# taki0112/vit-tensorflow

Measured on AMD Instinct MI355X. Metric: images/sec (fwd+bwd) ViT-B/16 224px bf16, higher is better.
Workload: dtype bf16; 1 GPU; vit_b16_224 fwd+bwd, batch 256/GPU, N(0,1) NHWC images resident in HBM, random-init weights, softmax-CE cotangent, dropout 0; global_batch=256, parallelism=dp1, compute=bf16

## Files before the change

### vit-tensorflow_amd/csrc/attn_bf16.hip

```cpp
#include "kernels.h"
#include "attn_lds.h"

#ifdef VITX_ATTN_PROBE
__device__ unsigned long long* vitx_attn_probe_buf;
#define ATTN_STAMP(i) do { if (threadIdx.x == 0 && vitx_attn_probe_buf) { vitx_attn_probe_buf[(size_t)blockIdx.x * 8 + (i)] = wall_clock64(); \
    if ((i) == 0) vitx_attn_probe_buf[(size_t)blockIdx.x * 8 + 6] = (unsigned long long)__builtin_amdgcn_s_getreg(63492) | ((unsigned long long)__builtin_amdgcn_s_getreg(63508) << 32); } } while (0)
#else
#define ATTN_STAMP(i) do { } while (0)
#endif

namespace {

using namespace attn_lds;

constexpr int ATT_THREADS = 512;

struct AttnLayout {
  int64_t tok_stride;
  int64_t kv_off;
  int64_t o_stride;
  int64_t q0, o0;
};
__device__ __forceinline__ AttnLayout attn_layout(int planar, int bi, int hi, int nb, int n, int h) {
  AttnLayout a;
// ... 77 lines not shown
}

template <bool MASKED, int QB>
__device__ __forceinline__ void fwd_max_pair(const char* k_rm, int u, int qi, int g, int n, const bf16x8 (&qf)[QB][2], float (&m)[QB]) {
  bf16x8 kf[2][2];
#pragma unroll
  for (int tt = 0; tt < 2; ++tt)
#pragma unroll
    for (int kh = 0; kh < 2; ++kh) kf[tt][kh] = frag_rm(k_rm, (2 * u + tt) * 16 + qi, g + 4 * kh);
  f32x4 a[2][QB];
#pragma unroll
  for (int tt = 0; tt < 2; ++tt)
#pragma unroll
    for (int s = 0; s < QB; ++s) a[tt][s] = mfma16(kf[tt][0], qf[s][0], f32x4{0.f, 0.f, 0.f, 0.f});
#pragma unroll
  for (int tt = 0; tt < 2; ++tt)
#pragma unroll
    for (int s = 0; s < QB; ++s) a[tt][s] = mfma16(kf[tt][1], qf[s][1], a[tt][s]);
#pragma unroll
  for (int tt = 0; tt < 2; ++tt)
#pragma unroll
    for (int s = 0; s < QB; ++s) {
      f32x4 v = a[tt][s];
      if (MASKED) {
#pragma unroll
        for (int r = 0; r < 4; ++r) v[r] = ((2 * u + tt) * 16 + 4 * g + r) < n ? v[r] : -INFINITY;
      }
      m[s] = fmaxf(fmaxf(m[s], fmaxf(v[0], v[1])), fmaxf(v[2], v[3]));
    }
}

template <int NTP>
__global__ __launch_bounds__(ATT_THREADS, 4) void attn_fwd_kernel(const bf16_t* __restrict__ qkv, bf16_t* __restrict__ o, float* __restrict__ lse,
                                                       int n, int h, float scale, const bf16_t* __restrict__ zero_page, int reverse, int planar) {
  constexpr int NKP = 16 * NTP, QB = QB_FWD;
  extern __shared__ __attribute__((aligned(16))) char smem[];
  char* k_rm = smem;
  char* v_rm = smem + NKP * ROWB;
  const int bh = reverse ? (int)(gridDim.x - 1 - blockIdx.x) : (int)blockIdx.x, bi = bh / h, hi = bh - bi * h;
  const AttnLayout L = attn_layout(planar, bi, hi, (int)gridDim.x / h, n, h);
  const int64_t tok_stride = L.tok_stride;
  const bf16_t* qbase = qkv + L.q0;
  const int tid = threadIdx.x, lane = tid & 63, nwaves = blockDim.x >> 6;
  const int wave = __builtin_amdgcn_readfirstlane(tid >> 6);
  ATTN_STAMP(0);
  stage_head_dma(qbase + L.kv_off, tok_stride, n, NKP, k_rm, zero_page, wave, lane, nwaves);
  stage_head_dma(qbase + 2 * L.kv_off, tok_stride, n, NKP, v_rm, zero_page, wave, lane, nwaves);

  const int qi = lane & 15, g = lane >> 4;
  const int nqb = (n + 16 * QB - 1) / (16 * QB);
  const float sl2 = scale * 1.44269504088896340736f;
  bf16x8 qf[QB][2];
  auto load_q = [&](int qb) {
#pragma unroll
    for (int s = 0; s < QB; ++s) {
      const int qc = min((qb * QB + s) * 16 + qi, n - 1);
#pragma unroll
      for (int ks = 0; ks < 2; ++ks) qf[s][ks] = *(const bf16x8*)(qbase + (int64_t)qc * tok_stride + (g + 4 * ks) * 8);
    }
  };
  if (wave < nqb) load_q(wave);
  asm volatile("s_waitcnt vmcnt(0)" ::: "memory");
  ATTN_STAMP(1);
  __syncthreads();
  ATTN_STAMP(2);

  const int u_full = n >> 5;
  const int u_end = min(NTP / 2, (n + 31) >> 5);
  for (int qb = wave; qb < nqb; qb += nwaves) {
    float m[QB];
#pragma unroll
    for (int s = 0; s < QB; ++s) m[s] = -INFINITY;
#pragma unroll 1
    for (int u = 0; u < u_full; ++u) fwd_max_pair<false, QB>(k_rm, u, qi, g, n, qf, m);
    if (u_full < u_end) fwd_max_pair<true, QB>(k_rm, u_full, qi, g, n, qf, m);
#pragma unroll
    for (int s = 0; s < QB; ++s) {
      m[s] = fmaxf(m[s], __shfl_xor(m[s], 16, 64));
      m[s] = fmaxf(m[s], __shfl_xor(m[s], 32, 64));
      m[s] *= sl2;
    }
    ATTN_STAMP(3);
    f32x2 lv[QB];
    f32x4 oacc[QB][4];
#pragma unroll
    for (int s = 0; s < QB; ++s) {
      lv[s] = f32x2{0.f, 0.f};
#pragma unroll
      for (int c = 0; c < 4; ++c) oacc[s][c] = f32x4{0.f, 0.f, 0.f, 0.f};
    }
#pragma unroll 1
    for (int u = 0; u < u_full; ++u) fwd_pair<false, QB>(k_rm, v_rm, u, qi, g, lane, n, qf, sl2, m, lv, oacc);
    if (u_full < u_end) fwd_pair<true, QB>(k_rm, v_rm, u_full, qi, g, lane, n, qf, sl2, m, lv, oacc);
    ATTN_STAMP(4);
#pragma unroll
    for (int s = 0; s < QB; ++s) {
      const int q = (qb * QB + s) * 16 + qi;
      float ls = lv[s][0] + lv[s][1];
      ls += __shfl_xor(ls, 16, 64);
      ls += __shfl_xor(ls, 32, 64);
      const float inv_l = 1.0f / ls;
      if (g == 0 && q < n) lse[(int64_t)bh * n + q] = (m[s] + log2f(ls)) * 0.69314718055994530942f;
      if (q < n) {
        bf16_t* op = o + L.o0 + (int64_t)q * L.o_stride;
#pragma unroll
        for (int c = 0; c < 4; ++c) {
          bf16x4 ov;
#pragma unroll
          for (int r = 0; r < 4; ++r) ov[r] = (bf16_t)(oacc[s][c][r] * inv_l);
          *(bf16x4*)(op + 16 * c + 4 * g) = ov;
        }
      }
    }
    if (qb + nwaves < nqb) load_q(qb + nwaves);
  }
  ATTN_STAMP(5);
}

template <bool MASKED>
__device__ __forceinline__ void dq_pair(const char* k_rm, const char* v_rm, int u, int qi, int g, int lane, int n, const bf16x8 (&qf)[2],
                                        const bf16x8 (&dof)[2], float sl2, float lse2, float scale, float nds, f32x4 (&dq)[4]) {
  bf16x8 kf[2][2], vf[2][2], kt[4];
#pragma unroll
  for (int tt = 0; tt < 2; ++tt)
#pragma unroll
    for (int kh = 0; kh < 2; ++kh) {
      kf[tt][kh] = frag_rm(k_rm, (2 * u + tt) * 16 + qi, g + 4 * kh);
      vf[tt][kh] = frag_rm(v_rm, (2 * u + tt) * 16 + qi, g + 4 * kh);
    }
#pragma unroll
  for (int c = 0; c < 4; ++c) kt[c] = frag_trr(k_rm, c, u, lane);
  f32x4 sa[2], dp[2];
#pragma unroll
  for (int tt = 0; tt < 2; ++tt) {
    sa[tt] = mfma16(kf[tt][0], qf[0], f32x4{0.f, 0.f, 0.f, 0.f});
    dp[tt] = mfma16(vf[tt][0], dof[0], f32x4{0.f, 0.f, 0.f, 0.f});
// ... 4 lines not shown
    dp[tt] = mfma16(vf[tt][1], dof[1], dp[tt]);
  }
  f32x4 ds[2];
#pragma unroll
  for (int tt = 0; tt < 2; ++tt) {
    const f32x4 e = sa[tt] * sl2 - lse2;
    const f32x4 w = dp[tt] * scale + nds;
#pragma unroll
    for (int r = 0; r < 4; ++r) {
      float p = fast_exp2(e[r]);
      if (MASKED) p = ((2 * u + tt) * 16 + 4 * g + r) < n ? p : 0.f;
      ds[tt][r] = p * w[r];
    }
  }
  const bf16x8 dsf = pack8(ds[0], ds[1]);
#pragma unroll
  for (int c = 0; c < 4; ++c) dq[c] = mfma16(kt[c], dsf, dq[c]);
}

struct DqOperands { bf16x8 qf[2], dof[2], of[2]; };
__device__ __forceinline__ void dq_load(DqOperands& x, const bf16_t* qbase, int64_t tok_stride, const bf16_t* o_rows, const bf16_t* do_rows, int64_t inner,
                                        int qb, int lane, int n) {
  const int qc = min(qb * 16 + (lane & 15), n - 1), g = lane >> 4;
#pragma unroll
  for (int ks = 0; ks < 2; ++ks) {
    x.qf[ks] = *(const bf16x8*)(qbase + (int64_t)qc * tok_stride + (g + 4 * ks) * 8);
    x.dof[ks] = *(const bf16x8*)(do_rows + (int64_t)qc * inner + (g + 4 * ks) * 8);
    x.of[ks] = *(const bf16x8*)(o_rows + (int64_t)qc * inner + (g + 4 * ks) * 8);
  }
}

template <int NTP>
__device__ __forceinline__ float dq_block(const char* k_rm, const char* v_rm, const DqOperands& x, int64_t tok_stride, bf16_t* dq_rows, int qb, int lane,
                                          int n, float scale, float lse2) {
  const int qi = lane & 15, g = lane >> 4;
  const int q = qb * 16 + qi;
  const float sl2 = scale * 1.44269504088896340736f;
  const bf16x8 (&qf)[2] = x.qf;
  const bf16x8 (&dof)[2] = x.dof;
  float dsum = 0.f;
#pragma unroll
  for (int ks = 0; ks < 2; ++ks)
#pragma unroll
    for (int e = 0; e < 8; ++e) dsum += (float)x.dof[ks][e] * (float)x.of[ks][e];
  dsum += __shfl_xor(dsum, 16, 64);
  dsum += __shfl_xor(dsum, 32, 64);
  const float nds = -dsum * scale;
  f32x4 dq[4];
#pragma unroll
  for (int c = 0; c < 4; ++c) dq[c] = f32x4{0.f, 0.f, 0.f, 0.f};
  const int u_full = n >> 5, u_end = min(NTP / 2, (n + 31) >> 5);
#pragma unroll 1
  for (int u = 0; u < u_full; ++u) dq_pair<false>(k_rm, v_rm, u, qi, g, lane, n, qf, dof, sl2, lse2, scale, nds, dq);
  if (u_full < u_end) dq_pair<true>(k_rm, v_rm, u_full, qi, g, lane, n, qf, dof, sl2, lse2, scale, nds, dq);
  if (q < n) {
    bf16_t* out = dq_rows + (int64_t)q * tok_stride;
#pragma unroll
    for (int c = 0; c < 4; ++c) {
      bf16x4 ov;
#pragma unroll
      for (int r = 0; r < 4; ++r) ov[r] = (bf16_t)dq[c][r];
      *(bf16x4*)(out + 16 * c + 4 * g) = ov;
    }
  }
  return dsum;
}

struct DkvOperands { bf16x8 kf[2], vf[2]; };
__device__ __forceinline__ void dkv_load(DkvOperands& x, const bf16_t* kbase, int64_t tok_stride, int64_t inner, int kb, int lane, int n) {
  const int kc = min(kb * 16 + (lane & 15), n - 1), g = lane >> 4;
#pragma unroll
  for (int ks = 0; ks < 2; ++ks) {
    x.kf[ks] = *(const bf16x8*)(kbase + (int64_t)kc * tok_stride + (g + 4 * ks) * 8);
    x.vf[ks] = *(const bf16x8*)(kbase + inner + (int64_t)kc * tok_stride + (g + 4 * ks) * 8);
  }
}

template <int NTP>
__device__ __forceinline__ void dkv_block(const char* q_rm, const char* do_rm, const float* lse_s, const float* d_s, const DkvOperands& x,
                                          int64_t tok_stride, int64_t inner, bf16_t* dk_rows, int kb, int lane, int n, float scale) {
  const int ki = lane & 15, g = lane >> 4;
  const int key = kb * 16 + ki;
  const float sl2 = scale * 1.44269504088896340736f;
  const bf16x8 (&kf)[2] = x.kf;
  const bf16x8 (&vf)[2] = x.vf;
  f32x4 dk[4], dv[4];
#pragma unroll
  for (int c = 0; c < 4; ++c) { dk[c] = f32x4{0.f, 0.f, 0.f, 0.f}; dv[c] = f32x4{0.f, 0.f, 0.f, 0.f}; }
  const int u_end = min(NTP / 2, (n + 31) >> 5);
#pragma unroll 1
  for (int u = 0; u < u_end; ++u) {
    f32x4 pp[2], ds[2];
#pragma unroll
    for (int tt = 0; tt < 2; ++tt) {
      const int t = 2 * u + tt;
      const bf16x8 qa0 = frag_rm(q_rm, t * 16 + ki, g), qa1 = frag_rm(q_rm, t * 16 + ki, g + 4);
      const bf16x8 da0 = frag_rm(do_rm, t * 16 + ki, g), da1 = frag_rm(do_rm, t * 16 + ki, g + 4);
      float lq[4], dd[4];
#pragma unroll
      for (int r = 0; r < 4; ++r) { lq[r] = lse_s[t * 16 + 4 * g + r]; dd[r] = d_s[t * 16 + 4 * g + r]; }
      f32x4 sa = {0.f, 0.f, 0.f, 0.f}, dp = {0.f, 0.f, 0.f, 0.f};
      sa = mfma16(qa0, kf[0], sa);
      sa = mfma16(qa1, kf[1], sa);
      dp = mfma16(da0, vf[0], dp);
      dp = mfma16(da1, vf[1], dp);
#pragma unroll
      for (int r = 0; r < 4; ++r) {
        const float p = fast_exp2(fmaf(sa[r], sl2, -lq[r]));
        pp[tt][r] = p;
        ds[tt][r] = p * ((dp[r] - dd[r]) * scale);
      }
    }
    const bf16x8 pf = pack8(pp[0], pp[1]), dsf = pack8(ds[0], ds[1]);
#pragma unroll
    for (int c = 0; c < 4; ++c) {
      const bf16x8 a1 = frag_trr(do_rm, c, u, lane), a2 = frag_trr(q_rm, c, u, lane);
      dv[c] = mfma16(a1, pf, dv[c]);
      dk[c] = mfma16(a2, dsf, dk[c]);
    }
  }
  if (key < n) {
    bf16_t* dkp = dk_rows + (int64_t)key * tok_stride;
    bf16_t* dvp = dkp + inner;
#pragma unroll
    for (int c = 0; c < 4; ++c) {
      bf16x4 a, b2;
#pragma unroll
      for (int r = 0; r < 4; ++r) { a[r] = (bf16_t)dk[c][r]; b2[r] = (bf16_t)dv[c][r]; }
      *(bf16x4*)(dkp + 16 * c + 4 * g) = a;
      *(bf16x4*)(dvp + 16 * c + 4 * g) = b2;
    }
  }
}

template <int NTP>
__global__ __launch_bounds__(ATT_THREADS) void attn_bwd_dq_kernel(const bf16_t* __restrict__ qkv, const bf16_t* __restrict__ o,
                                                          const bf16_t* __restrict__ d_o, const float* __restrict__ lse,
                                                          float* __restrict__ dsum, bf16_t* __restrict__ dqkv, int n, int h, float scale,
                                                          const bf16_t* __restrict__ zero_page) {
  constexpr int NKP = 16 * NTP;
  extern __shared__ __attribute__((aligned(16))) char smem[];
  char* k_rm = smem;
  char* v_rm = smem + NKP * ROWB;
  const int bh = blockIdx.x, bi = bh / h, hi = bh - bi * h;
  const int inner = h * DH;
  const int64_t tok_stride = 3 * (int64_t)inner;
  const bf16_t* qbase = qkv + (int64_t)bi * n * tok_stride + hi * DH;
  const int tid = threadIdx.x, lane = tid & 63, nwaves = blockDim.x >> 6;
  const int wave = __builtin_amdgcn_readfirstlane(tid >> 6);
  stage_head_dma(qbase + inner, tok_stride, n, NKP, k_rm, zero_page, wave, lane, nwaves);
  stage_head_dma(qbase + 2 * inner, tok_stride, n, NKP, v_rm, zero_page, wave, lane, nwaves);
  asm volatile("s_waitcnt vmcnt(0)" ::: "memory");
  __syncthreads();
  const int64_t orow0 = (int64_t)bi * n * inner + hi * DH;
  for (int qb = wave; qb < (n + 15) / 16; qb += nwaves) {
    const int qi = lane & 15, q = qb * 16 + qi, qc = min(q, n - 1);
    DqOperands x;
    dq_load(x, qbase, tok_stride, o + orow0, d_o + orow0, inner, qb, lane, n);
    const float d = dq_block<NTP>(k_rm, v_rm, x, tok_stride, dqkv + (int64_t)bi * n * tok_stride + hi * DH, qb, lane, n, scale,
                                  lse[(int64_t)bh * n + qc] * 1.44269504088896340736f);
    if ((lane >> 4) == 0 && q < n) dsum[(int64_t)bh * n + q] = d;
  }
}

template <int NTP>
__global__ __launch_bounds__(ATT_THREADS) void attn_bwd_dkv_kernel(const bf16_t* __restrict__ qkv, const bf16_t* __restrict__ d_o,
                                                           const float* __restrict__ lse, const float* __restrict__ dsum,
                                                           bf16_t* __restrict__ dqkv, int n, int h, float scale, const bf16_t* __restrict__ zero_page) {
  constexpr int NQP = 16 * NTP;
  extern __shared__ __attribute__((aligned(16))) char smem[];
  char* q_rm = smem;
  char* do_rm = smem + NQP * ROWB;
  float* lse_s = (float*)(smem + 2 * NQP * ROWB);
  float* d_s = lse_s + NQP;
  const int bh = blockIdx.x, bi = bh / h, hi = bh - bi * h;
  const int inner = h * DH;
  const int64_t tok_stride = 3 * (int64_t)inner;
  const bf16_t* qbase = qkv + (int64_t)bi * n * tok_stride + hi * DH;
  const int tid = threadIdx.x, lane = tid & 63, nwaves = blockDim.x >> 6;
  const int wave = __builtin_amdgcn_readfirstlane(tid >> 6);
  stage_head_dma(qbase, tok_stride, n, NQP, q_rm, zero_page, wave, lane, nwaves);
  stage_head_dma(d_o + (int64_t)bi * n * inner + hi * DH, inner, n, NQP, do_rm, zero_page, wave, lane, nwaves);
  for (int i = tid; i < NQP; i += blockDim.x) {
    lse_s[i] = i < n ? lse[(int64_t)bh * n + i] * 1.44269504088896340736f : 0.f;
    d_s[i] = i < n ? dsum[(int64_t)bh * n + i] : 0.f;
  }
  asm volatile("s_waitcnt vmcnt(0)" ::: "memory");
  __syncthreads();
  for (int kb = wave; kb < (n + 15) / 16; kb += nwaves) {
    DkvOperands x;
    dkv_load(x, qbase + inner, tok_stride, inner, kb, lane, n);
    dkv_block<NTP>(q_rm, do_rm, lse_s, d_s, x, tok_stride, inner, dqkv + (int64_t)bi * n * tok_stride + inner + hi * DH, kb, lane, n, scale);
  }
}

template <int NTP>
__global__ __launch_bounds__(ATT_THREADS, 4) void attn_bwd_fused_kernel(const bf16_t* __restrict__ qkv, const bf16_t* __restrict__ o,
                                                             const bf16_t* __restrict__ d_o, const float* __restrict__ lse,
                                                             bf16_t* __restrict__ dqkv, int n, int h, float scale,
                                                             const bf16_t* __restrict__ zero_page, int planar) {
  constexpr int NKP = 16 * NTP, NQP = 16 * NTP;
  extern __shared__ __attribute__((aligned(16))) char smem[];
  char* k_rm = smem;
  char* v_rm = smem + NKP * ROWB;
  char* q_rm = k_rm;
  char* do_rm = v_rm;
  float* lse_s = (float*)(smem + 2 * NKP * ROWB);
  float* d_s = lse_s + NQP;
  const int bh = blockIdx.x, bi = bh / h, hi = bh - bi * h;
  const AttnLayout L = attn_layout(planar, bi, hi, (int)gridDim.x / h, n, h);
  const int64_t tok_stride = L.tok_stride, inner = L.kv_off, ostr = L.o_stride;
  const bf16_t* qbase = qkv + L.q0;
  const int tid = threadIdx.x, lane = tid & 63, nwaves = blockDim.x >> 6;
  const int wave = __builtin_amdgcn_readfirstlane(tid >> 6);
  stage_head_dma(qbase + inner, tok_stride, n, NKP, k_rm, zero_page, wave, lane, nwaves);
  stage_head_dma(qbase + 2 * inner, tok_stride, n, NKP, v_rm, zero_page, wave, lane, nwaves);
  for (int i = tid; i < NQP; i += blockDim.x) {
    lse_s[i] = i < n ? lse[(int64_t)bh * n + i] * 1.44269504088896340736f : 0.f;
    d_s[i] = 0.f;
  }
  const int64_t orow0 = L.o0;
  const int nblk = (n + 15) / 16;
  DqOperands xq;
  if (wave < nblk) dq_load(xq, qbase, tok_stride, o + orow0, d_o + orow0, ostr, wave, lane, n);
  ATTN_STAMP(0);
  asm volatile("s_waitcnt vmcnt(0)" ::: "memory");
  __syncthreads();
  ATTN_STAMP(1);
  for (int qb = wave; qb < nblk; qb += nwaves) {
    const int q = qb * 16 + (lane & 15);
    DqOperands nx;
    if (qb + nwaves < nblk) dq_load(nx, qbase, tok_stride, o + orow0, d_o + orow0, ostr, qb + nwaves, lane, n);
    const float d = dq_block<NTP>(k_rm, v_rm, xq, tok_stride, dqkv + L.q0, qb, lane, n, scale, lse_s[min(q, n - 1)]);
    if ((lane >> 4) == 0 && q < n) d_s[q] = d;
    xq = nx;
  }
  DkvOperands xk;
  if (wave < nblk) dkv_load(xk, qbase + inner, tok_stride, inner, wave, lane, n);
  ATTN_STAMP(2);
  __syncthreads();
  ATTN_STAMP(3);
  stage_head_dma(qbase, tok_stride, n, NQP, q_rm, zero_page, wave, lane, nwaves);
  stage_head_dma(d_o + orow0, ostr, n, NQP, do_rm, zero_page, wave, lane, nwaves);
  asm volatile("s_waitcnt vmcnt(0)" ::: "memory");
  __syncthreads();
  ATTN_STAMP(4);
  for (int kb = wave; kb < nblk; kb += nwaves) {
    DkvOperands nx;
    if (kb + nwaves < nblk) dkv_load(nx, qbase + inner, tok_stride, inner, kb + nwaves, lane, n);
    dkv_block<NTP>(q_rm, do_rm, lse_s, d_s, xk, tok_stride, inner, dqkv + L.q0 + inner, kb, lane, n, scale);
    xk = nx;
  }
  ATTN_STAMP(5);
}

template <typename K>
void set_smem(K kern, int bytes) {
  vitx_set_max_smem((const void*)kern, bytes);
}

#ifdef VITX_ATTN_PROBE
int vitx_attn_probe_threads = 512;
inline int att_threads(int n) { (void)n; return vitx_attn_probe_threads; }
inline int pick_ntp(int n) { return n <= 64 ? 4 : n <= 96 ? 6 : n <= 192 ? 12 : n <= 224 ? 14 : 18; }
#else
inline int att_threads(int n) { (void)n; return 512; }
inline int pick_ntp(int n) { return n <= 64 ? 4 : n <= 96 ? 6 : n <= 224 ? 14 : 18; }
#endif

}

bool attn_bf16_supported(int n, int dim_head) { return dim_head == DH && n >= 1 && n <= 288; }

#define VITX_NTP_DISPATCH(ntp, CALL) \
  do { if ((ntp) == 4) { CALL(4); } else if ((ntp) == 6) { CALL(6); } else if ((ntp) == 14) { CALL(14); } else if ((ntp) == 12) { VITX_NTP12(CALL); } else { CALL(18); } } while (0)
#ifdef VITX_ATTN_PROBE
#define VITX_NTP12(CALL) CALL(12)
#else
#define VITX_NTP12(CALL) CALL(14)
#endif

int vitx_attn_probe_planar = 0;

void launch_attn_bf16_fwd(const bf16_t* qkv, bf16_t* o, float* lse, int b, int n, int h, float scale, const bf16_t* zero_page, int reverse, hipStream_t s) {
  const int ntp = pick_ntp(n);
  const int nkp = 16 * ntp;
  const int smem = 2 * nkp * ROWB;
#define CALL(NTP) { set_smem(attn_fwd_kernel<NTP>, smem); hipLaunchKernelGGL(attn_fwd_kernel<NTP>, dim3(b * h), dim3(att_threads(n)), smem, s, qkv, o, lse, n, h, scale, zero_page, reverse, vitx_attn_probe_planar); }
  VITX_NTP_DISPATCH(ntp, CALL);
#undef CALL
}

void launch_attn_bf16_bwd(const bf16_t* qkv, const bf16_t* o, const bf16_t* d_o, const float* lse, float* dsum_ws, bf16_t* dqkv, int b,
                          int n, int h, float scale, const bf16_t* zero_page, hipStream_t s) {
  const int ntp = pick_ntp(n);
  const int np = 16 * ntp;
  const int smem_dq = 2 * np * ROWB;
  const int smem_dkv = 2 * np * ROWB + 2 * np * 4;
  const char* split_env = vitx_env("VITX_ATTN_BWD_SPLIT");
  const bool split = split_env && atoi(split_env) != 0;
  if (!split) {
#define CALLF(NTP) { set_smem(attn_bwd_fused_kernel<NTP>, smem_dkv); hipLaunchKernelGGL(attn_bwd_fused_kernel<NTP>, dim3(b * h), dim3(att_threads(n)), smem_dkv, s, qkv, o, d_o, lse, dqkv, n, h, scale, zero_page, vitx_attn_probe_planar); }
    VITX_NTP_DISPATCH(ntp, CALLF);
#undef CALLF
    return;
  }
#define CALL(NTP)                                                                                                                  \
  {                                                                                                                                \
    set_smem(attn_bwd_dq_kernel<NTP>, smem_dq);                                                                                    \
    set_smem(attn_bwd_dkv_kernel<NTP>, smem_dkv);                                                                                  \
    hipLaunchKernelGGL(attn_bwd_dq_kernel<NTP>, dim3(b * h), dim3(att_threads(n)), smem_dq, s, qkv, o, d_o, lse, dsum_ws, dqkv, n, h, scale, zero_page);   \
    hipLaunchKernelGGL(attn_bwd_dkv_kernel<NTP>, dim3(b * h), dim3(att_threads(n)), smem_dkv, s, qkv, d_o, lse, dsum_ws, dqkv, n, h, scale, zero_page);    \
  }
  VITX_NTP_DISPATCH(ntp, CALL);
#undef CALL
}
```

### vit-tensorflow_amd/csrc/capi.hip

```cpp
#include <dlfcn.h>

#include <cstring>
#include <map>

#include "composite.h"

static thread_local std::string g_last_error;

static int fail(int code, const std::string& msg) {
  g_last_error = msg;
  return code;
}
int capi_fail(int code, const std::string& msg) { return fail(code, msg); }

extern "C" {

const char* vitx_version(void) { return "vitx 0.1.0 (gfx950)"; }
const char* vitx_last_error(void) { return g_last_error.c_str(); }

int32_t vitx_param_table_size(const vitx_config* cfg, int64_t* n_tensors, int64_t* n_elems) {
  CAPI_TRY
  if (!cfg) return fail(VITX_ERR_INVALID, "null config");
  vitx_config c = *cfg;
  if (c.channels <= 0) c.channels = 3;
// ... 739 lines not shown
  h->prof_events.clear();
  int n = 0;
  for (auto& s : stats) {
    if (s.launches == 0) continue;
    if (out && n < cap) out[n] = s;
    ++n;
  }
  if (n_out) *n_out = n;
  return VITX_OK;
  CAPI_CATCH
}

int32_t vitx_workspace_bytes(vitx_handle h, int64_t* bytes) {
  if (!h) return fail(VITX_ERR_INVALID, "null handle");
  if (bytes) *bytes = h->ws_bytes;
  return VITX_OK;
}

int32_t vitx_debug_read(vitx_handle h, const char* which, int32_t layer, float* out_host, int64_t cap, int64_t* n_elems) {
  CAPI_TRY
  if (!h || !which) return fail(VITX_ERR_INVALID, "null argument");
  const vitx_config& c = h->cfg;
  const int b = h->last_b;
  Stage* st = nullptr;
  int l = layer, nq = h->last_ntok, nk = h->last_ntok;
  for (auto& s : h->stages) {
    if (l < s.depth) { st = &s; break; }
    l -= s.depth;
  }
  const std::string w(which);
  const void* src = nullptr;
  int64_t rows = 0, cols = 0, ld = 0;
  bool is_t = false;
  if (w == "pooled_ln") { src = h->yh; rows = b; cols = ld = c.dim; is_t = true; }
  else if (w == "logits") { src = h->logits; rows = b; cols = c.num_classes; ld = h->nc_k; }
  else if (w == "dlogits") { src = h->dlogits; rows = b; cols = c.num_classes; ld = h->nc_k; }
  else if (w == "patches") { src = h->patches; rows = (int64_t)b * h->last_np; cols = h->pd; ld = h->pd_k; is_t = true; }
  else {
    if (!st) return fail(VITX_ERR_INVALID, "layer out of range");
    if (c.variant == VITX_VARIANT_CAIT) { nq = st->nq_max == 1 ? 1 : h->last_np; nk = st->nq_max == 1 ? 1 + h->last_np : h->last_np; }
    BlockActs& ba = st->ba[(size_t)l];
    rows = (int64_t)b * nq;
    if (w == "x_in" || w == "embed") { src = ba.x_in; cols = ld = c.dim; }
    else if (w == "x_mid") { src = ba.x_mid; cols = ld = c.dim; }
    else if (w == "x_out") { src = ba.x_out; cols = ld = c.dim; }
    else if (w == "y1") { src = ba.y1; cols = ld = c.dim; is_t = true; }
    else if (w == "y2") { src = ba.y2; cols = ld = c.dim; is_t = true; }
    else if (w == "qkv") { src = ba.qkv; cols = ld = 3 * h->inner; is_t = true; }
    else if (w == "q") { src = ba.q; cols = ld = h->inner; is_t = true; }
    else if (w == "kv") { src = ba.kv; rows = (int64_t)b * nk; cols = ld = 2 * h->inner; is_t = true; }
    else if (w == "attn_out") { src = ba.o; cols = ld = h->inner; is_t = true; }
    else if (w == "hpre") { src = ba.hpre; cols = ld = c.mlp_dim; is_t = true; }
    else if (w == "act") { src = ba.act; cols = ld = c.mlp_dim; is_t = true; }
    else return fail(VITX_ERR_INVALID, "unknown activation name");
  }
  if (!src) return fail(VITX_ERR_INVALID, "activation not available for this variant");
  const int64_t n = rows * cols;
  if (n_elems) *n_elems = n;
  if (!out_host) return VITX_OK;
  if (cap < n) return fail(VITX_ERR_INVALID, "output buffer too small");
  float* tmp = nullptr;
  CAPI_HIP(hipMalloc((void**)&tmp, (size_t)std::max<int64_t>(n, 1) * 4));
  launch_to_f32(src, is_t && h->bf16, ld, tmp, cols, (int)rows, (int)cols, h->stream);
  CAPI_HIP(hipMemcpyAsync(out_host, tmp, (size_t)n * 4, hipMemcpyDeviceToHost, h->stream));
  CAPI_HIP(hipStreamSynchronize(h->stream));
  (void)hipFree(tmp);
  return VITX_OK;
  CAPI_CATCH
}

int32_t vitx_check_gemm(vitx_handle h, int32_t kind, int32_t M, int32_t N, int32_t K, int32_t kernel, int32_t epilogue, float* errs2) {
  CAPI_TRY
  if (!h || !errs2) return fail(VITX_ERR_INVALID, "null argument");
  std::string err;
// ... 21 lines not shown
```

### vit-tensorflow_amd/csrc/elementwise.hip

```cpp
#include "kernels.h"

namespace {

template <typename TO>
__global__ void unfold_kernel(const float* __restrict__ img, TO* __restrict__ out, int b, int H, int W, int C, int ph, int pw,
                              int64_t ldo) {
  const int Hp = H / ph, Wp = W / pw;
  const int pd = ph * pw * C;
  const int run = pw * C;
  const int64_t total = (int64_t)b * Hp * Wp * ldo;
  for (int64_t e = (int64_t)blockIdx.x * blockDim.x + threadIdx.x; e < total; e += (int64_t)gridDim.x * blockDim.x) {
    const int64_t row = e / ldo;
    const int f = (int)(e - row * ldo);
    float v = 0.f;
    if (f < pd) {
      const int r = f / run, sc = f - r * run;
      const int wi = (int)(row % Wp);
      const int64_t t = row / Wp;
      const int hi = (int)(t % Hp);
      const int64_t bi = t / Hp;
      v = img[((bi * H + (int64_t)hi * ph + r) * W + (int64_t)wi * pw) * C + sc];
    }
    stf<TO>(out + e, v);
  }
// ... 416 lines not shown
    const int cc = c0 + c, rr = r0 + tx;
    if (cc < cols && rr < rows) op[(int64_t)cc * ldo + rr] = tile[tx][c];
  }
}

template <typename TO>
__global__ void convert_kernel(const float* __restrict__ in, int64_t ldi, TO* __restrict__ out, int64_t ldo, int rows, int cols,
                               int64_t zero_to) {
  const int64_t total = (int64_t)rows * zero_to;
  for (int64_t e = (int64_t)blockIdx.x * blockDim.x + threadIdx.x; e < total; e += (int64_t)gridDim.x * blockDim.x) {
    const int64_t r = e / zero_to;
    const int c = (int)(e - r * zero_to);
    stf<TO>(out + r * ldo + c, c < cols ? in[r * ldi + c] : 0.f);
  }
}

template <typename TI>
__global__ void to_f32_kernel(const TI* __restrict__ in, int64_t ldi, float* __restrict__ out, int64_t ldo, int rows, int cols) {
  const int64_t total = (int64_t)rows * cols;
  for (int64_t e = (int64_t)blockIdx.x * blockDim.x + threadIdx.x; e < total; e += (int64_t)gridDim.x * blockDim.x) {
    const int64_t r = e / cols;
    const int c = (int)(e - r * cols);
    out[r * ldo + c] = ldf<TI>(in + r * ldi + c);
  }
}

__global__ void set_token_row_kernel(float* __restrict__ x, const float* __restrict__ tok, int b, int ntok, int row, int d) {
  const int64_t e = (int64_t)blockIdx.x * blockDim.x + threadIdx.x;
  if (e >= (int64_t)b * d) return;
  const int64_t bi = e / d;
  const int c = (int)(e - bi * d);
  x[(bi * ntok + row) * d + c] = tok[c];
}
__global__ void mean_pool_kernel(const float* __restrict__ x, int b, int ntok, int d, float* __restrict__ out, int stride_tok) {
  const int64_t total = (int64_t)b * d;
  for (int64_t e = (int64_t)blockIdx.x * blockDim.x + threadIdx.x; e < total; e += (int64_t)gridDim.x * blockDim.x) {
    const int64_t bi = e / d;
    const int c = (int)(e - bi * d);
    float a = 0.f;
    for (int t = 0; t < ntok; ++t) a += x[(bi * stride_tok + t) * d + c];
    out[e] = a / (float)ntok;
  }
}
__global__ void mean_pool_bwd_kernel(const float* __restrict__ dp, int b, int ntok, int d, float* __restrict__ g, int stride_tok) {
  const int64_t total = (int64_t)b * ntok * d;
  for (int64_t e = (int64_t)blockIdx.x * blockDim.x + threadIdx.x; e < total; e += (int64_t)gridDim.x * blockDim.x) {
    const int c = (int)(e % d);
    const int64_t bi = e / ((int64_t)ntok * d);
    g[e + bi * (int64_t)(stride_tok - ntok) * d] = dp[bi * d + c] / (float)ntok;
  }
}
__global__ void batch_reduce_kernel(const float* __restrict__ g, int b, int ntok, int d, int j0, int nj, float* __restrict__ out) {
  const int64_t total = (int64_t)nj * d;
  for (int64_t e = (int64_t)blockIdx.x * blockDim.x + threadIdx.x; e < total; e += (int64_t)gridDim.x * blockDim.x) {
    const int64_t j = e / d;
    const int c = (int)(e - j * d);
    float a = 0.f;
    for (int bi = 0; bi < b; ++bi) a += g[((int64_t)bi * ntok + j0 + j) * d + c];
    out[e] = a;
  }
}
template <typename TO>
__global__ void extract_rows_kernel(const float* __restrict__ g, int b, int ntok, int tok_off, int np, int d, TO* __restrict__ out,
                                    int64_t ldo) {
  const int64_t total = (int64_t)b * np * d;
  for (int64_t e = (int64_t)blockIdx.x * blockDim.x + threadIdx.x; e < total; e += (int64_t)gridDim.x * blockDim.x) {
// ... 393 lines not shown
  const int chunks = (int)std::max<int64_t>(1, std::min<int64_t>({(int64_t)CS_CHUNKS, ceil_div(rows, 16), ceil_div(2048, cblocks)}));
  dim3 grid((unsigned)cblocks, chunks), block(256);
  if (is_bf16) hipLaunchKernelGGL(colsum_kernel<bf16_t>, grid, block, 0, s, (const bf16_t*)x, ld, rows, cols, partial_ws);
  else hipLaunchKernelGGL(colsum_kernel<float>, grid, block, 0, s, (const float*)x, ld, rows, cols, partial_ws);
  launch_reduce_partials3(partial_ws, chunks, cols, cols, 1, out, nullptr, nullptr, partial_ws + (int64_t)CS_CHUNKS * cols, 1.0f, s);
}

void launch_convert_weight(const float* w, int in, int out, bf16_t* wn, int64_t ldwn, bf16_t* wt, int64_t ldwt, hipStream_t s) {
  dim3 grid((unsigned)ceil_div(out, 64), (unsigned)ceil_div(in, 64)), block(256);
  hipLaunchKernelGGL(convert_weight_kernel, grid, block, 0, s, w, in, out, wn, ldwn, wt, ldwt);
}
void launch_convert_weights_batched(const ConvertDesc* descs_dev, int n, int total_blocks, hipStream_t s) {
  if (n > 0 && total_blocks > 0) hipLaunchKernelGGL(convert_weights_batched_kernel, dim3((unsigned)total_blocks), dim3(256), 0, s, descs_dev, n);
}
void launch_transpose_bf16(const bf16_t* in, int64_t ldi, int rows, int cols, bf16_t* out, int64_t ldo, hipStream_t s) {
  dim3 grid((unsigned)ceil_div(cols, 64), (unsigned)ceil_div(rows, 64)), block(256);
  hipLaunchKernelGGL(transpose_bf16_kernel, grid, block, 0, s, in, ldi, rows, cols, out, ldo);
}
void launch_convert(const float* in, int64_t ldi, void* out, int out_bf16, int64_t ldo, int rows, int cols, int64_t zero_to,
                    hipStream_t s) {
  const int64_t total = (int64_t)rows * zero_to;
  if (total == 0) return;
  if (out_bf16) hipLaunchKernelGGL(convert_kernel<bf16_t>, dim3(grid_for(total)), dim3(256), 0, s, in, ldi, (bf16_t*)out, ldo, rows, cols, zero_to);
  else hipLaunchKernelGGL(convert_kernel<float>, dim3(grid_for(total)), dim3(256), 0, s, in, ldi, (float*)out, ldo, rows, cols, zero_to);
}
void launch_to_f32(const void* in, int in_bf16, int64_t ldi, float* out, int64_t ldo, int rows, int cols, hipStream_t s) {
  const int64_t total = (int64_t)rows * cols;
  if (total == 0) return;
  if (in_bf16) hipLaunchKernelGGL(to_f32_kernel<bf16_t>, dim3(grid_for(total)), dim3(256), 0, s, (const bf16_t*)in, ldi, out, ldo, rows, cols);
  else hipLaunchKernelGGL(to_f32_kernel<float>, dim3(grid_for(total)), dim3(256), 0, s, (const float*)in, ldi, out, ldo, rows, cols);
}
void launch_set_token_row(float* x, const float* tok, int b, int ntok, int row, int d, hipStream_t s) {
  hipLaunchKernelGGL(set_token_row_kernel, dim3((unsigned)ceil_div((int64_t)b * d, 256)), dim3(256), 0, s, x, tok, b, ntok, row, d);
}
void launch_mean_pool(const float* x, int b, int ntok, int d, float* out, hipStream_t s, int stride_tok) {
  hipLaunchKernelGGL(mean_pool_kernel, dim3(grid_for((int64_t)b * d)), dim3(256), 0, s, x, b, ntok, d, out, stride_tok ? stride_tok : ntok);
}
void launch_mean_pool_bwd(const float* dp, int b, int ntok, int d, float* g, hipStream_t s, int stride_tok) {
  hipLaunchKernelGGL(mean_pool_bwd_kernel, dim3(grid_for((int64_t)b * ntok * d)), dim3(256), 0, s, dp, b, ntok, d, g, stride_tok ? stride_tok : ntok);
}
void launch_batch_reduce(const float* g, int b, int ntok, int d, int j0, int nj, float* out, hipStream_t s) {
  if (nj <= 0) return;
  if (d % 4 == 0 && ((uintptr_t)g) % 16 == 0 && ((uintptr_t)out) % 16 == 0) {
    if (b >= 32) hipLaunchKernelGGL(batch_reduce4_split_kernel, dim3((unsigned)ceil_div((int64_t)nj * (d / 4), 64)), dim3(512), 0, s, g, b, ntok, d / 4, j0, nj, out);
    else hipLaunchKernelGGL(batch_reduce4_kernel, dim3((unsigned)ceil_div((int64_t)nj * (d / 4), 64)), dim3(64), 0, s, g, b, ntok, d / 4, j0, nj, out);
    return;
  }
  hipLaunchKernelGGL(batch_reduce_kernel, dim3(grid_for((int64_t)nj * d)), dim3(256), 0, s, g, b, ntok, d, j0, nj, out);
}
void launch_extract_rows(const float* g, int b, int ntok, int tok_off, int np, int d, void* out, int out_bf16, int64_t ldo, hipStream_t s) {
  const int64_t total = (int64_t)b * np * d;
  if (total == 0) return;
  if (d % 4 == 0 && ldo % 4 == 0 && ((uintptr_t)g) % 16 == 0 && ((uintptr_t)out) % 16 == 0) {
    if (out_bf16) hipLaunchKernelGGL(extract_rows4_kernel<bf16_t>, dim3(grid_for(total / 4)), dim3(256), 0, s, g, b, ntok, tok_off, np, d / 4, (bf16_t*)out, ldo);
    else hipLaunchKernelGGL(extract_rows4_kernel<float>, dim3(grid_for(total / 4)), dim3(256), 0, s, g, b, ntok, tok_off, np, d / 4, (float*)out, ldo);
    return;
  }
  if (out_bf16) hipLaunchKernelGGL(extract_rows_kernel<bf16_t>, dim3(grid_for(total)), dim3(256), 0, s, g, b, ntok, tok_off, np, d, (bf16_t*)out, ldo);
  else hipLaunchKernelGGL(extract_rows_kernel<float>, dim3(grid_for(total)), dim3(256), 0, s, g, b, ntok, tok_off, np, d, (float*)out, ldo);
}
void launch_sum_rows(const float* in, int rows, int d, float* out, hipStream_t s) {
  if (rows >= 32) hipLaunchKernelGGL(sum_rows_split_kernel, dim3((unsigned)ceil_div(d, 64)), dim3(256), 0, s, in, rows, d, out);
  else hipLaunchKernelGGL(sum_rows_kernel, dim3((unsigned)ceil_div(d, 256)), dim3(256), 0, s, in, rows, d, out);
}
void launch_ce_grad(const float* logits, int64_t ld, const int32_t* labels, int b, int nc, float inv_batch, float* dlogits, float* loss,
                    hipStream_t s) {
// ... 187 lines not shown
```

### vit-tensorflow_amd/csrc/engine.h

```cpp
#pragma once
#include <string>
#include <vector>

#include "../../include/vitx.h"
#include "kernels.h"

struct ParamDesc {
  std::string name;
  std::vector<int64_t> shape;
  int64_t offset = 0, count = 0;
  int64_t aoff = 0;
};

std::string build_param_table(const vitx_config& c, std::vector<ParamDesc>& out);

struct CommState {
  hipStream_t stream = nullptr;
  void* all_reduce = nullptr;
  int overlap = 0;
  int64_t bucket = 0;
  int wire_bf16 = 0;
  bf16_t* wire = nullptr;
  std::vector<int64_t> covered;
  std::vector<char> launched;
// ... 15 lines not shown
  int64_t w = -1, b = -1;
  bf16_t* wt = nullptr;
  bf16_t* wn = nullptr;
  const float *ext_w = nullptr, *ext_b = nullptr;
  float *ext_gw = nullptr, *ext_gb = nullptr;
};

struct BlockParams {
  int64_t a_scale = -1, ln1_g = -1, ln1_b = -1;
  int64_t temp = -1;
  Dense qkv, q, kv, out;
  Dense qkvcat;
  bool has_out = true;
  int64_t mix_pre = -1, mix_post = -1, re_w = -1, re_g = -1, re_b = -1;
  int64_t m_scale = -1, ln2_g = -1, ln2_b = -1;
  Dense fc1, fc2;
  int64_t p_begin = 0, p_end = 0;
};

struct BlockActs {
  float *x_in = nullptr, *x_mid = nullptr, *x_out = nullptr;
  void *y1 = nullptr, *qkv = nullptr, *q = nullptr, *kv = nullptr, *ctx = nullptr, *o = nullptr, *fa = nullptr;
  void *y2 = nullptr, *hpre = nullptr, *act = nullptr, *fm = nullptr;
  float *mean1 = nullptr, *rstd1 = nullptr, *mean2 = nullptr, *rstd2 = nullptr, *lse = nullptr;
  const float *ln1_src = nullptr, *ln2_src = nullptr;
  bool skip_attn = false, skip_mlp = false;
  float* sc_keep[3] = {nullptr, nullptr, nullptr};
  int64_t sc_keep_elems = 0;
  int64_t sc_geom = -1;
  int sc_pi = 0;
  bool sc_no_mixed = false;
  bool sc_a2_bf16 = false;
  int par_first = 0, par_last = 0;
};

struct Stage {
  std::string prefix;
  int depth = 0;
  int nq_max = 0, nc_max = 0;
  std::vector<BlockParams> bp;
  std::vector<BlockActs> ba;
};

struct ProfEvent {
  int cls;
  int cls2 = -1;
  hipEvent_t e0, e1;
  double flops, bytes;
};

constexpr int SIDE_RING_MAX = 8;
struct SideRing {
  void* slot[SIDE_RING_MAX] = {};
  hipEvent_t rd[SIDE_RING_MAX] = {};
  bool pend[SIDE_RING_MAX] = {};
  int n = 0, cur = 0;
};
struct PendingReady { int64_t off, cnt; hipEvent_t ev; };

struct vitx_engine {
  vitx_config cfg{};
  std::vector<ParamDesc> table;
  int64_t n_params = 0;
  int64_t n_arena = 0;
  bool bf16 = false;
  bool x3_attn = false;
// ... 28 lines not shown
  int merge_after = -1, merge_t = 0;
  int64_t pm_g = -1, pm_b = -1, pm_q = -1;
  float *pm_xn = nullptr, *pm_mean = nullptr, *pm_rstd = nullptr, *pm_attn = nullptr, *pm_dattn = nullptr, *pm_out = nullptr, *pm_dxn = nullptr,
        *pm_dxn2 = nullptr, *pm_dq = nullptr;

  int64_t spt_g = -1, spt_b = -1;
  float *spt_mean = nullptr, *spt_rstd = nullptr, *spt_img = nullptr, *spt_ws = nullptr, *lsa_ws = nullptr;

  int64_t pos = -1, cls = -1, head_g = -1, head_b = -1;
  Dense patch, head;
  std::vector<Stage> stages;

  std::vector<void*> allocs;
  std::vector<std::pair<void*, size_t>> t_buffers;
  int64_t ws_bytes = 0;
  float* img_dev = nullptr;
  void* patches = nullptr;
  float* pooled = nullptr; void* yh = nullptr; float *mean_h = nullptr, *rstd_h = nullptr;
  float *logits = nullptr, *dlogits = nullptr; void* dl_lp = nullptr; void* dyh = nullptr; float* dpooled = nullptr;
  float* g2 = nullptr;
  float* g = nullptr; void* g_lp = nullptr; float* g_ctx = nullptr;
  void *d_h = nullptr, *d_y = nullptr, *d_o = nullptr, *d_qkv = nullptr, *d_ctx = nullptr, *d_br = nullptr;
  bf16_t *xt = nullptr, *dyt = nullptr; int64_t t_rows = 0;
  float* partial_ws = nullptr; int64_t partial_elems = 0;
  float* red_ws = nullptr; int64_t red_elems = 0;
  float* sc[4] = {nullptr, nullptr, nullptr, nullptr}; int64_t sc_elems = 0;
  float* dsum = nullptr;
  void* zero_page = nullptr;
  float* tmp_f32 = nullptr;
  float* loss_rows = nullptr;
  float* distill_ws = nullptr;
  float *opt_m = nullptr, *opt_v = nullptr; int opt_step = 0;
  bf16_t *bench_a = nullptr, *bench_b = nullptr; float* bench_c = nullptr; int64_t bench_elems = 0;

  bool have_fwd = false;
  bool have_tf = false;
  int next_patch_np = 0;
  const float* fwd_patches = nullptr;
  int fwd_np = 0;
  bool last_from_patches = false;
  int tf_b = 0, tf_n = 0;
  float tf_drop = 0.f;
  uint64_t tf_seed = 0;
  bool have_embed = false, have_head = false;
  int shell_b = 0, shell_n = 0;
  float* shell_x = nullptr;
  bool have_pt = false;
  int pt_b = 0, pt_np = 0;
  int64_t patch_rows = -1;
  void* pt_dy = nullptr;
  int64_t pt_dy_rows = -1;
  int last_extra = 0;
  int last_b = 0, last_np = 0, last_ntok = 0, last_H = 0, last_W = 0, last_training = 0;
  uint64_t last_seed = 0;
  std::vector<std::vector<bool>> layer_kept;
  int64_t zero_geom = -1;

  bool keep_scores = true;
  int64_t sc_keep_bytes = 0, sc_keep_budget = 48LL << 30;
  bool force_generic_gemm = false, force_generic_attn = false, wgrad_via_transpose = true;
  bool small_attn = true;
  int gemm_kernel = 0;
  int gemm_tail = 0;
  int reverse_mask = 7;
  int64_t reverse_min_bytes = 200ll << 20;
  bool bgemm_pairs = true;
// ... 6 lines not shown
  bool score_bf16 = true;
  bool cait_qkv_cat = true;
  bool cait_fused = true;
  bool deepvit_fused = true;
  bool unfused_headops = false;
  int gemm_stagger = 0;

  bool profiling = false;
  std::vector<ProfEvent> prof_events;
  std::vector<std::string> prof_names;

  vitx_grad_ready_fn grad_cb = nullptr; void* grad_cb_user = nullptr;
  void* rccl_lib = nullptr; void* comm = nullptr; int rank = 0, world = 1;
  CommState cm;
};

int comm_unique_id(void* out128, std::string& err);
int comm_init(vitx_engine* e, int rank, int world, const void* uid, std::string& err);
int comm_overlap(vitx_engine* e, int enable, int64_t bucket_bytes, int wire_bf16, std::string& err);
void comm_on_ready(vitx_engine* e, int64_t off, int64_t cnt);
int comm_busy(vitx_engine* e);
void comm_wait_event(vitx_engine* e, hipEvent_t ev);
int comm_finish(vitx_engine* e, std::string& err);
void comm_stats(vitx_engine* e, int64_t* out4);
void comm_destroy(vitx_engine* e);

int engine_check_small_dataset(const vitx_config& cfg, std::string& err);
int engine_create(const vitx_config& cfg, vitx_engine** out, std::string& err);
void engine_destroy(vitx_engine* e);
int engine_forward(vitx_engine* e, const float* img_dev, int b, int H, int W, int training, uint64_t seed, float* logits_dev,
                   std::string& err, const float* distill_token_dev = nullptr, float* distill_out_dev = nullptr);
int engine_backward(vitx_engine* e, const float* dlogits_dev, float* dimg_dev, std::string& err, const float* d_distill_dev = nullptr,
                    float* d_token_out_dev = nullptr);
int engine_transformer_forward(vitx_engine* e, const float* tokens_dev, int b, int n, int training, uint64_t seed, float* out_dev, std::string& err);
int engine_transformer_backward(vitx_engine* e, const float* dout_dev, float* dtokens_dev, std::string& err);
int engine_patch_tokens_forward(vitx_engine* e, const float* img_dev, int b, int H, int W, float* tokens_dev, float* patches_f32_dev_or_null,
                                std::string& err);
int engine_patch_tokens_backward(vitx_engine* e, const float* dtokens_dev, std::string& err);
int engine_embed_forward(vitx_engine* e, const float* img_dev, int b, int H, int W, float* tokens_dev, std::string& err);
int engine_spt_forward(vitx_engine* e, const float* img_dev, int b, int H, int W, float* tokens_dev, std::string& err);
int engine_patch_dense_forward(vitx_engine* e, const float* patches_dev, int rows, float* out_dev, std::string& err);
int engine_head_forward(vitx_engine* e, const float* x_dev, int b, int n, float* logits_dev, std::string& err);
int engine_head_backward(vitx_engine* e, const float* dlogits_dev, float* dx_dev, std::string& err);
int engine_embed_backward(vitx_engine* e, const float* dtokens_dev, float* dimg_dev, std::string& err);
void engine_refresh_weights(vitx_engine* e);
void engine_params_moved(vitx_engine* e);
int engine_ext_dense_init(vitx_engine* e, Dense& w, int in, int out, const float* W, const float* bias, float* gW, float* gbias, std::string& err);
void engine_ext_dense_refresh(vitx_engine* e, const Dense& w);
void engine_ext_dense_fwd(vitx_engine* e, const void* X, int64_t ldx, int rows, const Dense& w, float* y);
void engine_ext_dense_bwd(vitx_engine* e, const void* X, int64_t ldx, const void* dY, int64_t ldy, const float* dY_f32, int rows, const Dense& w,
                          float* dx_or_null);
int engine_check_gemm(vitx_engine* e, int kind, int M, int N, int K, int kernel, int epilogue, float* errs, std::string& err);
int engine_bench_gemm(vitx_engine* e, int M, int N, int K, int kernel, int epilogue, int iters, float* avg_ms, float* max_err,
                      std::string& err);
int prof_class(vitx_engine* e, const char* name);
```

### vit-tensorflow_amd/csrc/engine.hip

```cpp
#include "engine.h"

#include <algorithm>
#include <cmath>
#include <cstdio>
#include <cstdlib>
#include <cstring>

#define HIPCHK(x)                                                                                   \
  do {                                                                                              \
    hipError_t e_ = (x);                                                                            \
    if (e_ != hipSuccess) {                                                                         \
      err = std::string(#x) + ": " + hipGetErrorString(e_);                                         \
      return VITX_ERR_HIP;                                                                          \
    }                                                                                               \
  } while (0)

std::string build_param_table(const vitx_config& c, std::vector<ParamDesc>& out) {
  out.clear();
  if (c.variant < 0 || c.variant > 3) return "unknown variant";
  if (c.patch_h <= 0 || c.patch_w <= 0 || c.image_h <= 0 || c.image_w <= 0) return "image/patch size must be positive";
  if (c.image_h % c.patch_h != 0 || c.image_w % c.patch_w != 0)
    return "Image dimensions must be divisible by the patch size.";
  if (c.variant != VITX_VARIANT_CAIT && c.pool != VITX_POOL_CLS && c.pool != VITX_POOL_MEAN)
    return "pool type must be either cls (cls token) or mean (mean pooling)";
// ... 840 lines not shown
    Prof pr(e, "attn_generic_headops", 0, 0);
    if (e->cfg.variant == VITX_VARIANT_CAIT) {
      launch_headmix_bwd(sc[1], dA, e->params + bp.mix_post, dA, e->red_ws, e->grads + bp.mix_post, b, h, a.nq, a.nk, ld, e->stream);
      launch_softmax_bwd_rows(sc[1], dA, rows, a.nk, ld, e->stream);
      launch_headmix_bwd(sc[0], dA, e->params + bp.mix_pre, dA, e->red_ws, e->grads + bp.mix_pre, b, h, a.nq, a.nk, ld, e->stream);
    } else if (e->cfg.variant == VITX_VARIANT_DEEPVIT) {
      launch_headnorm_bwd(sc[1], dA, e->params + bp.re_g, dA, e->red_ws, e->grads + bp.re_g, e->grads + bp.re_b, b, h, a.nq, a.nk, ld,
                          e->cfg.ln_eps, e->stream);
      launch_headmix_bwd(sc[0], dA, e->params + bp.re_w, dA, e->red_ws, e->grads + bp.re_w, b, h, a.nq, a.nk, ld, e->stream);
      launch_softmax_bwd_rows(sc[0], dA, rows, a.nk, ld, e->stream);
    } else {
      launch_softmax_bwd_rows(sc[0], dA, rows, a.nk, ld, e->stream);
    }
  }
  if (ds_lp) {
    bgemm_pair(e, BgemmCall{ds_lp, 1, ld2, 1, bs2, hs2, a.k, T, a.ldk, 1, a.kb, dh, a.nq, dh, a.nk, b, h, EPI_STORE, T, gr.dq, gr.lddq, gr.dqb, dh, scale},
               BgemmCall{ds_lp, 1, 1, ld2, bs2, hs2, a.q, T, a.ldq, 1, a.qb, dh, a.nk, dh, a.nq, b, h, EPI_STORE, T, gr.dk, gr.lddk, gr.dkb, dh, scale});
    return;
  }
  bgemm_pair(e, BgemmCall{dA, 0, ld, 1, bs, hs, a.k, T, a.ldk, 1, a.kb, dh, a.nq, dh, a.nk, b, h, EPI_STORE, T, gr.dq, gr.lddq, gr.dqb, dh, scale},
             BgemmCall{dA, 0, 1, ld, bs, hs, a.q, T, a.ldq, 1, a.qb, dh, a.nk, dh, a.nq, b, h, EPI_STORE, T, gr.dk, gr.lddk, gr.dkb, dh, scale});
}

static bool use_small_attn(const vitx_engine* e, int n) {
  return e->cfg.nest_block && e->small_attn && !e->force_generic_attn && attn_small_supported(n, e->cfg.dim_head);
}
static bool use_fused_attn(const vitx_engine* e, int n) {
  return e->bf16 && e->cfg.variant == VITX_VARIANT_VIT && !e->force_generic_attn && attn_bf16_supported(n, e->cfg.dim_head);
}
static bool use_fused_attn_x3(const vitx_engine* e, int n) {
  return e->x3 && e->x3_attn && e->x3_fused_attn && e->cfg.variant == VITX_VARIANT_VIT && !e->force_generic_attn && attn_x3_supported(n, e->cfg.dim_head);
}

static int block_forward(vitx_engine* e, Stage& st, int si, int l, int b, int nq, int nc, const float* context, float drop, uint64_t seed,
                         std::string& err) {
  const uint32_t site0 = (uint32_t)((si * 1000 + l) * 4);
  const BlockParams& bp = st.bp[l];
  BlockActs& ba = st.ba[l];
  const vitx_config& c = e->cfg;
  const int d = c.dim, inner = e->inner, m = c.mlp_dim, T = e->bf16, esz = e->esz;
  const int rows = b * nq;
  const int nk = nq + nc;
  const double lnb = (double)rows * d * (4 + esz);
  if (!ba.skip_attn) {
  {
    Prof pr(e, "layernorm_fwd", 0, lnb);
    launch_layernorm_fwd(ba.ln1_src ? ba.ln1_src : ba.x_in, d, e->params + bp.ln1_g, e->params + bp.ln1_b, ba.y1, T, d, ba.mean1, ba.rstd1, rows, d, c.ln_eps,
                         e->stream);
  }
  AttnView av;
  av.nq = nq; av.nk = nk; av.o = ba.o; av.ldo = inner; av.ob = (int64_t)nq * inner;
  if (c.variant == VITX_VARIANT_CAIT && bp.qkvcat.wt) {
    EpiParams ep; ep.out = ba.qkv; ep.ldo = 3 * inner;
    dense_fwd(e, ba.y1, d, rows, bp.qkvcat, EPI_STORE, ep);
    av.q = ba.qkv; av.k = boff(ba.qkv, inner, esz); av.v = boff(ba.qkv, 2 * inner, esz);
    av.ldq = av.ldk = av.ldv = 3 * inner;
    av.qb = av.kb = av.vb = (int64_t)nq * 3 * inner;
  } else if (c.variant == VITX_VARIANT_CAIT) {
    EpiParams ep; ep.out = ba.q; ep.ldo = inner;
    dense_fwd(e, ba.y1, d, rows, bp.q, EPI_STORE, ep);
    const void* ctx = ba.y1;
    if (nc > 0) {
      Prof pr(e, "concat_ctx", 0, 0);
      launch_concat_ctx(ba.y1, T, context, ba.ctx, T, b, nq, nc, d, e->stream);
      ctx = ba.ctx;
    }
    EpiParams ep2; ep2.out = ba.kv; ep2.ldo = 2 * inner;
    dense_fwd(e, ctx, d, b * nk, bp.kv, EPI_STORE, ep2);
    av.q = ba.q; av.ldq = inner; av.qb = (int64_t)nq * inner;
    av.k = ba.kv; av.ldk = 2 * inner; av.kb = (int64_t)nk * 2 * inner;
    av.v = boff(ba.kv, inner, esz); av.ldv = 2 * inner; av.vb = av.kb;
  } else {
    EpiParams ep; ep.out = ba.qkv; ep.ldo = 3 * inner;
    dense_fwd(e, ba.y1, d, rows, bp.qkv, EPI_STORE, ep);
    av.q = ba.qkv; av.k = boff(ba.qkv, inner, esz); av.v = boff(ba.qkv, 2 * inner, esz);
    av.ldq = av.ldk = av.ldv = 3 * inner;
    av.qb = av.kb = av.vb = (int64_t)nq * 3 * inner;
  }
  if (c.small_dataset) {
    Prof pr(e, "attn_lsa_fwd", 4.0 * b * c.heads * (double)nq * nq * c.dim_head, (double)rows * inner * 4 * esz);
    launch_attn_lsa_fwd(ba.qkv, ba.o, ba.lse, T, b, nq, c.heads, c.dim_head, e->params + bp.temp, e->stream);
  } else if (use_small_attn(e, nq)) {
    Prof pr(e, "attn_small_fwd", 4.0 * b * c.heads * (double)nq * nq * c.dim_head, (double)rows * inner * 4 * esz);
    launch_attn_small_fwd(ba.qkv, ba.o, ba.lse, T, b, nq, c.heads, c.dim_head, 1.0f / std::sqrt((float)c.dim_head), e->stream);
  } else if (use_fused_attn_x3(e, nq)) {
    Prof pr(e, "attn_x3_fwd", 4.0 * b * c.heads * (double)nq * nq * c.dim_head, (double)rows * inner * 4 * esz);
    launch_attn_x3_fwd((const float*)ba.qkv, (float*)ba.o, ba.lse, b, nq, c.heads, 1.0f / std::sqrt((float)c.dim_head), e->stream);
  } else if (use_fused_attn(e, nq)) {
    Prof pr(e, "attn_bf16_fwd", 4.0 * b * c.heads * (double)nq * nq * c.dim_head, (double)rows * inner * 4 * esz);
    launch_attn_bf16_fwd((const bf16_t*)ba.qkv, (bf16_t*)ba.o, ba.lse, b, nq, c.heads, 1.0f / std::sqrt((float)c.dim_head), (const bf16_t*)e->zero_page, (e->reverse_mask >> 2) & 1, e->stream);
  } else {
    const int need = c.variant == VITX_VARIANT_VIT ? 1 : 3;
    if (e->keep_scores && ba.sc_keep_elems == 0) {
      const int64_t emax = (int64_t)c.max_batch * c.heads * st.nq_max * round_up(st.nq_max + st.nc_max, 4);
      if (e->sc_keep_bytes + need * emax * 4 <= e->sc_keep_budget) {
        for (int i = 0; i < need; ++i) DALLOC(ba.sc_keep[i], (size_t)emax * 4, false);
        ba.sc_keep_elems = emax;
        e->sc_keep_bytes += need * emax * 4;
      } else {
        ba.sc_keep_elems = -1;
      }
    }
    const int64_t elems = (int64_t)b * c.heads * nq * round_up(nk, 4);
    const bool keep = e->keep_scores && ba.sc_keep_elems >= elems;
    if (!keep) {
      ba.sc_geom = -1;
      int rc = ensure_scores(e, need, elems, err);
      if (rc != VITX_OK) return rc;
    }
    attn_generic_fwd(e, bp, av, b, keep ? &ba : nullptr);
  }
  if (bp.has_out && drop > 0.f) {
    EpiParams ep; ep.out = e->tmp_f32; ep.ldo = d;
    dense_fwd(e, ba.o, inner, rows, bp.out, EPI_STORE_F32, ep);
    Prof pr(e, "dropout", 0, 0);
    launch_dropout(e->tmp_f32, 0, (int64_t)rows * d, drop, seed, site0 + 1, e->stream);
    launch_axpy_resid(ba.x_in, e->tmp_f32, bp.a_scale >= 0 ? e->params + bp.a_scale : nullptr, ba.x_mid, bp.a_scale >= 0 ? ba.fa : nullptr, T,
                      rows, d, e->stream);
  } else if (bp.has_out) {
    EpiParams ep;
    ep.out = ba.x_mid; ep.ldo = d; ep.resid = ba.x_in; ep.ldr = d;
    if (bp.a_scale >= 0) { ep.scale = e->params + bp.a_scale; ep.out2 = ba.fa; ep.ldo2 = d; }
    dense_fwd(e, ba.o, inner, rows, bp.out, EPI_BIAS_RESID, ep);
  } else {
    Prof pr(e, "resid_add", 0, 0);
    launch_resid_add(ba.x_in, ba.o, T, ba.x_mid, (int64_t)rows * d, e->stream);
  }
  }
  if (ba.skip_mlp) return VITX_OK;
  {
    Prof pr(e, "layernorm_fwd", 0, lnb);
    launch_layernorm_fwd(ba.ln2_src ? ba.ln2_src : ba.x_mid, d, e->params + bp.ln2_g, e->params + bp.ln2_b, ba.y2, T, d, ba.mean2, ba.rstd2, rows, d, c.ln_eps,
                         e->stream);
  }
  const float* mlp_resid = ba.x_mid;
  if (c.cct_block) {
    if (T) {
      Prof pr(e, "layernorm_fwd", 0, lnb);
      launch_layernorm_fwd(ba.x_mid, d, e->params + bp.ln2_g, e->params + bp.ln2_b, e->tmp_f32, 0, d, ba.mean2, ba.rstd2, rows, d, c.ln_eps, e->stream);
      mlp_resid = e->tmp_f32;
    } else {
      mlp_resid = (const float*)ba.y2;
    }
  }
  {
    EpiParams ep; ep.out = ba.hpre; ep.ldo = m; ep.out2 = ba.act; ep.ldo2 = m;
    ep.nt_out = e->nt_mask & 1;
    dense_fwd(e, ba.y2, d, rows, bp.fc1, EPI_BIAS_GELU, ep);
  }
  if (drop > 0.f) {
    {
      Prof pr(e, "dropout", 0, 0);
      launch_dropout(ba.act, T, (int64_t)rows * m, drop, seed, site0 + 2, e->stream);
    }
    EpiParams ep; ep.out = e->tmp_f32; ep.ldo = d;
    dense_fwd(e, ba.act, m, rows, bp.fc2, EPI_STORE_F32, ep);
    Prof pr(e, "dropout", 0, 0);
    launch_dropout(e->tmp_f32, 0, (int64_t)rows * d, drop, seed, site0 + 3, e->stream);
    launch_axpy_resid(ba.x_mid, e->tmp_f32, bp.m_scale >= 0 ? e->params + bp.m_scale : nullptr, ba.x_out, bp.m_scale >= 0 ? ba.fm : nullptr, T,
                      rows, d, e->stream);
  } else {
    EpiParams ep;
    ep.out = ba.x_out; ep.ldo = d; ep.resid = mlp_resid; ep.ldr = d;
    if (bp.m_scale >= 0) { ep.scale = e->params + bp.m_scale; ep.out2 = ba.fm; ep.ldo2 = d; }
    dense_fwd(e, ba.act, m, rows, bp.fc2, EPI_BIAS_RESID, ep);
  }
  return VITX_OK;
}

static inline int64_t branch_key(int si, int l, int mlp) { return (((int64_t)si + 1) << 32) | ((int64_t)l << 1) | mlp; }
static int block_backward(vitx_engine* e, Stage& st, int si, int l, int b, int nq, int nc, float drop, uint64_t seed, std::string& err, int next_l = -1) {
  const uint32_t site0 = (uint32_t)((si * 1000 + l) * 4);
  const BlockParams& bp = st.bp[l];
  BlockActs& ba = st.ba[l];
  const vitx_config& c = e->cfg;
  const int d = c.dim, inner = e->inner, m = c.mlp_dim, T = e->bf16, esz = e->esz;
  const int rows = b * nq, nk = nq + nc;
  const void* gT = T ? e->g_lp : (const void*)e->g;
  const double lnb = (double)rows * d * (4 + 4 + 4 + esz + esz);
  const bool grouped = ba.par_first || ba.par_last || ba.ln1_src || ba.ln2_src;
  const float* ln_gin = (!grouped || ba.par_first) ? e->g : e->g2;
  float* ln_gout = (!grouped || ba.par_last) ? e->g : e->g2;
  bool glp_dead = e->glp_skip;
  for (const Stage& sx : e->stages)
    for (const BlockParams& bx : sx.bp) glp_dead = glp_dead && bx.a_scale >= 0 && bx.m_scale >= 0;
  const bool ln_writes_glp = T && (!grouped || ba.par_last) && !glp_dead;
  auto next_glp = [&]() -> void* {
    if (!ln_writes_glp) return nullptr;
    side_rotate(e, e->rg_glp, e->g_lp);
    return e->g_lp;
  };

  const void* dbranch = gT;
  bool fc2_bias_done = false, out_bias_done = false;
  const int64_t key_mlp = branch_key(si, l, 1), key_attn = branch_key(si, l, 0);
  if (!ba.skip_mlp) {
  if (e->dbr_ready == key_mlp) {
    e->dbr_ready = 0;
    dbranch = e->d_br;
    fc2_bias_done = dense_gb(e, bp.fc2) != nullptr;
  } else if (bp.m_scale >= 0 || drop > 0.f) {
    Prof pr(e, "branch_grad", 0, 0);
    const bool one_pass = bp.m_scale >= 0 && drop == 0.f && d % 4 == 0;
    fc2_bias_done = one_pass && dense_gb(e, bp.fc2) != nullptr;
    side_rotate(e, e->rg_dbr, e->d_br);
    if (bp.m_scale >= 0)
      launch_scale_grad(ba.fm, T, d, e->g, d, rows, d, e->red_ws, e->grads + bp.m_scale, e->stream, one_pass ? e->params + bp.m_scale : nullptr,
                        one_pass ? e->d_br : nullptr, d, fc2_bias_done ? dense_gb(e, bp.fc2) : nullptr);
    if (!one_pass) launch_branch_grad(e->g, bp.m_scale >= 0 ? e->params + bp.m_scale : nullptr, e->d_br, T, rows, d, drop, seed, site0 + 3, e->stream);
    dbranch = e->d_br;
  }
  const bool fc1_bias_fused = e->bf16 && !e->force_generic_gemm && !(e->gemm_kernel & 256) && drop == 0.f && bp.fc1.b >= 0;
  const int cs_rows = (int)ceil_div(rows, 96);
  const hipEvent_t fork_fc2 = side_prefork(e);
  hipEvent_t fork_fc1 = nullptr;
  {
    side_rotate(e, e->rg_dh, e->d_h);
    EpiParams ep; ep.out = e->d_h; ep.ldo = m; ep.aux = ba.hpre; ep.ldaux = m;
    const bool cs_side = fc1_bias_fused && e->side_live && e->side2 && e->rg_cs.n && rows >= e->side2_min_rows;
    if (cs_side) side_rotate(e, e->rg_cs, e->cs_part);
    float* cs = cs_side ? e->cs_part : e->red_ws;
    if (fc1_bias_fused) {
      launch_fill_zero(cs, (int64_t)cs_rows * m * 4, e->stream);
      ep.colsum = cs; ep.ldcs = m;
    }
    dense_dgrad(e, dbranch, d, rows, bp.fc2, EPI_GELU_BWD, ep);
    if (fc1_bias_fused) {
      Prof pr(e, "reduce_partials", 0, (double)(cs_rows + 1) * m * 4);
      if (cs_side) side2_begin(e);
// ... 35 lines not shown
      block_layernorm_bwd(e, e->tmp_f32, 0, d, ba.x_mid, ba.mean2, ba.rstd2, e->params + bp.ln2_g, nullptr, ln_gout, nullptr, e->grads + bp.ln2_g,
                          e->grads + bp.ln2_b, nullptr, rows);
      if (ln_glp) launch_convert(ln_gout, d, ln_glp, 1, d, rows, d, d, e->stream);
    } else
    block_layernorm_bwd(e, e->d_y, T, d, ba.ln2_src ? ba.ln2_src : ba.x_mid, ba.mean2, ba.rstd2, e->params + bp.ln2_g, ln_gin, ln_gout, ln_glp,
                        e->grads + bp.ln2_g, e->grads + bp.ln2_b, fc2_bias_in_ln ? e->grads + bp.fc2.b : nullptr, rows, fuse ? &nb : nullptr);
  }
  }
  if (ba.skip_attn) {
    report_ready(e, bp.p_begin, bp.p_end - bp.p_begin);
    return VITX_OK;
  }

  gT = T ? e->g_lp : (const void*)e->g;
  dbranch = gT;
  if (e->dbr_ready == key_attn) {
    e->dbr_ready = 0;
    dbranch = e->d_br;
    out_bias_done = bp.has_out && dense_gb(e, bp.out) != nullptr;
  } else if (bp.a_scale >= 0 || (drop > 0.f && bp.has_out)) {
    Prof pr(e, "branch_grad", 0, 0);
    const float adrop = bp.has_out ? drop : 0.f;
    const bool one_pass = bp.a_scale >= 0 && adrop == 0.f && d % 4 == 0;
    out_bias_done = one_pass && bp.has_out && dense_gb(e, bp.out) != nullptr;
    side_rotate(e, e->rg_dbr, e->d_br);
    if (bp.a_scale >= 0)
      launch_scale_grad(ba.fa, T, d, e->g, d, rows, d, e->red_ws, e->grads + bp.a_scale, e->stream, one_pass ? e->params + bp.a_scale : nullptr,
                        one_pass ? e->d_br : nullptr, d, out_bias_done ? dense_gb(e, bp.out) : nullptr);
    if (!one_pass) launch_branch_grad(e->g, bp.a_scale >= 0 ? e->params + bp.a_scale : nullptr, e->d_br, T, rows, d, adrop, seed, site0 + 1, e->stream);
    dbranch = e->d_br;
  }
  bool out_bias_in_ln = false;
  const void* d_o = dbranch;
  if (bp.has_out) {
    EpiParams ep; ep.out = e->d_o; ep.ldo = inner;
    const hipEvent_t fork_out = side_prefork(e);
    dense_dgrad(e, dbranch, d, rows, bp.out, EPI_STORE, ep);
    dense_wgrad(e, ba.o, inner, dbranch, d, rows, bp.out, fork_out);
    side_note_read(e, dbranch == e->d_br ? e->rg_dbr : e->rg_glp);
    out_bias_in_ln = dbranch != e->d_br && !grouped;
    if (!out_bias_in_ln && !out_bias_done) bias_grad(e, dbranch == e->d_br ? (const void*)e->d_br : (const void*)e->g, dbranch == e->d_br ? T : 0, d, rows, bp.out);
    d_o = e->d_o;
  }
  side_rotate(e, e->rg_dqkv, e->d_qkv);
  AttnView av;
  av.nq = nq; av.nk = nk; av.o = ba.o; av.ldo = inner; av.ob = (int64_t)nq * inner;
  AttnGrad ag;
  ag.d_o = d_o; ag.ldo = inner; ag.ob = (int64_t)nq * inner;
  if (c.variant == VITX_VARIANT_CAIT && bp.qkvcat.wt) {
    av.q = ba.qkv; av.k = boff(ba.qkv, inner, esz); av.v = boff(ba.qkv, 2 * inner, esz);
    av.ldq = av.ldk = av.ldv = 3 * inner;
    av.qb = av.kb = av.vb = (int64_t)nq * 3 * inner;
    ag.dq = e->d_qkv; ag.dk = boff(e->d_qkv, inner, esz); ag.dv = boff(e->d_qkv, 2 * inner, esz);
    ag.lddq = ag.lddk = ag.lddv = 3 * inner;
    ag.dqb = ag.dkb = ag.dvb = (int64_t)nq * 3 * inner;
    int rc = ensure_scores(e, 4, (int64_t)b * c.heads * nq * round_up(nk, 4), err);
    if (rc != VITX_OK) return rc;
    attn_generic_bwd(e, bp, av, ag, b, &ba);
    EpiParams ep; ep.out = e->d_y; ep.ldo = d;
    const hipEvent_t fork_qkv = side_prefork(e);
    dense_dgrad(e, e->d_qkv, 3 * inner, rows, bp.qkvcat, EPI_STORE, ep);
    dense_wgrad(e, ba.y1, d, ag.dq, 3 * inner, rows, bp.q, fork_qkv);
    dense_wgrad(e, ba.y1, d, ag.dk, 3 * inner, rows, bp.kv, fork_qkv);
    side_note_read(e, e->rg_dqkv);
  } else if (c.variant == VITX_VARIANT_CAIT) {
    av.q = ba.q; av.ldq = inner; av.qb = (int64_t)nq * inner;
    av.k = ba.kv; av.ldk = 2 * inner; av.kb = (int64_t)nk * 2 * inner;
// ... 12 lines not shown
    dense_dgrad(e, dq, inner, rows, bp.q, EPI_STORE, ep);
    dense_wgrad(e, ba.y1, d, dq, inner, rows, bp.q, fork_qkv);
    EpiParams ep2; ep2.out = e->d_ctx; ep2.ldo = d;
    dense_dgrad(e, dkv, 2 * inner, b * nk, bp.kv, EPI_STORE, ep2);
    dense_wgrad(e, ctx, d, dkv, 2 * inner, b * nk, bp.kv, fork_qkv);
    side_note_read(e, e->rg_dqkv);
    Prof pr(e, "ctx_bwd", 0, 0);
    if (nc > 0) {
      side_rotate(e, e->rg_dbr, e->d_br);
      launch_split_ctx_bwd(e->d_ctx, T, e->d_br, e->g_ctx, b, nq, nc, d, e->stream);
      launch_add_T(e->d_y, e->d_br, T, (int64_t)rows * d, e->stream);
    } else {
      launch_add_T(e->d_y, e->d_ctx, T, (int64_t)rows * d, e->stream);
    }
  } else {
    av.q = ba.qkv; av.k = boff(ba.qkv, inner, esz); av.v = boff(ba.qkv, 2 * inner, esz);
    av.ldq = av.ldk = av.ldv = 3 * inner;
    av.qb = av.kb = av.vb = (int64_t)nq * 3 * inner;
    ag.dq = e->d_qkv; ag.dk = boff(e->d_qkv, inner, esz); ag.dv = boff(e->d_qkv, 2 * inner, esz);
    ag.lddq = ag.lddk = ag.lddv = 3 * inner;
    ag.dqb = ag.dkb = ag.dvb = (int64_t)nq * 3 * inner;
    if (c.small_dataset) {
      Prof pr(e, "attn_lsa_bwd", 14.0 * b * c.heads * (double)nq * nq * c.dim_head, (double)rows * inner * 8 * esz);
      launch_attn_lsa_bwd(ba.qkv, ba.o, d_o, ba.lse, e->dsum, e->d_qkv, T, b, nq, c.heads, c.dim_head, e->params + bp.temp, e->grads + bp.temp,
                          e->lsa_ws, e->stream);
    } else if (use_small_attn(e, nq)) {
      Prof pr(e, "attn_small_bwd", 14.0 * b * c.heads * (double)nq * nq * c.dim_head, (double)rows * inner * 8 * esz);
      launch_attn_small_bwd(ba.qkv, ba.o, d_o, ba.lse, e->dsum, e->d_qkv, T, b, nq, c.heads, c.dim_head, 1.0f / std::sqrt((float)c.dim_head), e->stream);
    } else if (use_fused_attn_x3(e, nq)) {
      Prof pr(e, "attn_x3_bwd", 14.0 * b * c.heads * (double)nq * nq * c.dim_head, (double)rows * inner * 8 * esz);
      launch_attn_x3_bwd((const float*)ba.qkv, (const float*)ba.o, (const float*)d_o, ba.lse, (float*)e->d_qkv, b, nq, c.heads,
                         1.0f / std::sqrt((float)c.dim_head), e->stream);
    } else if (use_fused_attn(e, nq)) {
      Prof pr(e, "attn_bf16_bwd", 14.0 * b * c.heads * (double)nq * nq * c.dim_head, (double)rows * inner * 8 * esz);
      launch_attn_bf16_bwd((const bf16_t*)ba.qkv, (const bf16_t*)ba.o, (const bf16_t*)d_o, ba.lse, e->dsum, (bf16_t*)e->d_qkv, b, nq,
                           c.heads, 1.0f / std::sqrt((float)c.dim_head), (const bf16_t*)e->zero_page, e->stream);
    } else {
      int rc = ensure_scores(e, 4, (int64_t)b * c.heads * nq * round_up(nk, 4), err);
      if (rc != VITX_OK) return rc;
      attn_generic_bwd(e, bp, av, ag, b, &ba);
    }
    EpiParams ep; ep.out = e->d_y; ep.ldo = d;
    ep.nt_out = (e->nt_mask >> 4) & 1;
    const hipEvent_t fork_qkv = side_prefork(e);
    dense_dgrad(e, e->d_qkv, 3 * inner, rows, bp.qkv, EPI_STORE, ep);
    dense_wgrad(e, ba.y1, d, e->d_qkv, 3 * inner, rows, bp.qkv, fork_qkv);
    side_note_read(e, e->rg_dqkv);
  }
  {
    Prof pr(e, "layernorm_bwd", 0, lnb);
    NextBranch nb{nullptr, nullptr, nullptr, nullptr};
    bool fuse = false;
    if (next_l >= 0 && e->ln_scale_fused && T && !grouped && drop == 0.f && !out_bias_in_ln && layernorm_bwd_scale_ok(d)) {
      const BlockParams& np_ = st.bp[(size_t)next_l];
      const BlockActs& na = st.ba[(size_t)next_l];
      if (np_.m_scale >= 0 && !na.skip_mlp && !(na.par_first || na.par_last || na.ln1_src || na.ln2_src)) {
        nb = NextBranch{na.fm, e->params + np_.m_scale, e->grads + np_.m_scale, dense_gb(e, np_.fc2)};
        fuse = true;
      }
    }
    void* ln_glp = fuse ? nullptr : next_glp();
    if (fuse) { side_rotate(e, e->rg_dbr, e->d_br); e->dbr_ready = branch_key(si, next_l, 1); }
    block_layernorm_bwd(e, e->d_y, T, d, ba.ln1_src ? ba.ln1_src : ba.x_in, ba.mean1, ba.rstd1, e->params + bp.ln1_g, ln_gin, ln_gout, ln_glp,
                        e->grads + bp.ln1_g, e->grads + bp.ln1_b, out_bias_in_ln ? e->grads + bp.out.b : nullptr, rows, fuse ? &nb : nullptr);
  }
  report_ready(e, bp.p_begin, bp.p_end - bp.p_begin);
  return VITX_OK;
}

// ... 289 lines not shown
  DALLOC(e->dlogits, (size_t)e->bp * e->nc_k * 4, false);
  DALLOC(e->dl_lp, (size_t)e->bp * e->nc_k * esz, true);
  DALLOC(e->dyh, (size_t)e->bp * d * esz, true);
  DALLOC(e->dpooled, (size_t)e->bp * d * 4, false);
  DALLOC(e->loss_rows, (size_t)e->bp * 4, false);
  DALLOC(e->g, (size_t)rmax * d * 4, false);
  if (c.num_parallel_branches > 1) DALLOC(e->g2, (size_t)rmax * d * 4, false);
  if (e->bf16) DALLOC(e->g_lp, (size_t)rmax * d * esz, true);
  if (cait) DALLOC(e->g_ctx, (size_t)e->mpp * d * 4, false);
  DALLOC(e->d_h, (size_t)rmax * m * esz, true);
  DALLOC(e->d_y, (size_t)rmax * d * esz, true);
  DALLOC(e->d_o, (size_t)rmax * inner * esz, true);
  DALLOC(e->d_qkv, (size_t)(rmax + 256) * 3 * inner * esz + (size_t)crow_max * 2 * inner * esz, true);
  DALLOC(e->d_ctx, (size_t)crow_max * d * esz, true);
  DALLOC(e->d_br, (size_t)rmax * d * esz, true);
  if (e->side) {
    auto ring = [&](SideRing& r, void* first, size_t bytes, int n) -> int {
      r.n = n; r.cur = 0; r.slot[0] = first;
      for (int i = 1; i < n; ++i) DALLOC(r.slot[i], bytes, true);
      for (int i = 0; i < n; ++i) HIPCHK(hipEventCreateWithFlags(&r.rd[i], hipEventDisableTiming));
      return VITX_OK;
    };
    if ((rc = ring(e->rg_dh, e->d_h, (size_t)rmax * m * esz, 2)) != VITX_OK) return rc;
    if ((rc = ring(e->rg_glp, e->g_lp, (size_t)rmax * d * esz, 3)) != VITX_OK) return rc;
    if ((rc = ring(e->rg_dqkv, e->d_qkv, (size_t)(rmax + 256) * 3 * inner * esz + (size_t)crow_max * 2 * inner * esz, 2)) != VITX_OK) return rc;
    if ((rc = ring(e->rg_dbr, e->d_br, (size_t)rmax * d * esz, 3)) != VITX_OK) return rc;
    DALLOC(e->ln_part, (size_t)layernorm_bwd_ws_elems(d) * 4, false);
    if ((rc = ring(e->rg_lnp, e->ln_part, (size_t)layernorm_bwd_ws_elems(d) * 4, 4)) != VITX_OK) return rc;
    const size_t cs_bytes = (size_t)(ceil_div(rmax, 96) + 64) * m * 4;
    DALLOC(e->cs_part, cs_bytes, false);
    if ((rc = ring(e->rg_cs, e->cs_part, cs_bytes, 4)) != VITX_OK) return rc;
  }
  DALLOC(e->dsum, (size_t)B * c.heads * e->ntok_cap * 4 + 16, false);
  if (c.small_dataset) {
    e->spt_g = find_param(e, "patch_embedding.norm.gamma");
    e->spt_b = find_param(e, "patch_embedding.norm.beta");
    DALLOC(e->spt_mean, (size_t)e->mpp * 4, false);
    DALLOC(e->spt_rstd, (size_t)e->mpp * 4, false);
    DALLOC(e->spt_img, (size_t)B * c.image_h * c.image_w * c.channels * 4, false);
    DALLOC(e->spt_ws, (size_t)spt_bwd_ws_elems(e->pd) * 4, false);
    DALLOC(e->lsa_ws, (size_t)attn_lsa_ws_elems((int)B, e->ntok_cap, c.heads) * 4, false);
  }
  DALLOC(e->zero_page, 256, false);
  DALLOC(e->tmp_f32, (size_t)rmax * std::max<int64_t>(d, e->pd) * 4, false);
  const int64_t maxfeat = std::max<int64_t>({(int64_t)d, 3LL * inner, (int64_t)m, (int64_t)e->pd_k, (int64_t)e->nc_k});
  if (e->x3) {
    const int64_t max_w = std::max<int64_t>({(int64_t)d * 3 * inner, (int64_t)d * m, (int64_t)e->pd * d, (int64_t)d * c.num_classes, (int64_t)inner * d});
    e->partial_elems = std::min<int64_t>(64LL * 1024 * 1024, 32 * max_w);
    DALLOC(e->partial_ws, (size_t)e->partial_elems * 4, false);
  }
  if (e->bf16) {
    e->t_rows = round_up(maxfeat, 256);
    if (e->wgrad_via_transpose) {
      DALLOC(e->xt, (size_t)e->t_rows * rmax * 2, false);
      DALLOC(e->dyt, (size_t)e->t_rows * rmax * 2, false);
    }
    const int64_t max_w = std::max<int64_t>({(int64_t)d * 3 * inner, (int64_t)d * m, (int64_t)e->pd * d, (int64_t)d * c.num_classes, (int64_t)inner * d});
    e->partial_elems = 512LL * 256 * 256 + 2 * max_w;
    DALLOC(e->partial_ws, (size_t)e->partial_elems * 4, false);
  }
  e->red_elems = std::max<int64_t>({layernorm_bwd_ws_elems(d), colsum_ws_elems((int)maxfeat), headmix_ws_elems((int)B, c.heads, 1, 1),
                                    (int64_t)256 * 2 * 32, (int64_t)(1024 + 64) * d, (ceil_div(std::max<int64_t>(e->mp, e->mpp), 96) + 40) * (int64_t)m,
                                    headchain_ws_elems(c.heads), deepvit_point_ws_elems((int)B, c.heads, e->ntok_cap),
                                    deepvit_point_bwd_ws_elems(c.heads), deepvit_attn_bwd_ws_elems((int)B, c.heads, e->ntok_cap)});
  DALLOC(e->red_ws, (size_t)e->red_elems * 4, false);
  HIPCHK(hipStreamSynchronize(e->stream));
// ... 143 lines not shown
  }
  EpiParams ep; ep.out = e->logits; ep.ldo = e->nc_k;
  dense_fwd(e, e->yh, d, b, e->head, EPI_STORE_F32, ep);
  if (logits_dev)
    HIPCHK(hipMemcpy2DAsync(logits_dev, (size_t)c.num_classes * 4, e->logits, (size_t)e->nc_k * 4, (size_t)c.num_classes * 4, b,
                            hipMemcpyDeviceToDevice, e->stream));
  return VITX_OK;
}

int engine_forward(vitx_engine* e, const float* img_dev, int b, int H, int W, int training, uint64_t seed, float* logits_dev,
                   std::string& err, const float* distill_token_dev, float* distill_out_dev) {
  const vitx_config& c = e->cfg;
  const int extra = distill_token_dev ? 1 : 0;
  if (extra && c.variant == VITX_VARIANT_CAIT) { err = "distillation token: ViT / DeepViT only"; return VITX_ERR_UNSUPPORTED; }
  if (b <= 0 || b > c.max_batch) { err = "batch must be in [1, max_batch]"; return VITX_ERR_INVALID; }
  const float* patches_in = e->fwd_patches;
  e->fwd_patches = nullptr;
  if (c.cct_block) { err = "cct_block handles serve vitx_cct_* through the transformer entry points only"; return VITX_ERR_UNSUPPORTED; }
  if (c.nest_block) { err = "nest_block handles serve vitx_nest_* through the transformer entry points only"; return VITX_ERR_UNSUPPORTED; }
  if (c.small_dataset && (patches_in || extra)) { err = "small_dataset handles take images only (no patch rows, no distillation token)"; return VITX_ERR_UNSUPPORTED; }
  if (patches_in) {
    if (e->fwd_np <= 0 || e->fwd_np > e->np_max) { err = "forward_patches: np must be in [1, num_patches]"; return VITX_ERR_INVALID; }
    H = e->fwd_np * c.patch_h; W = c.patch_w;
  } else if (H <= 0 || W <= 0 || H > c.image_h || W > c.image_w || H % c.patch_h || W % c.patch_w) {
    err = "Image dimensions must be divisible by the patch size.";
    return VITX_ERR_INVALID;
  }
  const bool cait = c.variant == VITX_VARIANT_CAIT, merger = c.variant == VITX_VARIANT_PATCH_MERGER;
  if (extra && merger) { err = "distillation token: ViT / DeepViT only"; return VITX_ERR_UNSUPPORTED; }
  const bool no_cls = cait || merger;
  const int np = (H / c.patch_h) * (W / c.patch_w);
  const int ntok = no_cls ? np : np + 1 + extra;
  const int d = c.dim, T = e->bf16;
  ensure_geometry(e, b, ntok);
  if (e->params_dirty) engine_refresh_weights(e);
  Stage& s0 = e->stages[0];
  float* x0 = s0.depth > 0 ? s0.ba[0].x_in : e->tmp_f32;
  prepare_patch_rows(e, (int64_t)b * np);
  if (patches_in) {
    launch_convert(patches_in, e->pd, e->patches, T, e->pd_k, b * np, e->pd, e->pd_k, e->stream);
  } else if (c.small_dataset) {
    if (img_dev != e->spt_img) HIPCHK(hipMemcpyAsync(e->spt_img, img_dev, (size_t)b * H * W * c.channels * 4, hipMemcpyDeviceToDevice, e->stream));
    Prof pr(e, "spt_fwd", 0, (double)b * H * W * c.channels * 4 + (double)b * np * e->pd_k * e->esz);
    launch_spt_fwd(e->spt_img, e->patches, T, e->pd_k, e->spt_mean, e->spt_rstd, e->params + e->spt_g, e->params + e->spt_b, b, H, W, c.channels,
                   c.patch_h, c.ln_eps, e->stream);
  } else {
    Prof pr(e, "patch_unfold", 0, (double)b * H * W * c.channels * 4 + (double)b * np * e->pd_k * e->esz);
    launch_unfold(img_dev, e->patches, T, b, H, W, c.channels, c.patch_h, c.patch_w, e->pd_k, e->stream);
  }
  e->last_from_patches = patches_in != nullptr;
  if (!no_cls) {
    Prof pr(e, "cls_pos_row", 0, 0);
    launch_cls_pos_row(x0, e->params + e->cls, e->params + e->pos, b, ntok, d, d, e->stream);
  }
  {
    EpiParams ep;
    ep.out = x0; ep.ldo = d; ep.pos = e->params + e->pos; ep.ldr = d;
    ep.np = np; ep.ntok = ntok; ep.tok_off = no_cls ? 0 : 1;
    dense_fwd(e, e->patches, e->pd_k, b * np, e->patch, EPI_PATCH, ep);
  }
  if (extra)
    launch_set_token_row(x0, distill_token_dev, b, ntok, ntok - 1, d, e->stream);
  const float drop = training ? c.dropout : 0.f, emb_drop = training ? c.emb_dropout : 0.f;
  if (emb_drop > 0.f) {
    Prof pr(e, "dropout", 0, 0);
    launch_dropout(x0, 0, (int64_t)b * ntok * d, emb_drop, seed, 0u, e->stream);
  }
  draw_layer_dropout(e, seed);
  int rc;
  for (int l = 0; l < s0.depth; ++l) {
    if (!e->layer_kept[0][(size_t)l]) {
      HIPCHK(hipMemcpyAsync(s0.ba[l].x_out, s0.ba[l].x_in, (size_t)b * ntok * d * 4, hipMemcpyDeviceToDevice, e->stream));
      continue;
    }
    const bool merged = merger && e->merge_after >= 0 && l > e->merge_after;
    if ((rc = block_forward(e, s0, 0, l, b, merged ? e->merge_t : ntok, 0, nullptr, drop, seed, err)) != VITX_OK) return rc;
    if (merger && l == e->merge_after) merger_forward(e, s0.ba[l].x_out, b, ntok);
  }
  const float* x_last = s0.depth > 0 ? s0.ba[s0.depth - 1].x_out : x0;
  int head_tok = ntok;
  if (merger && e->merge_after >= 0) {
    head_tok = e->merge_t;
    if (e->merge_after == s0.depth - 1) x_last = e->pm_out;
  }
  if (cait) {
    Stage& s1 = e->stages[1];
    float* xc = s1.depth > 0 ? s1.ba[0].x_in : e->pooled;
    {
      Prof pr(e, "cls_broadcast", 0, 0);
      launch_broadcast_rows(e->params + e->cls, d, xc, b, e->stream);
    }
    for (int l = 0; l < s1.depth; ++l) {
      if (!e->layer_kept[1][(size_t)l]) {
        HIPCHK(hipMemcpyAsync(s1.ba[l].x_out, s1.ba[l].x_in, (size_t)b * d * 4, hipMemcpyDeviceToDevice, e->stream));
        continue;
      }
      if ((rc = block_forward(e, s1, 1, l, b, 1, np, x_last, drop, seed, err)) != VITX_OK) return rc;
    }
    x_last = s1.depth > 0 ? s1.ba[s1.depth - 1].x_out : xc;
    head_tok = 1;
  }
  if (extra && distill_out_dev)
    HIPCHK(hipMemcpy2DAsync(distill_out_dev, (size_t)d * 4, x_last + (int64_t)(ntok - 1) * d, (size_t)ntok * d * 4, (size_t)d * 4, b, hipMemcpyDeviceToDevice, e->stream));
  if ((rc = head_forward(e, x_last, b, head_tok, cait ? 0 : extra, logits_dev, err)) != VITX_OK) return rc;
  e->last_extra = extra;
  e->have_fwd = true;
  e->have_tf = false;
  e->last_b = b; e->last_np = np; e->last_ntok = ntok; e->last_H = H; e->last_W = W; e->last_training = training; e->last_seed = seed;
  return VITX_OK;
}

static int shell_check(const vitx_engine* e, std::string& err) {
  const vitx_config& c = e->cfg;
  if (c.variant != VITX_VARIANT_VIT && c.variant != VITX_VARIANT_DEEPVIT) { err = "embed / head entry points: ViT / DeepViT handles only"; return VITX_ERR_UNSUPPORTED; }
  if (c.num_parallel_branches > 1) { err = "embed / head entry points: not for parallel_vit handles"; return VITX_ERR_UNSUPPORTED; }
  if (c.small_dataset) { err = "embed / head entry points: not for small_dataset handles"; return VITX_ERR_UNSUPPORTED; }
  if (c.cct_block) { err = "embed / head entry points: not for cct_block handles"; return VITX_ERR_UNSUPPORTED; }
  if (c.nest_block) { err = "embed / head entry points: not for nest_block handles"; return VITX_ERR_UNSUPPORTED; }
  return VITX_OK;
}

int engine_embed_forward(vitx_engine* e, const float* img_dev, int b, int H, int W, float* tokens_dev, std::string& err) {
  const vitx_config& c = e->cfg;
  int rc;
  if ((rc = shell_check(e, err)) != VITX_OK) return rc;
  if (b <= 0 || b > c.max_batch) { err = "batch must be in [1, max_batch]"; return VITX_ERR_INVALID; }
  if (H <= 0 || W <= 0 || H > c.image_h || W > c.image_w || H % c.patch_h || W % c.patch_w) {
    err = "image dimensions must be divisible by the patch size";
    return VITX_ERR_INVALID;
  }
  const int np = (H / c.patch_h) * (W / c.patch_w), ntok = np + 1, d = c.dim, T = e->bf16;
  ensure_geometry(e, b, ntok);
  if (e->params_dirty) engine_refresh_weights(e);
  prepare_patch_rows(e, (int64_t)b * np);
  {
    Prof pr(e, "patch_unfold", 0, (double)b * H * W * c.channels * 4 + (double)b * np * e->pd_k * e->esz);
    launch_unfold(img_dev, e->patches, T, b, H, W, c.channels, c.patch_h, c.patch_w, e->pd_k, e->stream);
  }
  {
    Prof pr(e, "cls_pos_row", 0, 0);
    launch_cls_pos_row(tokens_dev, e->params + e->cls, e->params + e->pos, b, ntok, d, d, e->stream);
  }
  EpiParams ep;
  ep.out = tokens_dev; ep.ldo = d; ep.pos = e->params + e->pos; ep.ldr = d;
  ep.np = np; ep.ntok = ntok; ep.tok_off = 1;
  dense_fwd(e, e->patches, e->pd_k, b * np, e->patch, EPI_PATCH, ep);
  e->have_fwd = false;
  e->have_embed = true;
  e->last_b = b; e->last_np = np; e->last_ntok = ntok; e->last_H = H; e->last_W = W; e->last_training = 0; e->last_extra = 0;
  return VITX_OK;
}

int engine_spt_forward(vitx_engine* e, const float* img_dev, int b, int H, int W, float* tokens_dev, std::string& err) {
  const vitx_config& c = e->cfg;
  if (!c.small_dataset) { err = "spt_forward: small_dataset handles only"; return VITX_ERR_UNSUPPORTED; }
  if (b <= 0 || b > c.max_batch) { err = "batch must be in [1, max_batch]"; return VITX_ERR_INVALID; }
  if (H <= 0 || W <= 0 || H > c.image_h || W > c.image_w || H % c.patch_h || W % c.patch_w) {
    err = "Image dimensions must be divisible by the patch size.";
    return VITX_ERR_INVALID;
  }
  const int np = (H / c.patch_h) * (W / c.patch_w);
  if (e->params_dirty) engine_refresh_weights(e);
  prepare_patch_rows(e, (int64_t)b * np);
  {
    Prof pr(e, "spt_fwd", 0, (double)b * H * W * c.channels * 4 + (double)b * np * e->pd_k * e->esz);
    launch_spt_fwd(img_dev, e->patches, e->bf16, e->pd_k, e->spt_mean, e->spt_rstd, e->params + e->spt_g, e->params + e->spt_b, b, H, W, c.channels,
                   c.patch_h, c.ln_eps, e->stream);
  }
  EpiParams ep;
  ep.out = tokens_dev; ep.ldo = c.dim;
  dense_fwd(e, e->patches, e->pd_k, b * np, e->patch, EPI_STORE_F32, ep);
  e->have_fwd = false; e->have_embed = false;
  return VITX_OK;
}

int engine_patch_dense_forward(vitx_engine* e, const float* patches_dev, int rows, float* out_dev, std::string& err) {
  const vitx_config& c = e->cfg;
  if (c.small_dataset) { err = "patch_dense_forward: not for small_dataset handles (vitx_spt_forward is their tokenizer)"; return VITX_ERR_UNSUPPORTED; }
  if (rows <= 0 || (int64_t)rows > (int64_t)c.max_batch * e->np_max) { err = "patch_dense_forward: rows must be in [1, max_batch * num_patches]"; return VITX_ERR_INVALID; }
  if (e->params_dirty) engine_refresh_weights(e);
  prepare_patch_rows(e, rows);
  launch_convert(patches_dev, e->pd, e->patches, e->bf16, e->pd_k, rows, e->pd, e->pd_k, e->stream);
  EpiParams ep;
  ep.out = out_dev; ep.ldo = c.dim;
  dense_fwd(e, e->patches, e->pd_k, rows, e->patch, EPI_STORE_F32, ep);
  e->have_fwd = false; e->have_embed = false;
  return VITX_OK;
}

int engine_head_forward(vitx_engine* e, const float* x_dev, int b, int n, float* logits_dev, std::string& err) {
  const vitx_config& c = e->cfg;
  int rc;
  if (b <= 0 || b > c.max_batch || n <= 0 || n > e->ntok_cap) { err = "head_forward: b or n out of range"; return VITX_ERR_INVALID; }
  e->have_fwd = false;
  const int d = c.dim;
  if (e->params_dirty) engine_refresh_weights(e);
  if (!e->shell_x) DALLOC(e->shell_x, (size_t)e->mp * d * 4, false);
  if (x_dev != e->shell_x) HIPCHK(hipMemcpyAsync(e->shell_x, x_dev, (size_t)b * n * d * 4, hipMemcpyDeviceToDevice, e->stream));
  if (e->bf16) {
    const int64_t r1 = round_up(b, 64);
    if (r1 > b) HIPCHK(hipMemsetAsync(boff(e->yh, (int64_t)b * d, 2), 0, (size_t)(r1 - b) * d * 2, e->stream));
  }
  if ((rc = head_forward(e, e->shell_x, b, n, 0, logits_dev, err)) != VITX_OK) return rc;
  e->have_head = true; e->shell_b = b; e->shell_n = n;
  return VITX_OK;
}

int engine_head_backward(vitx_engine* e, const float* dlogits_dev, float* dx_dev, std::string& err) {
  const vitx_config& c = e->cfg;
  if (!e->have_head) { err = "head_backward requires a preceding head_forward"; return VITX_ERR_STATE; }
  const int b = e->shell_b, n = e->shell_n, d = c.dim, T = e->bf16, nc = c.num_classes;
  if (dlogits_dev)
    HIPCHK(hipMemcpy2DAsync(e->dlogits, (size_t)e->nc_k * 4, dlogits_dev, (size_t)nc * 4, (size_t)nc * 4, b, hipMemcpyDeviceToDevice, e->stream));
  {
    Prof pr(e, "head_prep", 0, 0);
    launch_colsum(e->dlogits, 0, e->nc_k, b, nc, e->red_ws, e->grads + e->head.b, e->stream);
    if (T) {
      const int64_t r1 = round_up(b, 64);
      if (r1 > b) HIPCHK(hipMemsetAsync(boff(e->dl_lp, (int64_t)b * e->nc_k, 2), 0, (size_t)(r1 - b) * e->nc_k * 2, e->stream));
      launch_convert(e->dlogits, e->nc_k, e->dl_lp, 1, e->nc_k, b, nc, e->nc_k, e->stream);
    }
  }
  const void* dlT = T ? e->dl_lp : (const void*)e->dlogits;
  {
    EpiParams ep; ep.out = e->dyh; ep.ldo = d;
    dense_dgrad(e, dlT, e->nc_k, b, e->head, EPI_STORE, ep);
  }
// ... 29 lines not shown
  {
    Prof pr(e, "embed_bwd", 0, (double)b * ntok * d * 4);
    if (ntok < e->ntok_max)
      launch_fill_zero(e->grads + e->pos + (int64_t)ntok * d, (int64_t)(e->ntok_max - ntok) * d * 4, e->stream);
    launch_batch_reduce(e->g, b, ntok, d, 0, ntok, e->grads + e->pos, e->stream);
    launch_batch_reduce(e->g, b, ntok, d, 0, 1, e->grads + e->cls, e->stream);
    launch_sum_rows(e->grads + e->pos + d, np, d, e->grads + e->patch.b, e->stream);
  }
  if (dimg_dev) {
    EpiParams ep; ep.out = e->tmp_f32; ep.ldo = e->pd;
    dense_dgrad(e, e->d_y, d, b * np, e->patch, EPI_STORE_F32, ep);
    Prof pr(e, "patch_fold", 0, 0);
    launch_fold_add(e->tmp_f32, e->pd, dimg_dev, b, e->last_H, e->last_W, c.channels, c.patch_h, c.patch_w, e->stream);
  }
  return VITX_OK;
}

int engine_transformer_forward(vitx_engine* e, const float* tokens_dev, int b, int n, int training, uint64_t seed, float* out_dev, std::string& err) {
  const vitx_config& c = e->cfg;
  if (c.variant == VITX_VARIANT_CAIT || c.variant == VITX_VARIANT_PATCH_MERGER) { err = "transformer_forward: ViT / DeepViT only"; return VITX_ERR_UNSUPPORTED; }
  if (c.small_dataset) { err = "transformer_forward: not for small_dataset handles"; return VITX_ERR_UNSUPPORTED; }
  if (b <= 0 || b > c.max_batch || n <= 0 || n > e->ntok_cap) { err = "transformer_forward: b or n out of range"; return VITX_ERR_INVALID; }
  ensure_geometry(e, b, n);
  if (e->params_dirty) engine_refresh_weights(e);
  Stage& s0 = e->stages[0];
  const size_t bytes = (size_t)b * n * c.dim * 4;
  if (s0.depth == 0) { HIPCHK(hipMemcpyAsync(out_dev, tokens_dev, bytes, hipMemcpyDeviceToDevice, e->stream)); return VITX_OK; }
  HIPCHK(hipMemcpyAsync(s0.ba[0].x_in, tokens_dev, bytes, hipMemcpyDeviceToDevice, e->stream));
  int rc;
  const float drop = training ? c.dropout : 0.f;
  for (int l = 0; l < s0.depth; ++l)
    if ((rc = block_forward(e, s0, 0, l, b, n, 0, nullptr, drop, seed, err)) != VITX_OK) return rc;
  HIPCHK(hipMemcpyAsync(out_dev, s0.ba[s0.depth - 1].x_out, bytes, hipMemcpyDeviceToDevice, e->stream));
  e->have_fwd = false;
  e->have_tf = true; e->tf_b = b; e->tf_n = n; e->tf_drop = drop; e->tf_seed = seed;
  e->last_training = 0;
  return VITX_OK;
}

int engine_transformer_backward(vitx_engine* e, const float* dout_dev, float* dtokens_dev, std::string& err) {
  const vitx_config& c = e->cfg;
  if (!e->have_tf) { err = "transformer_backward requires a preceding transformer_forward"; return VITX_ERR_STATE; }
  const int b = e->tf_b, n = e->tf_n, d = c.dim, T = e->bf16;
  Stage& s0 = e->stages[0];
  const size_t bytes = (size_t)b * n * d * 4;
  { Prof pr(e, "fill_zero", 0, (double)e->n_arena * 4); launch_fill_zero(e->grads, (int64_t)e->n_arena * 4, e->stream); }
  launch_fill_zero(e->g, (int64_t)round_up((int64_t)b * n, 256) * d * 4, e->stream);
  HIPCHK(hipMemcpyAsync(e->g, dout_dev, bytes, hipMemcpyDeviceToDevice, e->stream));
  if (T) launch_convert(e->g, d, e->g_lp, 1, d, b * n, d, d, e->stream);
  int rc;
  SideScope side_scope(e, true);
  e->dbr_ready = 0;
  for (int l = s0.depth - 1; l >= 0; --l)
    if ((rc = block_backward(e, s0, 0, l, b, n, 0, e->tf_drop, e->tf_seed, err, l - 1)) != VITX_OK) return rc;
  if (dtokens_dev) HIPCHK(hipMemcpyAsync(dtokens_dev, e->g, bytes, hipMemcpyDeviceToDevice, e->stream));
  return VITX_OK;
}

int engine_patch_tokens_forward(vitx_engine* e, const float* img_dev, int b, int H, int W, float* tokens_dev, float* patches_f32_dev,
                                std::string& err) {
  const vitx_config& c = e->cfg;
  if (c.variant == VITX_VARIANT_CAIT || c.variant == VITX_VARIANT_PATCH_MERGER) { err = "patch_tokens_forward: ViT / DeepViT only"; return VITX_ERR_UNSUPPORTED; }
  if (c.small_dataset) { err = "patch_tokens_forward: not for small_dataset handles"; return VITX_ERR_UNSUPPORTED; }
  if (c.cct_block) { err = "patch_tokens_forward: not for cct_block handles"; return VITX_ERR_UNSUPPORTED; }
  if (c.nest_block) { err = "patch_tokens_forward: not for nest_block handles"; return VITX_ERR_UNSUPPORTED; }
  if (b <= 0 || b > c.max_batch) { err = "batch must be in [1, max_batch]"; return VITX_ERR_INVALID; }
  if (H <= 0 || W <= 0 || H > c.image_h || W > c.image_w || H % c.patch_h || W % c.patch_w) {
// ... 61 lines not shown
    Stage& s1 = e->stages[1];
    x_last = s1.depth > 0 ? s1.ba[s1.depth - 1].x_out : e->pooled;
    head_tok = 1;
  } else {
    x_last = s0.depth > 0 ? s0.ba[s0.depth - 1].x_out : e->tmp_f32;
    head_tok = ntok;
    if (merging) {
      head_tok = e->merge_t;
      if (e->merge_after == s0.depth - 1) x_last = e->pm_out;
      if (T) {
        const int64_t r0 = (int64_t)b * e->merge_t, r1 = round_up(r0, 64);
        if (r1 > r0) {
          HIPCHK(hipMemsetAsync(boff(e->g_lp, r0 * d, 2), 0, (size_t)(r1 - r0) * d * 2, e->stream));
          HIPCHK(hipMemsetAsync(boff(e->d_br, r0 * d, 2), 0, (size_t)(r1 - r0) * d * 2, e->stream));
          HIPCHK(hipMemsetAsync(boff(e->d_qkv, r0 * 3 * e->inner, 2), 0, (size_t)(r1 - r0) * 3 * e->inner * 2, e->stream));
          HIPCHK(hipMemsetAsync(boff(e->d_o, r0 * e->inner, 2), 0, (size_t)(r1 - r0) * e->inner * 2, e->stream));
        }
      }
    }
  }
  (void)s_last;
  {
    Prof pr(e, "head_prep", 0, 0);
    launch_colsum(e->dlogits, 0, e->nc_k, b, nc, e->red_ws, e->grads + e->head.b, e->stream);
    if (T) launch_convert(e->dlogits, e->nc_k, e->dl_lp, 1, e->nc_k, b, nc, e->nc_k, e->stream);
  }
  const void* dlT = T ? e->dl_lp : (const void*)e->dlogits;
  {
    EpiParams ep; ep.out = e->dyh; ep.ldo = d;
    dense_dgrad(e, dlT, e->nc_k, b, e->head, EPI_STORE, ep);
  }
  dense_wgrad(e, e->yh, d, dlT, e->nc_k, b, e->head);
  const bool mean_pool = !cait && c.pool == VITX_POOL_MEAN;
  const int head_rows = b * head_tok;
  { Prof pr(e, "fill_zero", 0, (double)head_rows * d * 4); launch_fill_zero(e->g, (int64_t)round_up(head_rows, 256) * d * 4, e->stream); }
  {
    Prof pr(e, "layernorm_bwd", 0, 0);
    if (mean_pool) {
      launch_layernorm_bwd(e->dyh, T, d, e->pooled, d, e->mean_h, e->rstd_h, e->params + e->head_g, nullptr, 0, e->dpooled, d, nullptr, 0,
                           e->red_ws, e->grads + e->head_g, e->grads + e->head_b, nullptr, b, d, e->stream);
      launch_mean_pool_bwd(e->dpooled, b, head_tok - extra, d, e->g, e->stream, head_tok);
    } else {
      const int64_t ldrow = (int64_t)head_tok * d;
      launch_layernorm_bwd(e->dyh, T, d, x_last, ldrow, e->mean_h, e->rstd_h, e->params + e->head_g, nullptr, 0, e->g, ldrow, nullptr, 0,
                           e->red_ws, e->grads + e->head_g, e->grads + e->head_b, nullptr, b, d, e->stream);
    }
    if (extra && d_distill_dev)
      HIPCHK(hipMemcpy2DAsync(e->g + (int64_t)(ntok - 1) * d, (size_t)ntok * d * 4, d_distill_dev, (size_t)d * 4, (size_t)d * 4, b, hipMemcpyDeviceToDevice, e->stream));
    if (T) launch_convert(e->g, d, e->g_lp, 1, d, head_rows, d, d, e->stream);
  }
  report_ready(e, e->head_g, e->n_arena - e->head_g);

  int rc;
  e->dbr_ready = 0;
  auto next_kept = [&](int si, int l) {
    for (int j = l - 1; j >= 0; --j) if (e->layer_kept[(size_t)si][(size_t)j]) return j;
    return -1;
  };
  if (cait) {
    Stage& s1 = e->stages[1];
    launch_fill_zero(e->g_ctx, (int64_t)b * np * d * 4, e->stream);
    for (int l = s1.depth - 1; l >= 0; --l) {
      if (e->layer_kept[1][(size_t)l]) {
        if ((rc = block_backward(e, s1, 1, l, b, 1, np, drop, e->last_seed, err, next_kept(1, l))) != VITX_OK) return rc;
      } else {
#ifndef VITX_COMM_LEGACY_ORDER
        report_ready(e, s1.bp[(size_t)l].p_begin, s1.bp[(size_t)l].p_end - s1.bp[(size_t)l].p_begin);
#endif
      }
    }
    {
      Prof pr(e, "embed_bwd", 0, 0);
      launch_batch_reduce(e->g, b, 1, d, 0, 1, e->grads + e->cls, e->stream);
      HIPCHK(hipMemcpyAsync(e->g, e->g_ctx, (size_t)b * np * d * 4, hipMemcpyDeviceToDevice, e->stream));
      if (T) launch_convert(e->g, d, e->g_lp, 1, d, b * np, d, d, e->stream);
    }
  }
  for (int l = s0.depth - 1; l >= 0; --l) {
    if (merging && l == e->merge_after && (rc = merger_backward(e, s0.ba[l].x_out, b, ntok, err)) != VITX_OK) return rc;
    const int rows_tok = (merging && l > e->merge_after) ? e->merge_t : ntok;
    if (e->layer_kept[0][(size_t)l]) {
      if ((rc = block_backward(e, s0, 0, l, b, rows_tok, 0, drop, e->last_seed, err, merging ? -1 : next_kept(0, l))) != VITX_OK) return rc;
    } else {
#ifndef VITX_COMM_LEGACY_ORDER
      report_ready(e, s0.bp[(size_t)l].p_begin, s0.bp[(size_t)l].p_end - s0.bp[(size_t)l].p_begin);
#endif
    }
  }
  if (e->last_training && c.emb_dropout > 0.f) {
    Prof pr(e, "dropout", 0, 0);
    launch_dropout(e->g, 0, (int64_t)b * ntok * d, c.emb_dropout, e->last_seed, 0u, e->stream);
  }

  const int tok_off = no_cls ? 0 : 1;
  {
    Prof pr(e, "embed_bwd", 0, 0);
    launch_extract_rows(e->g, b, ntok, tok_off, np, d, e->d_y, T, d, e->stream);
  }
  dense_wgrad(e, e->patches, e->pd_k, e->d_y, d, b * np, e->patch);
  {
    Prof pr(e, "embed_bwd", 0, (double)b * ntok * d * 4);
    launch_batch_reduce(e->g, b, ntok, d, 0, ntok - extra, e->grads + e->pos, e->stream);
    if (extra && d_token_out_dev) launch_batch_reduce(e->g, b, ntok, d, ntok - 1, 1, d_token_out_dev, e->stream);
    if (!no_cls) launch_batch_reduce(e->g, b, ntok, d, 0, 1, e->grads + e->cls, e->stream);
    launch_sum_rows(e->grads + e->pos + (int64_t)tok_off * d, np, d, e->grads + e->patch.b, e->stream);
  }
  if (c.small_dataset) {
    EpiParams ep; ep.out = e->tmp_f32; ep.ldo = e->pd;
    dense_dgrad(e, e->d_y, d, b * np, e->patch, EPI_STORE_F32, ep);
    Prof pr(e, "spt_bwd", 0, (double)b * np * e->pd * 8);
    launch_spt_bwd(e->spt_img, e->tmp_f32, e->pd, e->spt_mean, e->spt_rstd, e->params + e->spt_g, e->spt_ws, e->grads + e->spt_g, e->grads + e->spt_b,
                   dimg_dev != nullptr, b, e->last_H, e->last_W, c.channels, c.patch_h, e->stream);
    if (dimg_dev) launch_spt_dimg(e->tmp_f32, e->pd, dimg_dev, b, e->last_H, e->last_W, c.channels, c.patch_h, e->stream);
  } else if (dimg_dev) {
    EpiParams ep; ep.out = e->tmp_f32; ep.ldo = e->pd;
// ... 259 lines not shown
```

### vit-tensorflow_amd/csrc/env.hip

```cpp
#include "env.h"

#include <cstdio>
#include <cstdlib>
#include <cstring>
#include <mutex>
#include <set>
#include <string>

namespace {

const VitxEnvSwitch kSwitches[] = {
    {"VITX_GENERIC_GEMM", VITX_ENV_PATH, "1: every Dense on the k-ordered fp32-FMA kernel instead of the MFMA kernels"},
    {"VITX_GENERIC_ATTN", VITX_ENV_PATH, "1: materialised attention (batched products + row softmax) instead of the fused kernel"},
    {"VITX_DEEPVIT_FUSED", VITX_ENV_PATH, "0: DeepViT Re-attention forward as batched GEMMs + head-axis kernels instead of the one-kernel form"},
    {"VITX_DEEPVIT_FUSED_BWD", VITX_ENV_PATH, "0: DeepViT Re-attention backward as batched GEMMs + point / row kernels"},
    {"VITX_CAIT_FUSED", VITX_ENV_PATH, "0: CaiT talking-heads forward as batched GEMMs + chain kernel instead of the one-kernel form"},
    {"VITX_CAIT_QKV_CAT", VITX_ENV_PATH, "0: CaiT patch stage: to_q and to_kv as two Dense launches each way (rounds d(y1) twice)"},
    {"VITX_LN_SCALE_FUSED", VITX_ENV_PATH, "0: CaiT LayerScale VJP as a pass of its own instead of on the LayerNorm VJP (bias gradient from the bf16 rounding)"},
    {"VITX_CHAIN_MFMA", VITX_ENV_PATH, "0: talking-heads chain kernels with in-lane FMAs instead of the fp32 matrix pipe"},
    {"VITX_UNFUSED_HEADOPS", VITX_ENV_PATH, "1: head-axis operations (mix / softmax / LayerNorm over heads) as one kernel each"},
    {"VITX_WGRAD_TRANSPOSE", VITX_ENV_PATH, "1: weight gradients through explicit bf16 transposes + the NT kernel"},
    {"VITX_GELU_TABLE", VITX_ENV_PATH, "0: fc1 epilogue evaluates the degree-7 polynomial GELU instead of the LDS table (another rounding of gelu, both inside a bf16 ulp)"},
    {"VITX_X3_ATTN", VITX_ENV_PATH, "BF16X3 handles: 1 fused split-operand attention (default), 2 materialised scores + split-operand products, 0 exact fp32 products"},
    {"VITX_F32_MFMA", VITX_ENV_TUNING, "0: parity-mode GEMMs on the scalar-FMA kernel instead of the fp32 matrix pipe (same bits)"},
    {"VITX_GEMM_KERNEL", VITX_ENV_TUNING, "force one NT tile variant (1, 2, 3, 5, 6, 7, 9, 10, 11, 13; +256 direct / +512 LDS-staged epilogue); every variant adds in the same K order"},
    {"VITX_GEMM_TAIL_KERNEL", VITX_ENV_TUNING, "with VITX_GEMM_KERNEL=13 / 11: tile variant (1, 3, 10) of the tail launch (tail balancing)"},
    {"VITX_GEMM_TAIL", VITX_ENV_TUNING, "1: the per-shape measurement also times the tail-balanced forms (off by default: loses inside the step)"},
    {"VITX_GEMM_AUTOTUNE", VITX_ENV_TUNING, "0: static variant rule instead of the first-launch measurement"},
    {"VITX_GEMM_AUTOTUNE_LOG", VITX_ENV_TUNING, "1: print the measured variant choices"},
    {"VITX_GEMM_WALK", VITX_ENV_TUNING, "0: no XCD-owned row bands in the persistent NT kernel"},
    {"VITX_GEMM_GRID", VITX_ENV_TUNING, "n: persistent workgroups per launch (default 256)"},
    {"VITX_GEMM_PHASE", VITX_ENV_TUNING, "n: start-phase offsets between the persistent workgroups of an XCD (sleeps only)"},
    {"VITX_EPI_WIDE", VITX_ENV_TUNING, "0: 4-B instead of 16-B-per-lane epilogue accesses"},
    {"VITX_NT", VITX_ENV_TUNING, "bits: non-temporal stores (1 = gelu' of the fc1 epilogue, 16 = d(y) of the fc1 / qkv input gradients; default 17)"},
    {"VITX_REVERSE", VITX_ENV_TUNING, "bits: row tiles walked back to front for operands larger than the memory-side cache (1 forward, 2 input gradients)"},
    {"VITX_REVERSE_MIN_MB", VITX_ENV_TUNING, "operand size from which VITX_REVERSE applies"},
    {"VITX_MLP_BWD_ORDER", VITX_ENV_TUNING, "0: fc2 weight gradient between the producer and the consumers of d(hpre)"},
    {"VITX_BGEMM_PAIRS", VITX_ENV_TUNING, "0: the batched products of the materialised attention backward as four launches instead of two (same bits)"},
    {"VITX_ATTN_BWD_SPLIT", VITX_ENV_TUNING, "1: fused attention backward as two launches (same bits)"},
    {"VITX_GLP_SKIP", VITX_ENV_TUNING, "0: LayerNorm VJPs always write the bf16 copy of the residual gradient"},
    {"VITX_SCORE_BF16", VITX_ENV_TUNING, "0: DeepViT / CaiT score tensors that only batched products read stay fp32 planes (same bits)"},
    {"VITX_LN_CORESIDENT", VITX_ENV_TUNING, "1: LayerNorm VJP of 768-wide bf16 rows as 4-wave, 96-register blocks that fit beside a resident weight-gradient GEMM (experiment; partials summed in another order)"},
    {"VITX_LN_CO_BLOCKS", VITX_ENV_TUNING, "blocks of the co-resident LayerNorm VJP form (default 1024; 256 = one 4-wave block per CU, what fits beside a resident GEMM workgroup)"},
    {"VITX_SIDE_STREAM", VITX_ENV_TUNING, "0 one stream; 1 weight gradients on a lowest-priority side stream (default); 2 the same at the highest priority"},
    {"VITX_LN_REDUCE_SIDE_ROWS", VITX_ENV_TUNING, "LayerNorm VJPs of fewer rows keep their small reductions on the main stream (default 8192)"},
    {"VITX_SC_KEEP_MB", VITX_ENV_TUNING, "budget of the score tensors kept per block for the backward; blocks beyond it recompute (same bits)"},
    {"VITX_RECOMPUTE_SCORES", VITX_ENV_TUNING, "1: materialised attention recomputes its score tensors in the backward (same bits)"},
    {"VITX_WGRAD_WGS", VITX_ENV_TUNING, "workgroups per weight-gradient launch (default 128 up to 24576 token rows, else 256); changes the split-K slice count: fixed-order sums in another order"},
    {"VITX_SG_BLOCKS", VITX_ENV_TUNING, "blocks per LayerScale-gradient launch"},
    {"VITX_DV_CPI", VITX_ENV_TUNING, "chunks per image of the DeepViT one-kernel forward (tests: the multi-tile loop at small batches)"},
    {"VITX_COMM_PRIORITY", VITX_ENV_TUNING, "priority of the communication stream: 1 highest (default), 0 default, -1 lowest"},
    {"VITX_COMM_TIMING", VITX_ENV_TUNING, "0: no event brackets around the collectives (every Dense launch behind a bucket then takes the one-tile form)"},
    {"VITX_COMM_WAIT_ON_CHAIN", VITX_ENV_TUNING, "1: the compute stream (not the communication stream) waits for the weight-gradient stream's share of a reported range"},
    {"VITX_COMM_STREAM_EARLY", VITX_ENV_TUNING, "0: the communication stream is created at vitx_comm_overlap instead of with the handle's other streams (A/B: it may then share a command-processor pipe with the compute stream)"},
    {"VITX_COMM_SHARED", VITX_ENV_TUNING, "1: the Dense launches behind a bucket take the one-tile-per-workgroup form for as long as its collective was measured to last (default 0: persistent grids throughout, faster with emulated collectives)"},
// ... 46 lines not shown
```

### vit-tensorflow_amd/csrc/gemm_bf16.hip

```cpp
#include <array>
#include <map>
#include <mutex>

#include "gemm_bf16_common.h"

static int g_allow_320 = 1;
static int g_shared_gpu = 0;
int gemm_bf16_pick(int M, int N);

namespace {

template <int BM, int BN, int WM, int WN, int MODE, bool LDS_EPI, int SCHED>
__global__ __launch_bounds__(WM * WN * 64) void gemm_bf16_nt_kernel(Bf16GemmArgs g, EpiParams ep, int tiles_m, int tiles_n,
                                                                    int kt_per_split) {
  constexpr int NW = WM * WN;
  constexpr int WTM = BM / WM, WTN = BN / WN;
  constexpr int MT = WTM / 32, NT = WTN / 32;
  constexpr int A_BYTES = BM * BK * 2, B_BYTES = BN * BK * 2, STAGE = A_BYTES + B_BYTES;
  constexpr int A_INSTR = BM / 8 / NW, B_INSTR = BN / 8 / NW;
  static_assert(BM % (8 * NW) == 0 && BN % (8 * NW) == 0, "tile rows must split evenly over the waves");
  extern __shared__ __attribute__((aligned(16))) char smem[];

  const int nwg = gridDim.x, bid = blockIdx.x;
  const int xcd = bid & 7, q8 = nwg >> 3, r8 = nwg & 7;
// ... 324 lines not shown
  int r0 = 0;
  if (!tail_split_plan(g, mode, g.kernel & 15, &r0)) { Bf16GemmArgs g1 = g; g1.tail = 0; dispatch_gemm_bf16(g1, ep, mode, s); return; }
  Bf16GemmArgs gm = g, gt = g;
  EpiParams em = ep, et = ep;
  gm.tail = gt.tail = 0;
  gm.M = em.M = r0;
  gt.M = et.M = g.M - r0;
  gt.kernel = g.tail;
  gt.A = g.A + (int64_t)r0 * g.lda;
  const int osz = (mode == EPI_BIAS_RESID) ? 4 : 2;
  auto adv = [](const void* p, int64_t bytes) -> void* { return p ? (void*)((char*)p + bytes) : nullptr; };
  et.out = adv(ep.out, (int64_t)r0 * ep.ldo * osz);
  et.out2 = adv(ep.out2, (int64_t)r0 * ep.ldo2 * 2);
  et.resid = (const float*)adv(ep.resid, (int64_t)r0 * ep.ldr * 4);
  et.aux = adv(ep.aux, (int64_t)r0 * ep.ldaux * 2);
  const int main_cs_rows = (g.kernel & 15) == 11 ? 2 * (r0 / 320) : 2 * (r0 / 256);
  et.colsum = ep.colsum ? ep.colsum + (int64_t)main_cs_rows * ep.ldcs : nullptr;
  if (g.reverse_m) { dispatch_gemm_bf16(gt, et, mode, s); dispatch_gemm_bf16(gm, em, mode, s); }
  else { dispatch_gemm_bf16(gm, em, mode, s); dispatch_gemm_bf16(gt, et, mode, s); }
}

static std::mutex g_tune_mu;
static std::map<std::array<int64_t, 6>, int> g_tuned;
static int tail_enabled() {
  static int on = -1;
  if (on < 0) { const char* v = vitx_env("VITX_GEMM_TAIL"); on = (v && atoi(v) != 0) ? 1 : 0; }
  return on;
}
static int autotune_enabled() {
  static int on = -1;
  if (on < 0) { const char* v = vitx_env("VITX_GEMM_AUTOTUNE"); on = (v && atoi(v) == 0) ? 0 : 1; }
  return on;
}
void launch_gemm_bf16(const Bf16GemmArgs& g0, const EpiParams& ep, int mode, hipStream_t s) {
  const bool few_tiles = ceil_div(g0.M, 256) * ceil_div(g0.N, 256) < 512;
  const double work = (double)g0.M * g0.N * g0.K;
  const bool tunable = g0.kernel == 0 && autotune_enabled() && (g0.N % 256 == 0 || g0.N > 512) && (work >= 2.0e9 || (few_tiles && work >= 1.0e8)) &&
                       !(mode == EPI_BIAS_RESID && ep.out == (void*)ep.resid);
  if (!tunable) { dispatch_gemm_bf16_tail(g0, ep, mode, s); return; }
  const std::array<int64_t, 6> key = {mode, g0.M, g0.N, g0.K, g0.split_k > 1 ? g0.split_k : 1, (ep.scale != nullptr) + 2 * (g_shared_gpu | (g0.shared_gpu != 0))};
  int best = -1;
  {
    std::lock_guard<std::mutex> lk(g_tune_mu);
    auto it = g_tuned.find(key);
    if (it != g_tuned.end()) best = it->second;
  }
  Bf16GemmArgs g = g0;
  if (best < 0) {
    static const int cand[] = {13, 2, 11, 5, 3, 1};
    const bool small_m = ceil_div(g0.M, 256) * ceil_div(g0.N, 256) < 512;
    constexpr int NREP = 5;
    hipEvent_t ev[NREP + 1];
    for (auto& x : ev) (void)hipEventCreate(&x);
    float best_ms = 1e30f;
    best = gemm_bf16_pick(g0.M, g0.N);
    auto measure = [&](int c, int tail) {
      g.kernel = c; g.tail = tail;
      dispatch_gemm_bf16_tail(g, ep, mode, s);
      (void)hipEventRecord(ev[0], s);
      for (int r = 0; r < NREP; ++r) {
        dispatch_gemm_bf16_tail(g, ep, mode, s);
        (void)hipEventRecord(ev[r + 1], s);
      }
      if (hipEventSynchronize(ev[NREP]) != hipSuccess) return;
      float fastest = 1e30f;
      for (int r = 0; r < NREP; ++r) {
// ... 38 lines not shown
```

### vit-tensorflow_amd/csrc/gemm_bf16_pipe.hip

```cpp
#include "gemm_bf16_common.h"

#include <cmath>
#include <cstring>
#include <map>
#include <mutex>
#include <vector>

namespace {

__device__ __forceinline__ int wp_lane() {
  int l;
  asm volatile("v_mbcnt_lo_u32_b32 %0, -1, 0\n\tv_mbcnt_hi_u32_b32 %0, -1, %0" : "=v"(l));
  return l;
}

template <int POL>
__device__ __forceinline__ void wp_store16(bf16_t* base, uint32_t elem_off, bf16x8 v) {
  if constexpr (POL == 1) __builtin_nontemporal_store(v, (bf16x8*)(base + elem_off));
  else *(bf16x8*)(base + elem_off) = v;
}

constexpr int GT_LO = (127 - 12) << 7, GT_NE = ((127 + 3) << 7) - GT_LO, GT_BYTES = 2 * GT_NE * 4;
const uint32_t* gelu_table_dev() {
  static std::mutex mu;
  static std::map<int, const uint32_t*> per_dev;
  int dev = 0;
  (void)hipGetDevice(&dev);
  std::lock_guard<std::mutex> lk(mu);
  auto it = per_dev.find(dev);
  if (it != per_dev.end()) return it->second;
  std::vector<uint32_t> h((size_t)2 * GT_NE);
  auto f32_to_bf16 = [](float f) { uint32_t u; memcpy(&u, &f, 4); u += 0x7fffu + ((u >> 16) & 1u); return (uint16_t)(u >> 16); };
  auto f32_to_f16 = [](float f) { _Float16 hh = (_Float16)f; uint16_t u; memcpy(&u, &hh, 2); return u; };
  for (int sgn = 0; sgn < 2; ++sgn)
    for (int t = 0; t < GT_NE; ++t) {
      const uint32_t bits = ((uint32_t)sgn << 31) | ((uint32_t)(t + GT_LO) << 16);
      float xf; memcpy(&xf, &bits, 4);
      const double x = xf, phi = 0.5 * (1.0 + erf(x * 0.70710678118654752440)), gd = phi + x * 0.39894228040143267794 * exp(-0.5 * x * x);
      h[(size_t)sgn * GT_NE + t] = ((uint32_t)f32_to_f16((float)phi) << 16) | f32_to_bf16((float)gd);
    }
  uint32_t* d = nullptr;
  if (hipMalloc((void**)&d, GT_BYTES) != hipSuccess || hipMemcpy(d, h.data(), GT_BYTES, hipMemcpyHostToDevice) != hipSuccess) d = nullptr;
  per_dev[dev] = d;
  return d;
}

template <int BM, int BN, int WM, int WN, int MODE>
__global__ __launch_bounds__(WM * WN * 64, 2) void gemm_bf16_nt_pipe_kernel(Bf16GemmArgs g, EpiParams ep, int tiles_m, int tiles_n,
                                                                         int kt_per_split, const uint32_t* __restrict__ gelu_tab) {
  constexpr int NW = WM * WN;
  constexpr int WTM = BM / WM, WTN = BN / WN;
  constexpr int MT = WTM / 32, NT = WTN / 32;
  constexpr int A_BYTES = BM * BK * 2, B_BYTES = BN * BK * 2, STAGE = A_BYTES + B_BYTES;
  constexpr int A_INSTR = BM / 8 / NW, B_INSTR = BN / 8 / NW;
  static_assert(BM % (8 * NW) == 0 && BN % (8 * NW) == 0, "tile rows must split evenly over the waves");
  static_assert(BN == 256 || BN == 128, "256-column tiles (8 waves) or 128-column tiles (4 waves, two workgroups per CU)");
  extern __shared__ __attribute__((aligned(16))) char smem[];

  const int nwg = gridDim.x, bid = blockIdx.x;
  const int xcd = bid & 7, q8 = nwg >> 3, r8 = nwg & 7;
  const int logical0 = (xcd < r8 ? xcd * (q8 + 1) : r8 * (q8 + 1) + (xcd - r8) * q8) + (bid >> 3);
  const int total_tiles = tiles_m * tiles_n;
  const bool xw = BM == 256 && g.walk == 2;
  const int w_r0 = xw ? (tiles_m * xcd) >> 3 : 0, w_nr = xw ? ((tiles_m * (xcd + 1)) >> 3) - w_r0 : tiles_m;
  const int w_first = xw ? (bid >> 3) : logical0, w_stride = xw ? (nwg >> 3) : nwg, w_limit = xw ? w_nr * tiles_n : total_tiles;
  if (w_first >= w_limit) return;
  const int z = blockIdx.y;
  const int kt0 = z * kt_per_split;
  const int nk = min(kt_per_split, g.K / BK - kt0);
  const bool persistent = gridDim.y == 1;

  const int tid = threadIdx.x, lane = tid & 63;
  const int wave = __builtin_amdgcn_readfirstlane(tid >> 6);
  const int wm = wave / WN, wn = wave - wm * WN;

  if (g.phase > 0 && persistent) {
    const int n = g.phase >= 100 ? ((bid >> 3) & 1) * (g.phase - 100) : ((bid >> 3) & 7) * g.phase;
// ... 425 lines not shown
    stamp(2);
    if (!has_next) break;
    __builtin_amdgcn_s_waitcnt(0xC07F);
    asm volatile("" ::: "memory");
    issue();
    load_frags(fa[0], fb[0], smem + (it & 1) * STAGE, 0);
    stamp(3);
  }
}

template <int BM, int BN, int WM, int WN, int MODE>
void launch_pipe(const Bf16GemmArgs& g, const EpiParams& ep, hipStream_t s, bool one_tile_per_wg = false) {
  constexpr int SMEM = 2 * (BM + BN) * BK * 2 + ((MODE == EPI_BIAS_GELU && BM == 256) ? GT_BYTES : 0);
  if (((int64_t)ceil_div(g.M, BM) * BM * g.lda + g.K) * 2 >= (1LL << 31) || ((int64_t)ceil_div(g.N, BN) * BN * g.ldb + g.K) * 2 >= (1LL << 31)) {
    launch_gemm_bf16_persistent_lockstep(BM, MODE, g, ep, s);
    return;
  }
  auto kern = gemm_bf16_nt_pipe_kernel<BM, BN, WM, WN, MODE>;
  vitx_set_max_smem((const void*)kern, SMEM);
  const int tiles_m = (int)ceil_div(g.M, BM), tiles_n = (int)ceil_div(g.N, BN);
  const int nk = g.K / BK;
  const int split = g.split_k > 1 ? g.split_k : 1;
  const int per = (int)ceil_div(nk, split);
  const int zs = (int)ceil_div(nk, per);
  static const int phase_env = [] { const char* v = vitx_env("VITX_GEMM_PHASE"); return v ? atoi(v) : 0; }();
  Bf16GemmArgs gp = g;
  if (gp.phase == 0) gp.phase = phase_env;
  static const int walk_env = [] { const char* v = vitx_env("VITX_GEMM_WALK"); return v ? atoi(v) : -1; }();
  static const int grid_cap = [] { const char* v = vitx_env("VITX_GEMM_GRID"); return v ? atoi(v) : 256 * (WM * WN == 4 ? 2 : 1); }();
  const unsigned gx = (zs == 1 && !gemm_bf16_shared_gpu() && !g.shared_gpu && !one_tile_per_wg) ? (unsigned)std::min(tiles_m * tiles_n, grid_cap) : (unsigned)(tiles_m * tiles_n);
  dim3 grid(gx, (unsigned)zs), block(WM * WN * 64);
  const bool walk2_ok = BM == 256 && zs == 1 && gx == (unsigned)grid_cap && (gx & 7) == 0 && gx < (unsigned)(tiles_m * tiles_n) && tiles_n >= 8 && tiles_m >= 64 && g.stagger != 8;
  gp.walk = (walk2_ok && walk_env != 0) ? 2 : 0;
  static const int gelu_table_on = [] { const char* v = vitx_env("VITX_GELU_TABLE"); return v ? atoi(v) : 1; }();
  const uint32_t* gtab = (MODE == EPI_BIAS_GELU && BM == 256 && gelu_table_on) ? gelu_table_dev() : nullptr;
  hipLaunchKernelGGL(kern, grid, block, SMEM, s, gp, ep, tiles_m, tiles_n, per, gtab);
}

template <int MODE>
void pipe_mode(int variant, const Bf16GemmArgs& g, const EpiParams& ep, hipStream_t s) {
  switch (variant) {
    case 9: launch_pipe<192, 128, 2, 2, MODE>(g, ep, s); break;
    case 10: launch_pipe<192, 128, 2, 2, MODE>(g, ep, s, true); break;
    case 11: launch_pipe<320, 256, 2, 4, MODE>(g, ep, s); break;
    default: launch_pipe<256, 256, 2, 4, MODE>(g, ep, s); break;
  }
}

}

void launch_gemm_bf16_pipe(int variant, int mode, const Bf16GemmArgs& g, const EpiParams& ep, hipStream_t s) {
  switch (mode) {
    case EPI_STORE: pipe_mode<EPI_STORE>(variant, g, ep, s); break;
    case EPI_STORE_F32: pipe_mode<EPI_STORE_F32>(variant, g, ep, s); break;
    case EPI_BIAS_GELU: pipe_mode<EPI_BIAS_GELU>(variant, g, ep, s); break;
    case EPI_BIAS_RESID: pipe_mode<EPI_BIAS_RESID>(variant, g, ep, s); break;
    case EPI_PATCH: pipe_mode<EPI_PATCH>(variant, g, ep, s); break;
    case EPI_GELU_BWD: pipe_mode<EPI_GELU_BWD>(variant, g, ep, s); break;
    case EPI_PARTIAL: pipe_mode<EPI_PARTIAL>(variant, g, ep, s); break;
    default: break;
  }
}
```

### vit-tensorflow_amd/csrc/kernels.h

```cpp
#pragma once
#include "common.h"
#include "epilogue.h"

struct GenericGemmArgs {
  const void* A = nullptr;
  const void* B = nullptr;
  int M = 0, N = 0, K = 0;
  int64_t sam = 0, sak = 1, sbk = 0, sbn = 1;
  int nb = 1, nh = 1;
  int64_t sAb = 0, sAh = 0, sBb = 0, sBh = 0;
  int k_last = 0;
  int x3 = 0;
};
void launch_gemm_generic(const GenericGemmArgs& g, const EpiParams& ep, int mode, int ta, int tb, int to, hipStream_t s);
bool gemm_f32_mfma_supported(const GenericGemmArgs& g, int ta, int tb, int to);
void launch_gemm_f32_mfma(const GenericGemmArgs& g, const EpiParams& ep, int mode, hipStream_t s);
void gemm_f32_mfma_read_env();
bool gemm_bf16x3_supported(const GenericGemmArgs& g, int ta, int tb, int to);
void launch_gemm_bf16x3(const GenericGemmArgs& g, const EpiParams& ep, int mode, hipStream_t s);

bool headchain_supported(int h, int nk);
int64_t headchain_ws_elems(int h);
void launch_cait_chain_fwd(const float* s0, const float* wpre, const float* wpost, float* a1_or_null, float* a2, int b, int h, int nq, int nk,
                           int64_t ld, hipStream_t s);
void launch_cait_chain_bwd(const float* s0, const float* a1, float* da_inout, const float* wpre, const float* wpost, float* ws, float* dwpre,
                           float* dwpost, int b, int h, int nq, int nk, int64_t ld, hipStream_t s, bf16_t* ds_lp = nullptr);
bool cait_chain_bwd_bf16_out_ok();
void launch_deepvit_chain_fwd(float* s0_inout, const float* wre, const float* gamma, const float* beta, float* mixed_or_null, float* a2, int keep,
                              int b, int h, int nq, int nk, int64_t ld, float eps, hipStream_t s);
void launch_deepvit_chain_bwd(const float* a0, const float* mixed, float* da_inout, const float* wre, const float* gamma, float* ws, float* dwre,
                              float* dgamma, float* dbeta, int b, int h, int nq, int nk, int64_t ld, float eps, hipStream_t s);

bool bgemm_mfma_supported(const GenericGemmArgs& g, int ta, int tb, int to, int mode);
void launch_bgemm_mfma(const GenericGemmArgs& g, const EpiParams& ep, int ta, int to, hipStream_t s);
void launch_bgemm_mfma_pair(const GenericGemmArgs& g1, const EpiParams& ep1, int ta1, int to1, const GenericGemmArgs& g2, const EpiParams& ep2, int ta2,
                            int to2, hipStream_t s);

struct Bf16GemmArgs {
  const bf16_t* A = nullptr;
  const bf16_t* B = nullptr;
  int64_t lda = 0, ldb = 0;
  int M = 0, N = 0, K = 0;
  int split_k = 1;
  int kernel = 0;
  unsigned long long* stamps = nullptr;
  int phase = 0;
  int reverse_m = 0;
  int shared_gpu = 0;
  int walk = 0;
  int stagger = 0;
  int tail = 0;
};
void launch_gemm_bf16(const Bf16GemmArgs& g, const EpiParams& ep, int mode, hipStream_t s);
int gemm_bf16_tile_m(int kernel, int M, int N);
int gemm_bf16_tile_n(int kernel, int M, int N);
int gemm_bf16_num_slices(int K, int split_k);
void gemm_bf16_set_shared_gpu(int on);
void gemm_bf16_allow_320(int on);
void launch_gemm_bf16_tn(const Bf16GemmArgs& g, const EpiParams& ep, hipStream_t s);
int gemm_bf16_tn_tile(int kernel, int M, int N);

bool attn_bf16_supported(int n, int dim_head);
void launch_attn_bf16_fwd(const bf16_t* qkv, bf16_t* o, float* lse, int b, int n, int h, float scale, const bf16_t* zero_page, int reverse,
                          hipStream_t s);
bool attn_x3_supported(int n, int dim_head);
void launch_attn_x3_fwd(const float* qkv, float* o, float* lse, int b, int n, int h, float scale, hipStream_t s);
void launch_attn_x3_bwd(const float* qkv, const float* o, const float* d_o, const float* lse, float* dqkv, int b, int n, int h, float scale, hipStream_t s);
void launch_attn_bf16_bwd(const bf16_t* qkv, const bf16_t* o, const bf16_t* d_o, const float* lse, float* dsum_ws,
                          bf16_t* dqkv, int b, int n, int h, float scale, const bf16_t* zero_page, hipStream_t s);

constexpr int LSA_N_MAX = 288;
bool attn_lsa_supported(int n, int dim_head);
int64_t attn_lsa_ws_elems(int b, int n, int h);
void launch_attn_lsa_fwd(const void* qkv, void* o, float* lse, int is_bf16, int b, int n, int h, int dim_head, const float* temperature, hipStream_t s);
void launch_attn_lsa_bwd(const void* qkv, const void* o, const void* d_o, const float* lse, float* dsum_ws, void* dqkv, int is_bf16, int b, int n, int h,
                         int dim_head, const float* temperature, float* dtemperature, float* part_ws, hipStream_t s);
bool attn_small_supported(int n, int dim_head);
void launch_attn_small_fwd(const void* qkv, void* o, float* lse, int is_bf16, int b, int n, int h, int dim_head, float scale, hipStream_t s);
void launch_attn_small_bwd(const void* qkv, const void* o, const void* d_o, const float* lse, float* dsum_ws, void* dqkv, int is_bf16, int b, int n, int h,
                           int dim_head, float scale, hipStream_t s);

void launch_spt_fwd(const float* img, void* rows, int rows_bf16, int64_t ldo, float* mean, float* rstd, const float* gamma, const float* beta, int b,
                    int H, int W, int C, int p, float eps, hipStream_t s);
int64_t spt_bwd_ws_elems(int feat);
void launch_spt_bwd(const float* img, float* d_rows, int64_t ld, const float* mean, const float* rstd, const float* gamma, float* ws, float* dgamma,
                    float* dbeta, int want_dx, int b, int H, int W, int C, int p, hipStream_t s);
void launch_spt_dimg(const float* dx, int64_t ld, float* dimg, int b, int H, int W, int C, int p, hipStream_t s);

void launch_cct_im2col(const float* x, float* rows, int b, int H, int W, int C, int k, int st, int Kp, hipStream_t s);
void launch_cct_relu_maxpool_fwd(const float* conv, float* out, int b, int H, int W, int C, int k, int st, hipStream_t s);
void launch_cct_relu_maxpool_bwd(const float* conv, const float* dout, float* dconv, int b, int H, int W, int C, int k, int st, hipStream_t s);

void launch_nest_to_blocks(const float* x, const float* pos, float* tokens, int b, int nb, int hb, int wb, int c, hipStream_t s);
void launch_nest_from_blocks(const float* tokens, float* x, int b, int nb, int hb, int wb, int c, hipStream_t s);
void launch_nest_dpos(const float* dtokens, float* part, float* dpos, int nseq, int n, int c, hipStream_t s);
void launch_nest_maxpool_fwd(const float* x, float* out, int b, int H, int W, int C, int k, int st, hipStream_t s);
void launch_nest_maxpool_bwd(const float* x, const float* dout, float* dx, int b, int H, int W, int C, int k, int st, hipStream_t s);

void launch_unfold(const float* img, void* out, int out_bf16, int b, int H, int W, int C, int ph, int pw,
                   int64_t ldo, hipStream_t s);
void launch_fold_add(const float* dpatches, int64_t ld, float* dimg, int b, int H, int W, int C, int ph, int pw, hipStream_t s);
void extract_patches_geometry(int H, int W, int k, int st, int* oh, int* ow, int* pad_top, int* pad_left);
void launch_extract_patches(const float* x, float* out, int b, int H, int W, int C, int k, int st, hipStream_t s);
void launch_extract_patches_bwd(const float* dout, float* dx, int b, int H, int W, int C, int k, int st, hipStream_t s);
void launch_cls_pos_row(float* x, const float* cls, const float* pos, int b, int ntok, int d, int64_t ldx, hipStream_t s);
void launch_layernorm_fwd(const float* x, int64_t ldx, const float* gamma, const float* beta, void* y, int y_bf16,
                          int64_t ldy, float* mean, float* rstd, int rows, int d, float eps, hipStream_t s);
void launch_layernorm_bwd(const void* dy, int dy_bf16, int64_t lddy, const float* x, int64_t ldx, const float* mean,
                          const float* rstd, const float* gamma, const float* g_in, int64_t ldgi, float* g_out, int64_t ldgo,
                          void* g_lp, int64_t ldglp, float* partial_ws, float* dgamma, float* dbeta, float* gsum, int rows, int d,
                          hipStream_t s, int* deferred = nullptr);
void launch_layernorm_bwd_reduce(float* partial_ws, int nparts, int d, float* dgamma, float* dbeta, float* gsum, hipStream_t s);
int64_t layernorm_bwd_ws_elems(int d);
bool layernorm_bwd_scale_ok(int d);
void launch_layernorm_bwd_scale(const bf16_t* dy, int64_t lddy, const float* x, int64_t ldx, const float* mean, const float* rstd, const float* gamma,
                                const float* g_in, int64_t ldgi, float* g_out, int64_t ldgo, bf16_t* dbr, int64_t lddbr, const bf16_t* nf, int64_t ldnf,
                                const float* nscale, float* partial_ws, int rows, int d, hipStream_t s, int* nparts);
void launch_layernorm_bwd_scale_reduce(float* partial_ws, int nparts, int d, float* dgamma, float* dbeta, float* dscale, float* dbias, const float* nscale,
                                       hipStream_t s);
void launch_colsum(const void* x, int is_bf16, int64_t ld, int rows, int cols, float* partial_ws, float* out, hipStream_t s);
int64_t colsum_ws_elems(int cols);
void launch_reduce_partials(const float* partial, int nparts, int64_t stride, int64_t n, float* out, float alpha, hipStream_t s);
void launch_reduce_partials3(const float* partial, int nparts, int64_t stride, int64_t seg, int nseg, float* out0, float* out1, float* out2,
                             float* ws2, float alpha, hipStream_t s);
void launch_convert_weight(const float* w, int in, int out, bf16_t* wn, int64_t ldwn, bf16_t* wt, int64_t ldwt, hipStream_t s);
struct ConvertDesc { const float* w; bf16_t* wn; bf16_t* wt; int64_t ldwn, ldwt; int in, out, tiles_x, block0; };
void launch_convert_weights_batched(const ConvertDesc* descs_dev, int n, int total_blocks, hipStream_t s);
void launch_transpose_bf16(const bf16_t* in, int64_t ldi, int rows, int cols, bf16_t* out, int64_t ldo, hipStream_t s);
void launch_convert(const float* in, int64_t ldi, void* out, int out_bf16, int64_t ldo, int rows, int cols, int64_t out_cols_zero_to,
                    hipStream_t s);
void launch_to_f32(const void* in, int in_bf16, int64_t ldi, float* out, int64_t ldo, int rows, int cols, hipStream_t s);
void launch_set_token_row(float* x, const float* tok, int b, int ntok, int row, int d, hipStream_t s);
void launch_mean_pool(const float* x, int b, int ntok, int d, float* out, hipStream_t s, int stride_tok = 0);
void launch_mean_pool_bwd(const float* dp, int b, int ntok, int d, float* g, hipStream_t s, int stride_tok = 0);
void launch_batch_reduce(const float* g, int b, int ntok, int d, int j0, int nj, float* out, hipStream_t s);
void launch_extract_rows(const float* g, int b, int ntok, int tok_off, int np, int d, void* out, int out_bf16, int64_t ldo, hipStream_t s);
void launch_sum_rows(const float* in, int rows, int d, float* out, hipStream_t s);
void launch_ce_grad(const float* logits, int64_t ld, const int32_t* labels, int b, int nc, float inv_batch, float* dlogits,
                    float* loss, hipStream_t s);
void launch_adamw(float* p, const float* g, float* m, float* v, int64_t n, float lr, float b1, float b2, float eps, float wd, int step, hipStream_t s);
void launch_sgd(float* p, const float* g, float* m, int64_t n, float lr, float mom, float wd, hipStream_t s);
void launch_fill_zero(void* p, int64_t bytes, hipStream_t s);
void launch_fill_random_bf16(bf16_t* p, int64_t n, uint32_t seed, float scale, hipStream_t s);
void launch_max_rel_diff(const void* a, const void* b, int is_bf16, int64_t rows, int cols, int64_t lda, int64_t ldb, float* out_max, hipStream_t s);
void launch_dropout(void* x, int is_bf16, int64_t n, float rate, uint64_t seed, uint32_t site, hipStream_t s);
void launch_axpy_resid(const float* resid, const float* f, const float* scale, float* out, void* keep, int keep_bf16, int64_t rows, int d,
                       hipStream_t s);
void launch_branch_grad(const float* g, const float* scale, void* out, int out_bf16, int64_t rows, int d, float rate, uint64_t seed,
                        uint32_t site, hipStream_t s);
void launch_resid_add(const float* resid, const void* t, int t_bf16, float* out, int64_t n, hipStream_t s);

void launch_softmax_rows(float* sc, int64_t rows, int n, int64_t ld, hipStream_t s);
void launch_softmax_bwd_rows(const float* p, float* dp_inout, int64_t rows, int n, int64_t ld, hipStream_t s);
int64_t deepvit_point_bwd_ws_elems(int h);
void launch_deepvit_point_bwd(const float* a0, float* da_inout, const float* w, const float* gamma, float* ws, float* dw,
                              float* dgamma, float* dbeta, int b, int h, int nq, int nk, int64_t ld, float eps, hipStream_t s);
bool deepvit_attn_fused_supported(int h, int dim_head, int nq, int nk);
bool cait_attn_fused_supported(int h, int dim_head, int nq, int nk);
void launch_cait_attn_fwd(const bf16_t* q, const bf16_t* k, const bf16_t* v, int64_t ldq, int64_t ldk, int64_t ldv, int64_t qb, int64_t kb, int64_t vb,
                          bf16_t* o, int64_t ldo, int64_t ob, const float* wpre, const float* wpost, float* s0_keep, float* a1_keep, float* a2_keep,
                          int keep, int b, int h, int nq, int nk, int64_t ld, float scale, const bf16_t* zero_page, hipStream_t s);
int64_t deepvit_attn_bwd_ws_elems(int b, int h, int nq);
void launch_deepvit_attn_bwd(const bf16_t* q, const bf16_t* k, const bf16_t* v, int64_t ldq, int64_t ldk, int64_t ldv, int64_t qb, int64_t kb, int64_t vb,
                             const bf16_t* d_o, int64_t ldo, int64_t ob, const float* p_keep, const float* w, const float* gamma, float* ds_out,
                             bf16_t* dq, int64_t lddq, int64_t dqb, float* ws, float* dw, float* dgamma, float* dbeta, int b, int h, int nq, int nk,
// ... 47 lines not shown
```

Measured before the change: 7281 images/sec.

## Compute last ViT block only on class-token rows for cls-pooled models

```diff
diff --git a/vit-tensorflow_amd/csrc/attn_bf16.hip b/vit-tensorflow_amd/csrc/attn_bf16.hip
--- a/vit-tensorflow_amd/csrc/attn_bf16.hip
+++ b/vit-tensorflow_amd/csrc/attn_bf16.hip
@@ -133,7 +133,8 @@
 
 template <int NTP>
 __global__ __launch_bounds__(ATT_THREADS, 4) void attn_fwd_kernel(const bf16_t* __restrict__ qkv, bf16_t* __restrict__ o, float* __restrict__ lse,
-                                                       int n, int h, float scale, const bf16_t* __restrict__ zero_page, int reverse, int planar) {
+                                                       int n, int h, float scale, const bf16_t* __restrict__ zero_page, int reverse, int planar,
+                                                       int nq_live) {
   constexpr int NKP = 16 * NTP, QB = QB_FWD;
   extern __shared__ __attribute__((aligned(16))) char smem[];
   char* k_rm = smem;
@@ -149,7 +150,7 @@
   stage_head_dma(qbase + 2 * L.kv_off, tok_stride, n, NKP, v_rm, zero_page, wave, lane, nwaves);
 
   const int qi = lane & 15, g = lane >> 4;
-  const int nqb = (n + 16 * QB - 1) / (16 * QB);
+  const int nqb = (nq_live + 16 * QB - 1) / (16 * QB);
   const float sl2 = scale * 1.44269504088896340736f;
   bf16x8 qf[QB][2];
   auto load_q = [&](int qb) {
@@ -201,8 +202,8 @@
       ls += __shfl_xor(ls, 16, 64);
       ls += __shfl_xor(ls, 32, 64);
       const float inv_l = 1.0f / ls;
-      if (g == 0 && q < n) lse[(int64_t)bh * n + q] = (m[s] + log2f(ls)) * 0.69314718055994530942f;
-      if (q < n) {
+      if (g == 0 && q < nq_live) lse[(int64_t)bh * n + q] = (m[s] + log2f(ls)) * 0.69314718055994530942f;
+      if (q < nq_live) {
         bf16_t* op = o + L.o0 + (int64_t)q * L.o_stride;
 #pragma unroll
         for (int c = 0; c < 4; ++c) {
@@ -273,7 +274,7 @@
 
 template <int NTP>
 __device__ __forceinline__ float dq_block(const char* k_rm, const char* v_rm, const DqOperands& x, int64_t tok_stride, bf16_t* dq_rows, int qb, int lane,
-                                          int n, float scale, float lse2) {
+                                          int n, float scale, float lse2, int nq_live) {
   const int qi = lane & 15, g = lane >> 4;
   const int q = qb * 16 + qi;
   const float sl2 = scale * 1.44269504088896340736f;
@@ -294,7 +295,7 @@
 #pragma unroll 1
   for (int u = 0; u < u_full; ++u) dq_pair<false>(k_rm, v_rm, u, qi, g, lane, n, qf, dof, sl2, lse2, scale, nds, dq);
   if (u_full < u_end) dq_pair<true>(k_rm, v_rm, u_full, qi, g, lane, n, qf, dof, sl2, lse2, scale, nds, dq);
-  if (q < n) {
+  if (q < nq_live) {
     bf16_t* out = dq_rows + (int64_t)q * tok_stride;
 #pragma unroll
     for (int c = 0; c < 4; ++c) {
@@ -303,6 +304,13 @@
       for (int r = 0; r < 4; ++r) ov[r] = (bf16_t)dq[c][r];
       *(bf16x4*)(out + 16 * c + 4 * g) = ov;
     }
+  } else if (q < n) {
+    bf16_t* out = dq_rows + (int64_t)q * tok_stride;
+    bf16x4 z;
+#pragma unroll
+    for (int r = 0; r < 4; ++r) z[r] = (bf16_t)0.f;
+#pragma unroll
+    for (int c = 0; c < 4; ++c) *(bf16x4*)(out + 16 * c + 4 * g) = z;
   }
   return dsum;
 }
@@ -319,7 +327,7 @@
 
 template <int NTP>
 __device__ __forceinline__ void dkv_block(const char* q_rm, const char* do_rm, const float* lse_s, const float* d_s, const DkvOperands& x,
-                                          int64_t tok_stride, int64_t inner, bf16_t* dk_rows, int kb, int lane, int n, float scale) {
+                                          int64_t tok_stride, int64_t inner, bf16_t* dk_rows, int kb, int lane, int n, float scale, int nq) {
   const int ki = lane & 15, g = lane >> 4;
   const int key = kb * 16 + ki;
   const float sl2 = scale * 1.44269504088896340736f;
@@ -328,7 +336,7 @@
   f32x4 dk[4], dv[4];
 #pragma unroll
   for (int c = 0; c < 4; ++c) { dk[c] = f32x4{0.f, 0.f, 0.f, 0.f}; dv[c] = f32x4{0.f, 0.f, 0.f, 0.f}; }
-  const int u_end = min(NTP / 2, (n + 31) >> 5);
+  const int u_end = min(NTP / 2, (nq + 31) >> 5);
 #pragma unroll 1
   for (int u = 0; u < u_end; ++u) {
     f32x4 pp[2], ds[2];
@@ -374,11 +382,16 @@
   }
 }
 
+__device__ __forceinline__ void dq_zero_dead_blocks(bf16_t* dq_rows, int64_t tok_stride, int nblk_live, int n, int tid, int nthreads) {
+  for (int idx = tid; idx < (n - 16 * nblk_live) * 8; idx += nthreads)
+    *(bf16x8*)(dq_rows + (int64_t)(16 * nblk_live + (idx >> 3)) * tok_stride + (idx & 7) * 8) = zero8();
+}
+
 template <int NTP>
 __global__ __launch_bounds__(ATT_THREADS) void attn_bwd_dq_kernel(const bf16_t* __restrict__ qkv, const bf16_t* __restrict__ o,
                                                           const bf16_t* __restrict__ d_o, const float* __restrict__ lse,
                                                           float* __restrict__ dsum, bf16_t* __restrict__ dqkv, int n, int h, float scale,
-                                                          const bf16_t* __restrict__ zero_page) {
+                                                          const bf16_t* __restrict__ zero_page, int nq_live) {
   constexpr int NKP = 16 * NTP;
   extern __shared__ __attribute__((aligned(16))) char smem[];
   char* k_rm = smem;
@@ -394,20 +407,23 @@
   asm volatile("s_waitcnt vmcnt(0)" ::: "memory");
   __syncthreads();
   const int64_t orow0 = (int64_t)bi * n * inner + hi * DH;
-  for (int qb = wave; qb < (n + 15) / 16; qb += nwaves) {
+  const int nblk_live = (nq_live + 15) / 16;
+  for (int qb = wave; qb < nblk_live; qb += nwaves) {
     const int qi = lane & 15, q = qb * 16 + qi, qc = min(q, n - 1);
     DqOperands x;
     dq_load(x, qbase, tok_stride, o + orow0, d_o + orow0, inner, qb, lane, n);
     const float d = dq_block<NTP>(k_rm, v_rm, x, tok_stride, dqkv + (int64_t)bi * n * tok_stride + hi * DH, qb, lane, n, scale,
-                                  lse[(int64_t)bh * n + qc] * 1.44269504088896340736f);
-    if ((lane >> 4) == 0 && q < n) dsum[(int64_t)bh * n + q] = d;
-  }
+                                  lse[(int64_t)bh * n + qc] * 1.44269504088896340736f, nq_live);
+    if ((lane >> 4) == 0 && q < nq_live) dsum[(int64_t)bh * n + q] = d;
+  }
+  dq_zero_dead_blocks(dqkv + (int64_t)bi * n * tok_stride + hi * DH, tok_stride, nblk_live, n, tid, (int)blockDim.x);
 }
 
 template <int NTP>
 __global__ __launch_bounds__(ATT_THREADS) void attn_bwd_dkv_kernel(const bf16_t* __restrict__ qkv, const bf16_t* __restrict__ d_o,
                                                            const float* __restrict__ lse, const float* __restrict__ dsum,
-                                                           bf16_t* __restrict__ dqkv, int n, int h, float scale, const bf16_t* __restrict__ zero_page) {
+                                                           bf16_t* __restrict__ dqkv, int n, int h, float scale, const bf16_t* __restrict__ zero_page,
+                                                           int nq_live) {
   constexpr int NQP = 16 * NTP;
   extern __shared__ __attribute__((aligned(16))) char smem[];
   char* q_rm = smem;
@@ -420,18 +436,18 @@
   const bf16_t* qbase = qkv + (int64_t)bi * n * tok_stride + hi * DH;
   const int tid = threadIdx.x, lane = tid & 63, nwaves = blockDim.x >> 6;
   const int wave = __builtin_amdgcn_readfirstlane(tid >> 6);
-  stage_head_dma(qbase, tok_stride, n, NQP, q_rm, zero_page, wave, lane, nwaves);
-  stage_head_dma(d_o + (int64_t)bi * n * inner + hi * DH, inner, n, NQP, do_rm, zero_page, wave, lane, nwaves);
+  stage_head_dma(qbase, tok_stride, nq_live, NQP, q_rm, zero_page, wave, lane, nwaves);
+  stage_head_dma(d_o + (int64_t)bi * n * inner + hi * DH, inner, nq_live, NQP, do_rm, zero_page, wave, lane, nwaves);
   for (int i = tid; i < NQP; i += blockDim.x) {
-    lse_s[i] = i < n ? lse[(int64_t)bh * n + i] * 1.44269504088896340736f : 0.f;
-    d_s[i] = i < n ? dsum[(int64_t)bh * n + i] : 0.f;
+    lse_s[i] = i < nq_live ? lse[(int64_t)bh * n + i] * 1.44269504088896340736f : 0.f;
+    d_s[i] = i < nq_live ? dsum[(int64_t)bh * n + i] : 0.f;
   }
   asm volatile("s_waitcnt vmcnt(0)" ::: "memory");
   __syncthreads();
   for (int kb = wave; kb < (n + 15) / 16; kb += nwaves) {
     DkvOperands x;
     dkv_load(x, qbase + inner, tok_stride, inner, kb, lane, n);
-    dkv_block<NTP>(q_rm, do_rm, lse_s, d_s, x, tok_stride, inner, dqkv + (int64_t)bi * n * tok_stride + inner + hi * DH, kb, lane, n, scale);
+    dkv_block<NTP>(q_rm, do_rm, lse_s, d_s, x, tok_stride, inner, dqkv + (int64_t)bi * n * tok_stride + inner + hi * DH, kb, lane, n, scale, nq_live);
   }
 }
 
@@ -439,7 +455,7 @@
 __global__ __launch_bounds__(ATT_THREADS, 4) void attn_bwd_fused_kernel(const bf16_t* __restrict__ qkv, const bf16_t* __restrict__ o,
                                                              const bf16_t* __restrict__ d_o, const float* __restrict__ lse,
                                                              bf16_t* __restrict__ dqkv, int n, int h, float scale,
-                                                             const bf16_t* __restrict__ zero_page, int planar) {
+                                                             const bf16_t* __restrict__ zero_page, int planar, int nq_live) {
   constexpr int NKP = 16 * NTP, NQP = 16 * NTP;
   extern __shared__ __attribute__((aligned(16))) char smem[];
   char* k_rm = smem;
@@ -457,39 +473,41 @@
   stage_head_dma(qbase + inner, tok_stride, n, NKP, k_rm, zero_page, wave, lane, nwaves);
   stage_head_dma(qbase + 2 * inner, tok_stride, n, NKP, v_rm, zero_page, wave, lane, nwaves);
   for (int i = tid; i < NQP; i += blockDim.x) {
-    lse_s[i] = i < n ? lse[(int64_t)bh * n + i] * 1.44269504088896340736f : 0.f;
+    lse_s[i] = i < nq_live ? lse[(int64_t)bh * n + i] * 1.44269504088896340736f : 0.f;
     d_s[i] = 0.f;
   }
   const int64_t orow0 = L.o0;
   const int nblk = (n + 15) / 16;
+  const int nblk_live = (nq_live + 15) / 16;
   DqOperands xq;
-  if (wave < nblk) dq_load(xq, qbase, tok_stride, o + orow0, d_o + orow0, ostr, wave, lane, n);
+  if (wave < nblk_live) dq_load(xq, qbase, tok_stride, o + orow0, d_o + orow0, ostr, wave, lane, n);
   ATTN_STAMP(0);
   asm volatile("s_waitcnt vmcnt(0)" ::: "memory");
   __syncthreads();
   ATTN_STAMP(1);
-  for (int qb = wave; qb < nblk; qb += nwaves) {
+  for (int qb = wave; qb < nblk_live; qb += nwaves) {
     const int q = qb * 16 + (lane & 15);
     DqOperands nx;
-    if (qb + nwaves < nblk) dq_load(nx, qbase, tok_stride, o + orow0, d_o + orow0, ostr, qb + nwaves, lane, n);
-    const float d = dq_block<NTP>(k_rm, v_rm, xq, tok_stride, dqkv + L.q0, qb, lane, n, scale, lse_s[min(q, n - 1)]);
-    if ((lane >> 4) == 0 && q < n) d_s[q] = d;
+    if (qb + nwaves < nblk_live) dq_load(nx, qbase, tok_stride, o + orow0, d_o + orow0, ostr, qb + nwaves, lane, n);
+    const float d = dq_block<NTP>(k_rm, v_rm, xq, tok_stride, dqkv + L.q0, qb, lane, n, scale, lse_s[min(q, n - 1)], nq_live);
+    if ((lane >> 4) == 0 && q < nq_live) d_s[q] = d;
     xq = nx;
   }
+  dq_zero_dead_blocks(dqkv + L.q0, tok_stride, nblk_live, n, tid, (int)blockDim.x);
   DkvOperands xk;
   if (wave < nblk) dkv_load(xk, qbase + inner, tok_stride, inner, wave, lane, n);
   ATTN_STAMP(2);
   __syncthreads();
   ATTN_STAMP(3);
-  stage_head_dma(qbase, tok_stride, n, NQP, q_rm, zero_page, wave, lane, nwaves);
-  stage_head_dma(d_o + orow0, ostr, n, NQP, do_rm, zero_page, wave, lane, nwaves);
+  stage_head_dma(qbase, tok_stride, nq_live, NQP, q_rm, zero_page, wave, lane, nwaves);
+  stage_head_dma(d_o + orow0, ostr, nq_live, NQP, do_rm, zero_page, wave, lane, nwaves);
   asm volatile("s_waitcnt vmcnt(0)" ::: "memory");
   __syncthreads();
   ATTN_STAMP(4);
   for (int kb = wave; kb < nblk; kb += nwaves) {
     DkvOperands nx;
     if (kb + nwaves < nblk) dkv_load(nx, qbase + inner, tok_stride, inner, kb + nwaves, lane, n);
-    dkv_block<NTP>(q_rm, do_rm, lse_s, d_s, xk, tok_stride, inner, dqkv + L.q0 + inner, kb, lane, n, scale);
+    dkv_block<NTP>(q_rm, do_rm, lse_s, d_s, xk, tok_stride, inner, dqkv + L.q0 + inner, kb, lane, n, scale, nq_live);
     xk = nx;
   }
   ATTN_STAMP(5);
@@ -523,17 +541,20 @@
 
 int vitx_attn_probe_planar = 0;
 
-void launch_attn_bf16_fwd(const bf16_t* qkv, bf16_t* o, float* lse, int b, int n, int h, float scale, const bf16_t* zero_page, int reverse, hipStream_t s) {
+void launch_attn_bf16_fwd(const bf16_t* qkv, bf16_t* o, float* lse, int b, int n, int h, float scale, const bf16_t* zero_page, int reverse, hipStream_t s,
+                          int nq_live) {
+  if (nq_live <= 0 || nq_live > n) nq_live = n;
   const int ntp = pick_ntp(n);
   const int nkp = 16 * ntp;
   const int smem = 2 * nkp * ROWB;
-#define CALL(NTP) { set_smem(attn_fwd_kernel<NTP>, smem); hipLaunchKernelGGL(attn_fwd_kernel<NTP>, dim3(b * h), dim3(att_threads(n)), smem, s, qkv, o, lse, n, h, scale, zero_page, reverse, vitx_attn_probe_planar); }
+#define CALL(NTP) { set_smem(attn_fwd_kernel<NTP>, smem); hipLaunchKernelGGL(attn_fwd_kernel<NTP>, dim3(b * h), dim3(att_threads(n)), smem, s, qkv, o, lse, n, h, scale, zero_page, reverse, vitx_attn_probe_planar, nq_live); }
   VITX_NTP_DISPATCH(ntp, CALL);
 #undef CALL
 }
 
 void launch_attn_bf16_bwd(const bf16_t* qkv, const bf16_t* o, const bf16_t* d_o, const float* lse, float* dsum_ws, bf16_t* dqkv, int b,
-                          int n, int h, float scale, const bf16_t* zero_page, hipStream_t s) {
+                          int n, int h, float scale, const bf16_t* zero_page, hipStream_t s, int nq_live) {
+  if (nq_live <= 0 || nq_live > n) nq_live = n;
   const int ntp = pick_ntp(n);
   const int np = 16 * ntp;
   const int smem_dq = 2 * np * ROWB;
@@ -541,7 +562,7 @@
   const char* split_env = vitx_env("VITX_ATTN_BWD_SPLIT");
   const bool split = split_env && atoi(split_env) != 0;
   if (!split) {
-#define CALLF(NTP) { set_smem(attn_bwd_fused_kernel<NTP>, smem_dkv); hipLaunchKernelGGL(attn_bwd_fused_kernel<NTP>, dim3(b * h), dim3(att_threads(n)), smem_dkv, s, qkv, o, d_o, lse, dqkv, n, h, scale, zero_page, vitx_attn_probe_planar); }
+#define CALLF(NTP) { set_smem(attn_bwd_fused_kernel<NTP>, smem_dkv); hipLaunchKernelGGL(attn_bwd_fused_kernel<NTP>, dim3(b * h), dim3(att_threads(n)), smem_dkv, s, qkv, o, d_o, lse, dqkv, n, h, scale, zero_page, vitx_attn_probe_planar, nq_live); }
     VITX_NTP_DISPATCH(ntp, CALLF);
 #undef CALLF
     return;
@@ -550,8 +571,8 @@
   {                                                                                                                                \
     set_smem(attn_bwd_dq_kernel<NTP>, smem_dq);                                                                                    \
     set_smem(attn_bwd_dkv_kernel<NTP>, smem_dkv);                                                                                  \
-    hipLaunchKernelGGL(attn_bwd_dq_kernel<NTP>, dim3(b * h), dim3(att_threads(n)), smem_dq, s, qkv, o, d_o, lse, dsum_ws, dqkv, n, h, scale, zero_page);   \
-    hipLaunchKernelGGL(attn_bwd_dkv_kernel<NTP>, dim3(b * h), dim3(att_threads(n)), smem_dkv, s, qkv, d_o, lse, dsum_ws, dqkv, n, h, scale, zero_page);    \
+    hipLaunchKernelGGL(attn_bwd_dq_kernel<NTP>, dim3(b * h), dim3(att_threads(n)), smem_dq, s, qkv, o, d_o, lse, dsum_ws, dqkv, n, h, scale, zero_page, nq_live);   \
+    hipLaunchKernelGGL(attn_bwd_dkv_kernel<NTP>, dim3(b * h), dim3(att_threads(n)), smem_dkv, s, qkv, d_o, lse, dsum_ws, dqkv, n, h, scale, zero_page, nq_live);    \
   }
   VITX_NTP_DISPATCH(ntp, CALL);
 #undef CALL
diff --git a/vit-tensorflow_amd/csrc/capi.hip b/vit-tensorflow_amd/csrc/capi.hip
--- a/vit-tensorflow_amd/csrc/capi.hip
+++ b/vit-tensorflow_amd/csrc/capi.hip
@@ -795,6 +795,13 @@
   const void* src = nullptr;
   int64_t rows = 0, cols = 0, ld = 0;
   bool is_t = false;
+  if (w == "last_block_form") {
+    if (n_elems) *n_elems = 1;
+    if (!out_host) return VITX_OK;
+    if (cap < 1) return fail(VITX_ERR_INVALID, "output buffer too small");
+    out_host[0] = (h->have_fwd && h->last_cls_only) ? 1.f : 0.f;
+    return VITX_OK;
+  }
   if (w == "pooled_ln") { src = h->yh; rows = b; cols = ld = c.dim; is_t = true; }
   else if (w == "logits") { src = h->logits; rows = b; cols = c.num_classes; ld = h->nc_k; }
   else if (w == "dlogits") { src = h->dlogits; rows = b; cols = c.num_classes; ld = h->nc_k; }
@@ -803,6 +810,11 @@
     if (!st) return fail(VITX_ERR_INVALID, "layer out of range");
     if (c.variant == VITX_VARIANT_CAIT) { nq = st->nq_max == 1 ? 1 : h->last_np; nk = st->nq_max == 1 ? 1 + h->last_np : h->last_np; }
     BlockActs& ba = st->ba[(size_t)l];
+    if (h->last_cls_only && st == &h->stages[0] && l == st->depth - 1 && w != "x_in" && w != "embed" && w != "y1" && w != "qkv") {
+      std::string err;
+      const int rc = engine_complete_last_block(h, err);
+      if (rc != VITX_OK) return fail(rc, err);
+    }
     rows = (int64_t)b * nq;
     if (w == "x_in" || w == "embed") { src = ba.x_in; cols = ld = c.dim; }
     else if (w == "x_mid") { src = ba.x_mid; cols = ld = c.dim; }
diff --git a/vit-tensorflow_amd/csrc/elementwise.hip b/vit-tensorflow_amd/csrc/elementwise.hip
--- a/vit-tensorflow_amd/csrc/elementwise.hip
+++ b/vit-tensorflow_amd/csrc/elementwise.hip
@@ -472,6 +472,14 @@
   const int c = (int)(e - bi * d);
   x[(bi * ntok + row) * d + c] = tok[c];
 }
+__global__ void copy_rows_kernel(const uint4* __restrict__ src, int64_t src_stride, uint4* __restrict__ dst, int64_t dst_stride, int rows, int row_chunks) {
+  const int64_t total = (int64_t)rows * row_chunks;
+  for (int64_t e = (int64_t)blockIdx.x * blockDim.x + threadIdx.x; e < total; e += (int64_t)gridDim.x * blockDim.x) {
+    const int64_t r = e / row_chunks;
+    const int c = (int)(e - r * row_chunks);
+    dst[r * dst_stride + c] = src[r * src_stride + c];
+  }
+}
 __global__ void mean_pool_kernel(const float* __restrict__ x, int b, int ntok, int d, float* __restrict__ out, int stride_tok) {
   const int64_t total = (int64_t)b * d;
   for (int64_t e = (int64_t)blockIdx.x * blockDim.x + threadIdx.x; e < total; e += (int64_t)gridDim.x * blockDim.x) {
@@ -931,6 +939,12 @@
 }
 void launch_set_token_row(float* x, const float* tok, int b, int ntok, int row, int d, hipStream_t s) {
   hipLaunchKernelGGL(set_token_row_kernel, dim3((unsigned)ceil_div((int64_t)b * d, 256)), dim3(256), 0, s, x, tok, b, ntok, row, d);
+}
+void launch_copy_rows(const void* src, int64_t src_stride_bytes, void* dst, int64_t dst_stride_bytes, int rows, int row_bytes, hipStream_t s) {
+  const int64_t total = (int64_t)rows * (row_bytes / 16);
+  if (total == 0) return;
+  hipLaunchKernelGGL(copy_rows_kernel, dim3(grid_for(total)), dim3(256), 0, s, (const uint4*)src, src_stride_bytes / 16, (uint4*)dst, dst_stride_bytes / 16, rows,
+                     row_bytes / 16);
 }
 void launch_mean_pool(const float* x, int b, int ntok, int d, float* out, hipStream_t s, int stride_tok) {
   hipLaunchKernelGGL(mean_pool_kernel, dim3(grid_for((int64_t)b * d)), dim3(256), 0, s, x, b, ntok, d, out, stride_tok ? stride_tok : ntok);
diff --git a/vit-tensorflow_amd/csrc/engine.h b/vit-tensorflow_amd/csrc/engine.h
--- a/vit-tensorflow_amd/csrc/engine.h
+++ b/vit-tensorflow_amd/csrc/engine.h
@@ -71,6 +71,12 @@
   bool sc_no_mixed = false;
   bool sc_a2_bf16 = false;
   int par_first = 0, par_last = 0;
+};
+
+struct ClsRows {
+  void *o = nullptr, *y2 = nullptr, *hpre = nullptr, *act = nullptr;
+  float *x_mid = nullptr, *x_out = nullptr, *mean2 = nullptr, *rstd2 = nullptr;
+  void *g_lp = nullptr, *g_lp2 = nullptr, *d_h = nullptr, *d_y = nullptr, *d_o = nullptr;
 };
 
 struct Stage {
@@ -165,6 +171,10 @@
   float* distill_ws = nullptr;
   float *opt_m = nullptr, *opt_v = nullptr; int opt_step = 0;
   bf16_t *bench_a = nullptr, *bench_b = nullptr; float* bench_c = nullptr; int64_t bench_elems = 0;
+
+  ClsRows cr;
+  bool cls_rows_ok = false;
+  bool last_cls_only = false;
 
   bool have_fwd = false;
   bool have_tf = false;
@@ -237,6 +247,7 @@
                    std::string& err, const float* distill_token_dev = nullptr, float* distill_out_dev = nullptr);
 int engine_backward(vitx_engine* e, const float* dlogits_dev, float* dimg_dev, std::string& err, const float* d_distill_dev = nullptr,
                     float* d_token_out_dev = nullptr);
+int engine_complete_last_block(vitx_engine* e, std::string& err);
 int engine_transformer_forward(vitx_engine* e, const float* tokens_dev, int b, int n, int training, uint64_t seed, float* out_dev, std::string& err);
 int engine_transformer_backward(vitx_engine* e, const float* dout_dev, float* dtokens_dev, std::string& err);
 int engine_patch_tokens_forward(vitx_engine* e, const float* img_dev, int b, int H, int W, float* tokens_dev, float* patches_f32_dev_or_null,
diff --git a/vit-tensorflow_amd/csrc/engine.hip b/vit-tensorflow_amd/csrc/engine.hip
--- a/vit-tensorflow_amd/csrc/engine.hip
+++ b/vit-tensorflow_amd/csrc/engine.hip
@@ -896,8 +896,70 @@
   return e->x3 && e->x3_attn && e->x3_fused_attn && e->cfg.variant == VITX_VARIANT_VIT && !e->force_generic_attn && attn_x3_supported(n, e->cfg.dim_head);
 }
 
+static bool cls_rows_apply(const vitx_engine* e, int ntok, int extra, float drop) {
+  if (!e->cls_rows_ok || extra || drop > 0.f || !use_fused_attn(e, ntok)) return false;
+  return !vitx_env_flag("VITX_LAST_BLOCK_FULL");
+}
+static void cls_fc1_fwd(vitx_engine* e, const Dense& w, int b, int nq) {
+  ClsRows& cr = e->cr;
+  const int d = e->cfg.dim, m = e->cfg.mlp_dim;
+  const int shared = comm_busy(e);
+  const int64_t rows_full = (int64_t)b * nq;
+  int vfull = e->gemm_kernel & 15;
+  if (vfull == 0) vfull = gemm_bf16_variant_for(EPI_BIAS_GELU, (int)rows_full, w.out, w.in_k, 0, shared);
+  int ntab = 0;
+  if (vfull == 13 && gemm_bf16_gelu_table_active()) ntab = (int)std::min<int64_t>(b, ceil_div(rows_full / 256 * 256, nq));
+  auto launch = [&](int r0, int rows, int kernel) {
+    EpiParams ep;
+    ep.out = boff(cr.hpre, (int64_t)r0 * m, 2); ep.ldo = m; ep.out2 = boff(cr.act, (int64_t)r0 * m, 2); ep.ldo2 = m;
+    ep.nt_out = e->nt_mask & 1;
+    ep.M = rows; ep.N = w.out; ep.bias = dense_b(e, w); ep.zero_pad = 1;
+    finalize_epi(ep);
+    Bf16GemmArgs g;
+    g.A = (const bf16_t*)cr.y2 + (int64_t)r0 * d; g.lda = d;
+    g.B = w.wt; g.ldb = w.in_k;
+    g.M = rows; g.N = w.out; g.K = w.in_k; g.kernel = kernel; g.shared_gpu = shared;
+    char shape[48];
+    if (e->profiling) snprintf(shape, sizeof shape, "shape nt e%d %dx%dx%d", (int)EPI_BIAS_GELU, g.M, g.N, g.K);
+    Prof pr(e, "gemm_bf16_mfma", 2.0 * rows * (double)w.out * w.in, dense_launch_bytes(e, EPI_BIAS_GELU, ep, rows, w.in, w.out), e->profiling ? shape : nullptr);
+    launch_gemm_bf16(g, ep, EPI_BIAS_GELU, e->stream);
+  };
+  const int mpad = (int)round_up(ntab, 256);
+  if (ntab > 0) launch(0, mpad, 13);
+  if (ntab < b) launch(ntab, b - ntab, 1);
+  if (mpad > b) {
+    launch_fill_zero(boff(cr.hpre, (int64_t)b * m, 2), (int64_t)(mpad - b) * m * 2, e->stream);
+    launch_fill_zero(boff(cr.act, (int64_t)b * m, 2), (int64_t)(mpad - b) * m * 2, e->stream);
+  }
+}
+
+static void block_forward_cls_rows(vitx_engine* e, const BlockParams& bp, const BlockActs& ba, int b, int nq) {
+  const vitx_config& c = e->cfg;
+  const int d = c.dim, inner = e->inner, m = c.mlp_dim;
+  ClsRows& cr = e->cr;
+  {
+    Prof pr(e, "cls_rows", 0, (double)b * inner * 4);
+    launch_copy_rows(ba.o, (int64_t)nq * inner * 2, cr.o, (int64_t)inner * 2, b, inner * 2, e->stream);
+  }
+  {
+    EpiParams ep;
+    ep.out = cr.x_mid; ep.ldo = d; ep.resid = ba.x_in; ep.ldr = (int64_t)nq * d;
+    dense_fwd(e, cr.o, inner, b, bp.out, EPI_BIAS_RESID, ep);
+  }
+  {
+    Prof pr(e, "layernorm_fwd", 0, (double)b * d * 6);
+    launch_layernorm_fwd(cr.x_mid, d, e->params + bp.ln2_g, e->params + bp.ln2_b, cr.y2, 1, d, cr.mean2, cr.rstd2, b, d, c.ln_eps, e->stream);
+  }
+  cls_fc1_fwd(e, bp.fc1, b, nq);
+  {
+    EpiParams ep;
+    ep.out = cr.x_out; ep.ldo = d; ep.resid = cr.x_mid; ep.ldr = d;
+    dense_fwd(e, cr.act, m, b, bp.fc2, EPI_BIAS_RESID, ep);
+  }
+}
+
 static int block_forward(vitx_engine* e, Stage& st, int si, int l, int b, int nq, int nc, const float* context, float drop, uint64_t seed,
-                         std::string& err) {
+                         std::string& err, bool cls_rows = false) {
   const uint32_t site0 = (uint32_t)((si * 1000 + l) * 4);
   const BlockParams& bp = st.bp[l];
   BlockActs& ba = st.ba[l];
@@ -951,8 +1013,10 @@
     Prof pr(e, "attn_x3_fwd", 4.0 * b * c.heads * (double)nq * nq * c.dim_head, (double)rows * inner * 4 * esz);
     launch_attn_x3_fwd((const float*)ba.qkv, (float*)ba.o, ba.lse, b, nq, c.heads, 1.0f / std::sqrt((float)c.dim_head), e->stream);
   } else if (use_fused_attn(e, nq)) {
-    Prof pr(e, "attn_bf16_fwd", 4.0 * b * c.heads * (double)nq * nq * c.dim_head, (double)rows * inner * 4 * esz);
-    launch_attn_bf16_fwd((const bf16_t*)ba.qkv, (bf16_t*)ba.o, ba.lse, b, nq, c.heads, 1.0f / std::sqrt((float)c.dim_head), (const bf16_t*)e->zero_page, (e->reverse_mask >> 2) & 1, e->stream);
+    const double live = cls_rows ? 1.0 / nq : 1.0;
+    Prof pr(e, "attn_bf16_fwd", 4.0 * b * c.heads * (double)nq * nq * c.dim_head * live, (double)rows * inner * (2 + 2 * live) * esz);
+    launch_attn_bf16_fwd((const bf16_t*)ba.qkv, (bf16_t*)ba.o, ba.lse, b, nq, c.heads, 1.0f / std::sqrt((float)c.dim_head), (const bf16_t*)e->zero_page, (e->reverse_mask >> 2) & 1, e->stream,
+                         cls_rows ? 1 : 0);
   } else {
     const int need = c.variant == VITX_VARIANT_VIT ? 1 : 3;
     if (e->keep_scores && ba.sc_keep_elems == 0) {
@@ -973,6 +1037,10 @@
       if (rc != VITX_OK) return rc;
     }
     attn_generic_fwd(e, bp, av, b, keep ? &ba : nullptr);
+  }
+  if (cls_rows) {
+    block_forward_cls_rows(e, bp, ba, b, nq);
+    return VITX_OK;
   }
   if (bp.has_out && drop > 0.f) {
     EpiParams ep; ep.out = e->tmp_f32; ep.ldo = d;
@@ -1032,8 +1100,54 @@
   return VITX_OK;
 }
 
+static void block_backward_cls_rows(vitx_engine* e, const BlockParams& bp, int b, int nq) {
+  const vitx_config& c = e->cfg;
+  const int d = c.dim, inner = e->inner, m = c.mlp_dim;
+  ClsRows& cr = e->cr;
+  {
+    Prof pr(e, "cls_rows", 0, (double)b * d * 6);
+    launch_extract_rows(e->g, b, nq, 0, 1, d, cr.g_lp, 1, d, e->stream);
+  }
+  const bool fc1_bias_fused = !(e->gemm_kernel & 256) && bp.fc1.b >= 0;
+  const int cs_rows = (int)ceil_div(b, 96);
+  {
+    EpiParams ep; ep.out = cr.d_h; ep.ldo = m; ep.aux = cr.hpre; ep.ldaux = m;
+    if (fc1_bias_fused) {
+      launch_fill_zero(e->red_ws, (int64_t)cs_rows * m * 4, e->stream);
+      ep.colsum = e->red_ws; ep.ldcs = m;
+    }
+    dense_dgrad(e, cr.g_lp, d, b, bp.fc2, EPI_GELU_BWD, ep);
+    if (fc1_bias_fused) {
+      Prof pr(e, "reduce_partials", 0, (double)(cs_rows + 1) * m * 4);
+      launch_reduce_partials3(e->red_ws, cs_rows, m, m, 1, e->grads + bp.fc1.b, nullptr, nullptr, e->red_ws + (int64_t)cs_rows * m, 1.0f, e->stream);
+    }
+  }
+  {
+    EpiParams ep; ep.out = cr.d_y; ep.ldo = d;
+    dense_dgrad(e, cr.d_h, m, b, bp.fc1, EPI_STORE, ep);
+  }
+  dense_wgrad(e, cr.y2, d, cr.d_h, m, b, bp.fc1);
+  if (!fc1_bias_fused) bias_grad(e, cr.d_h, 1, m, b, bp.fc1);
+  dense_wgrad(e, cr.act, m, cr.g_lp, d, b, bp.fc2);
+  {
+    Prof pr(e, "layernorm_bwd", 0, (double)b * d * 16);
+    launch_layernorm_bwd(cr.d_y, 1, d, cr.x_mid, d, cr.mean2, cr.rstd2, e->params + bp.ln2_g, e->g, (int64_t)nq * d, e->g, (int64_t)nq * d, cr.g_lp2, d,
+                         e->red_ws, e->grads + bp.ln2_g, e->grads + bp.ln2_b, dense_gb(e, bp.fc2), b, d, e->stream);
+  }
+  {
+    EpiParams ep; ep.out = cr.d_o; ep.ldo = inner;
+    dense_dgrad(e, cr.g_lp2, d, b, bp.out, EPI_STORE, ep);
+  }
+  dense_wgrad(e, cr.o, inner, cr.g_lp2, d, b, bp.out);
+  {
+    Prof pr(e, "cls_rows", 0, (double)b * inner * 4);
+    launch_copy_rows(cr.d_o, (int64_t)inner * 2, e->d_o, (int64_t)nq * inner * 2, b, inner * 2, e->stream);
+  }
+}
+
 static inline int64_t branch_key(int si, int l, int mlp) { return (((int64_t)si + 1) << 32) | ((int64_t)l << 1) | mlp; }
-static int block_backward(vitx_engine* e, Stage& st, int si, int l, int b, int nq, int nc, float drop, uint64_t seed, std::string& err, int next_l = -1) {
+static int block_backward(vitx_engine* e, Stage& st, int si, int l, int b, int nq, int nc, float drop, uint64_t seed, std::string& err, int next_l = -1,
+                          bool cls_rows = false) {
   const uint32_t site0 = (uint32_t)((si * 1000 + l) * 4);
   const BlockParams& bp = st.bp[l];
   BlockActs& ba = st.ba[l];
@@ -1058,7 +1172,9 @@
   const void* dbranch = gT;
   bool fc2_bias_done = false, out_bias_done = false;
   const int64_t key_mlp = branch_key(si, l, 1), key_attn = branch_key(si, l, 0);
-  if (!ba.skip_mlp) {
+  if (cls_rows) {
+    block_backward_cls_rows(e, bp, b, nq);
+  } else if (!ba.skip_mlp) {
   if (e->dbr_ready == key_mlp) {
     e->dbr_ready = 0;
     dbranch = e->d_br;
@@ -1160,7 +1276,10 @@
   }
   bool out_bias_in_ln = false;
   const void* d_o = dbranch;
-  if (bp.has_out) {
+  if (cls_rows) {
+    out_bias_in_ln = true;
+    d_o = e->d_o;
+  } else if (bp.has_out) {
     EpiParams ep; ep.out = e->d_o; ep.ldo = inner;
     const hipEvent_t fork_out = side_prefork(e);
     dense_dgrad(e, dbranch, d, rows, bp.out, EPI_STORE, ep);
@@ -1239,9 +1358,10 @@
       launch_attn_x3_bwd((const float*)ba.qkv, (const float*)ba.o, (const float*)d_o, ba.lse, (float*)e->d_qkv, b, nq, c.heads,
                          1.0f / std::sqrt((float)c.dim_head), e->stream);
     } else if (use_fused_attn(e, nq)) {
-      Prof pr(e, "attn_bf16_bwd", 14.0 * b * c.heads * (double)nq * nq * c.dim_head, (double)rows * inner * 8 * esz);
+      const double live = cls_rows ? 1.0 / nq : 1.0;
+      Prof pr(e, "attn_bf16_bwd", 14.0 * b * c.heads * (double)nq * nq * c.dim_head * live, (double)rows * inner * (5 + 3 * live) * esz);
       launch_attn_bf16_bwd((const bf16_t*)ba.qkv, (const bf16_t*)ba.o, (const bf16_t*)d_o, ba.lse, e->dsum, (bf16_t*)e->d_qkv, b, nq,
-                           c.heads, 1.0f / std::sqrt((float)c.dim_head), (const bf16_t*)e->zero_page, e->stream);
+                           c.heads, 1.0f / std::sqrt((float)c.dim_head), (const bf16_t*)e->zero_page, e->stream, cls_rows ? 1 : 0);
     } else {
       int rc = ensure_scores(e, 4, (int64_t)b * c.heads * nq * round_up(nk, 4), err);
       if (rc != VITX_OK) return rc;
@@ -1597,6 +1717,24 @@
     if ((rc = ring(e->rg_cs, e->cs_part, cs_bytes, 4)) != VITX_OK) return rc;
   }
   DALLOC(e->dsum, (size_t)B * c.heads * e->ntok_cap * 4 + 16, false);
+  e->cls_rows_ok = e->bf16 && c.variant == VITX_VARIANT_VIT && c.pool == VITX_POOL_CLS && nbranch == 1 && !c.small_dataset && !c.cct_block && !c.nest_block &&
+                   c.depth > 0 && e->stages[0].bp.back().has_out && !e->force_generic_gemm && !e->wgrad_via_transpose;
+  if (e->cls_rows_ok) {
+    ClsRows& cr = e->cr;
+    DALLOC(cr.o, (size_t)e->bp * inner * 2, true);
+    DALLOC(cr.y2, (size_t)e->bp * d * 2, true);
+    DALLOC(cr.hpre, (size_t)e->bp * m * 2, true);
+    DALLOC(cr.act, (size_t)e->bp * m * 2, true);
+    DALLOC(cr.g_lp, (size_t)e->bp * d * 2, true);
+    DALLOC(cr.g_lp2, (size_t)e->bp * d * 2, true);
+    DALLOC(cr.d_h, (size_t)e->bp * m * 2, true);
+    DALLOC(cr.d_y, (size_t)e->bp * d * 2, true);
+    DALLOC(cr.d_o, (size_t)e->bp * inner * 2, true);
+    DALLOC(cr.x_mid, (size_t)e->bp * d * 4, false);
+    DALLOC(cr.x_out, (size_t)e->bp * d * 4, false);
+    DALLOC(cr.mean2, (size_t)e->bp * 4, false);
+    DALLOC(cr.rstd2, (size_t)e->bp * 4, false);
+  }
   if (c.small_dataset) {
     e->spt_g = find_param(e, "patch_embedding.norm.gamma");
     e->spt_b = find_param(e, "patch_embedding.norm.beta");
@@ -1806,6 +1944,7 @@
   const int np = (H / c.patch_h) * (W / c.patch_w);
   const int ntok = no_cls ? np : np + 1 + extra;
   const int d = c.dim, T = e->bf16;
+  e->last_cls_only = false;
   ensure_geometry(e, b, ntok);
   if (e->params_dirty) engine_refresh_weights(e);
   Stage& s0 = e->stages[0];
@@ -1841,6 +1980,7 @@
     launch_dropout(x0, 0, (int64_t)b * ntok * d, emb_drop, seed, 0u, e->stream);
   }
   draw_layer_dropout(e, seed);
+  const bool cls_rows = cls_rows_apply(e, ntok, extra, drop);
   int rc;
   for (int l = 0; l < s0.depth; ++l) {
     if (!e->layer_kept[0][(size_t)l]) {
@@ -1848,7 +1988,7 @@
       continue;
     }
     const bool merged = merger && e->merge_after >= 0 && l > e->merge_after;
-    if ((rc = block_forward(e, s0, 0, l, b, merged ? e->merge_t : ntok, 0, nullptr, drop, seed, err)) != VITX_OK) return rc;
+    if ((rc = block_forward(e, s0, 0, l, b, merged ? e->merge_t : ntok, 0, nullptr, drop, seed, err, cls_rows && l == s0.depth - 1)) != VITX_OK) return rc;
     if (merger && l == e->merge_after) merger_forward(e, s0.ba[l].x_out, b, ntok);
   }
   const float* x_last = s0.depth > 0 ? s0.ba[s0.depth - 1].x_out : x0;
@@ -1874,14 +2014,26 @@
     x_last = s1.depth > 0 ? s1.ba[s1.depth - 1].x_out : xc;
     head_tok = 1;
   }
+  if (cls_rows) {
+    x_last = e->cr.x_out;
+    head_tok = 1;
+  }
   if (extra && distill_out_dev)
     HIPCHK(hipMemcpy2DAsync(distill_out_dev, (size_t)d * 4, x_last + (int64_t)(ntok - 1) * d, (size_t)ntok * d * 4, (size_t)d * 4, b, hipMemcpyDeviceToDevice, e->stream));
   if ((rc = head_forward(e, x_last, b, head_tok, cait ? 0 : extra, logits_dev, err)) != VITX_OK) return rc;
   e->last_extra = extra;
+  e->last_cls_only = cls_rows;
   e->have_fwd = true;
   e->have_tf = false;
   e->last_b = b; e->last_np = np; e->last_ntok = ntok; e->last_H = H; e->last_W = W; e->last_training = training; e->last_seed = seed;
   return VITX_OK;
+}
+
+int engine_complete_last_block(vitx_engine* e, std::string& err) {
+  if (!e->have_fwd || !e->last_cls_only) return VITX_OK;
+  Stage& s0 = e->stages[0];
+  e->last_cls_only = false;
+  return block_forward(e, s0, 0, s0.depth - 1, e->last_b, e->last_ntok, 0, nullptr, 0.f, e->last_seed, err, false);
 }
 
 static int shell_check(const vitx_engine* e, std::string& err) {
@@ -1919,7 +2071,7 @@
   ep.out = tokens_dev; ep.ldo = d; ep.pos = e->params + e->pos; ep.ldr = d;
   ep.np = np; ep.ntok = ntok; ep.tok_off = 1;
   dense_fwd(e, e->patches, e->pd_k, b * np, e->patch, EPI_PATCH, ep);
-  e->have_fwd = false;
+  e->have_fwd = false; e->last_cls_only = false;
   e->have_embed = true;
   e->last_b = b; e->last_np = np; e->last_ntok = ntok; e->last_H = H; e->last_W = W; e->last_training = 0; e->last_extra = 0;
   return VITX_OK;
@@ -1944,7 +2096,7 @@
   EpiParams ep;
   ep.out = tokens_dev; ep.ldo = c.dim;
   dense_fwd(e, e->patches, e->pd_k, b * np, e->patch, EPI_STORE_F32, ep);
-  e->have_fwd = false; e->have_embed = false;
+  e->have_fwd = false; e->last_cls_only = false; e->have_embed = false;
   return VITX_OK;
 }
 
@@ -1958,7 +2110,7 @@
   EpiParams ep;
   ep.out = out_dev; ep.ldo = c.dim;
   dense_fwd(e, e->patches, e->pd_k, rows, e->patch, EPI_STORE_F32, ep);
-  e->have_fwd = false; e->have_embed = false;
+  e->have_fwd = false; e->last_cls_only = false; e->have_embed = false;
   return VITX_OK;
 }
 
@@ -1966,7 +2118,7 @@
   const vitx_config& c = e->cfg;
   int rc;
   if (b <= 0 || b > c.max_batch || n <= 0 || n > e->ntok_cap) { err = "head_forward: b or n out of range"; return VITX_ERR_INVALID; }
-  e->have_fwd = false;
+  e->have_fwd = false; e->last_cls_only = false;
   const int d = c.dim;
   if (e->params_dirty) engine_refresh_weights(e);
   if (!e->shell_x) DALLOC(e->shell_x, (size_t)e->mp * d * 4, false);
@@ -2062,7 +2214,7 @@
   for (int l = 0; l < s0.depth; ++l)
     if ((rc = block_forward(e, s0, 0, l, b, n, 0, nullptr, drop, seed, err)) != VITX_OK) return rc;
   HIPCHK(hipMemcpyAsync(out_dev, s0.ba[s0.depth - 1].x_out, bytes, hipMemcpyDeviceToDevice, e->stream));
-  e->have_fwd = false;
+  e->have_fwd = false; e->last_cls_only = false;
   e->have_tf = true; e->tf_b = b; e->tf_n = n; e->tf_drop = drop; e->tf_seed = seed;
   e->last_training = 0;
   return VITX_OK;
@@ -2190,6 +2342,7 @@
   }
   dense_wgrad(e, e->yh, d, dlT, e->nc_k, b, e->head);
   const bool mean_pool = !cait && c.pool == VITX_POOL_MEAN;
+  const bool cls_rows = e->last_cls_only;
   const int head_rows = b * head_tok;
   { Prof pr(e, "fill_zero", 0, (double)head_rows * d * 4); launch_fill_zero(e->g, (int64_t)round_up(head_rows, 256) * d * 4, e->stream); }
   {
@@ -2200,12 +2353,12 @@
       launch_mean_pool_bwd(e->dpooled, b, head_tok - extra, d, e->g, e->stream, head_tok);
     } else {
       const int64_t ldrow = (int64_t)head_tok * d;
-      launch_layernorm_bwd(e->dyh, T, d, x_last, ldrow, e->mean_h, e->rstd_h, e->params + e->head_g, nullptr, 0, e->g, ldrow, nullptr, 0,
-                           e->red_ws, e->grads + e->head_g, e->grads + e->head_b, nullptr, b, d, e->stream);
+      launch_layernorm_bwd(e->dyh, T, d, cls_rows ? e->cr.x_out : x_last, cls_rows ? (int64_t)d : ldrow, e->mean_h, e->rstd_h, e->params + e->head_g, nullptr, 0,
+                           e->g, ldrow, nullptr, 0, e->red_ws, e->grads + e->head_g, e->grads + e->head_b, nullptr, b, d, e->stream);
     }
     if (extra && d_distill_dev)
       HIPCHK(hipMemcpy2DAsync(e->g + (int64_t)(ntok - 1) * d, (size_t)ntok * d * 4, d_distill_dev, (size_t)d * 4, (size_t)d * 4, b, hipMemcpyDeviceToDevice, e->stream));
-    if (T) launch_convert(e->g, d, e->g_lp, 1, d, head_rows, d, d, e->stream);
+    if (T && !cls_rows) launch_convert(e->g, d, e->g_lp, 1, d, head_rows, d, d, e->stream);
   }
   report_ready(e, e->head_g, e->n_arena - e->head_g);
 
@@ -2238,7 +2391,8 @@
     if (merging && l == e->merge_after && (rc = merger_backward(e, s0.ba[l].x_out, b, ntok, err)) != VITX_OK) return rc;
     const int rows_tok = (merging && l > e->merge_after) ? e->merge_t : ntok;
     if (e->layer_kept[0][(size_t)l]) {
-      if ((rc = block_backward(e, s0, 0, l, b, rows_tok, 0, drop, e->last_seed, err, merging ? -1 : next_kept(0, l))) != VITX_OK) return rc;
+      if ((rc = block_backward(e, s0, 0, l, b, rows_tok, 0, drop, e->last_seed, err, merging ? -1 : next_kept(0, l), cls_rows && l == s0.depth - 1)) != VITX_OK)
+        return rc;
     } else {
 #ifndef VITX_COMM_LEGACY_ORDER
       report_ready(e, s0.bp[(size_t)l].p_begin, s0.bp[(size_t)l].p_end - s0.bp[(size_t)l].p_begin);
diff --git a/vit-tensorflow_amd/csrc/env.hip b/vit-tensorflow_amd/csrc/env.hip
--- a/vit-tensorflow_amd/csrc/env.hip
+++ b/vit-tensorflow_amd/csrc/env.hip
@@ -21,6 +21,7 @@
     {"VITX_UNFUSED_HEADOPS", VITX_ENV_PATH, "1: head-axis operations (mix / softmax / LayerNorm over heads) as one kernel each"},
     {"VITX_WGRAD_TRANSPOSE", VITX_ENV_PATH, "1: weight gradients through explicit bf16 transposes + the NT kernel"},
     {"VITX_GELU_TABLE", VITX_ENV_PATH, "0: fc1 epilogue evaluates the degree-7 polynomial GELU instead of the LDS table (another rounding of gelu, both inside a bf16 ulp)"},
+    {"VITX_LAST_BLOCK_FULL", VITX_ENV_PATH, "1: the last block of a cls-pooled bf16 ViT on every token row instead of the class rows only (same logits; eight of its parameter gradients sum in another order); read per forward"},
     {"VITX_X3_ATTN", VITX_ENV_PATH, "BF16X3 handles: 1 fused split-operand attention (default), 2 materialised scores + split-operand products, 0 exact fp32 products"},
     {"VITX_F32_MFMA", VITX_ENV_TUNING, "0: parity-mode GEMMs on the scalar-FMA kernel instead of the fp32 matrix pipe (same bits)"},
     {"VITX_GEMM_KERNEL", VITX_ENV_TUNING, "force one NT tile variant (1, 2, 3, 5, 6, 7, 9, 10, 11, 13; +256 direct / +512 LDS-staged epilogue); every variant adds in the same K order"},
diff --git a/vit-tensorflow_amd/csrc/gemm_bf16.hip b/vit-tensorflow_amd/csrc/gemm_bf16.hip
--- a/vit-tensorflow_amd/csrc/gemm_bf16.hip
+++ b/vit-tensorflow_amd/csrc/gemm_bf16.hip
@@ -380,6 +380,13 @@
   if (on < 0) { const char* v = vitx_env("VITX_GEMM_AUTOTUNE"); on = (v && atoi(v) == 0) ? 0 : 1; }
   return on;
 }
+int gemm_bf16_variant_for(int mode, int M, int N, int K, int has_scale, int shared_gpu) {
+  const std::array<int64_t, 6> key = {mode, M, N, K, 1, (has_scale != 0) + 2 * (g_shared_gpu | (shared_gpu != 0))};
+  std::lock_guard<std::mutex> lk(g_tune_mu);
+  auto it = g_tuned.find(key);
+  return it != g_tuned.end() ? (it->second & 31) : gemm_bf16_pick(M, N);
+}
+
 void launch_gemm_bf16(const Bf16GemmArgs& g0, const EpiParams& ep, int mode, hipStream_t s) {
   const bool few_tiles = ceil_div(g0.M, 256) * ceil_div(g0.N, 256) < 512;
   const double work = (double)g0.M * g0.N * g0.K;
diff --git a/vit-tensorflow_amd/csrc/gemm_bf16_pipe.hip b/vit-tensorflow_amd/csrc/gemm_bf16_pipe.hip
--- a/vit-tensorflow_amd/csrc/gemm_bf16_pipe.hip
+++ b/vit-tensorflow_amd/csrc/gemm_bf16_pipe.hip
@@ -43,6 +43,11 @@
   if (hipMalloc((void**)&d, GT_BYTES) != hipSuccess || hipMemcpy(d, h.data(), GT_BYTES, hipMemcpyHostToDevice) != hipSuccess) d = nullptr;
   per_dev[dev] = d;
   return d;
+}
+
+int gelu_table_on() {
+  static const int on = [] { const char* v = vitx_env("VITX_GELU_TABLE"); return v ? atoi(v) : 1; }();
+  return on;
 }
 
 template <int BM, int BN, int WM, int WN, int MODE>
@@ -534,8 +539,7 @@
   dim3 grid(gx, (unsigned)zs), block(WM * WN * 64);
   const bool walk2_ok = BM == 256 && zs == 1 && gx == (unsigned)grid_cap && (gx & 7) == 0 && gx < (unsigned)(tiles_m * tiles_n) && tiles_n >= 8 && tiles_m >= 64 && g.stagger != 8;
   gp.walk = (walk2_ok && walk_env != 0) ? 2 : 0;
-  static const int gelu_table_on = [] { const char* v = vitx_env("VITX_GELU_TABLE"); return v ? atoi(v) : 1; }();
-  const uint32_t* gtab = (MODE == EPI_BIAS_GELU && BM == 256 && gelu_table_on) ? gelu_table_dev() : nullptr;
+  const uint32_t* gtab = (MODE == EPI_BIAS_GELU && BM == 256 && gelu_table_on()) ? gelu_table_dev() : nullptr;
   hipLaunchKernelGGL(kern, grid, block, SMEM, s, gp, ep, tiles_m, tiles_n, per, gtab);
 }
 
@@ -550,6 +554,8 @@
 }
 
 }
+
+bool gemm_bf16_gelu_table_active() { return gelu_table_on() && gelu_table_dev() != nullptr; }
 
 void launch_gemm_bf16_pipe(int variant, int mode, const Bf16GemmArgs& g, const EpiParams& ep, hipStream_t s) {
   switch (mode) {
diff --git a/vit-tensorflow_amd/csrc/kernels.h b/vit-tensorflow_amd/csrc/kernels.h
--- a/vit-tensorflow_amd/csrc/kernels.h
+++ b/vit-tensorflow_amd/csrc/kernels.h
@@ -52,6 +52,8 @@
   int tail = 0;
 };
 void launch_gemm_bf16(const Bf16GemmArgs& g, const EpiParams& ep, int mode, hipStream_t s);
+int gemm_bf16_variant_for(int mode, int M, int N, int K, int has_scale, int shared_gpu);
+bool gemm_bf16_gelu_table_active();
 int gemm_bf16_tile_m(int kernel, int M, int N);
 int gemm_bf16_tile_n(int kernel, int M, int N);
 int gemm_bf16_num_slices(int K, int split_k);
@@ -62,12 +64,12 @@
 
 bool attn_bf16_supported(int n, int dim_head);
 void launch_attn_bf16_fwd(const bf16_t* qkv, bf16_t* o, float* lse, int b, int n, int h, float scale, const bf16_t* zero_page, int reverse,
-                          hipStream_t s);
+                          hipStream_t s, int nq_live = 0);
 bool attn_x3_supported(int n, int dim_head);
 void launch_attn_x3_fwd(const float* qkv, float* o, float* lse, int b, int n, int h, float scale, hipStream_t s);
 void launch_attn_x3_bwd(const float* qkv, const float* o, const float* d_o, const float* lse, float* dqkv, int b, int n, int h, float scale, hipStream_t s);
 void launch_attn_bf16_bwd(const bf16_t* qkv, const bf16_t* o, const bf16_t* d_o, const float* lse, float* dsum_ws,
-                          bf16_t* dqkv, int b, int n, int h, float scale, const bf16_t* zero_page, hipStream_t s);
+                          bf16_t* dqkv, int b, int n, int h, float scale, const bf16_t* zero_page, hipStream_t s, int nq_live = 0);
 
 constexpr int LSA_N_MAX = 288;
 bool attn_lsa_supported(int n, int dim_head);
@@ -131,6 +133,7 @@
                     hipStream_t s);
 void launch_to_f32(const void* in, int in_bf16, int64_t ldi, float* out, int64_t ldo, int rows, int cols, hipStream_t s);
 void launch_set_token_row(float* x, const float* tok, int b, int ntok, int row, int d, hipStream_t s);
+void launch_copy_rows(const void* src, int64_t src_stride_bytes, void* dst, int64_t dst_stride_bytes, int rows, int row_bytes, hipStream_t s);
 void launch_mean_pool(const float* x, int b, int ntok, int d, float* out, hipStream_t s, int stride_tok = 0);
 void launch_mean_pool_bwd(const float* dp, int b, int ntok, int d, float* g, hipStream_t s, int stride_tok = 0);
 void launch_batch_reduce(const float* g, int b, int ntok, int d, int j0, int nj, float* out, hipStream_t s);
```

Result: faster. 7660 images/sec (median of 6 runs) (+5.2%).
